# koadman/mauveAligner

Hardware: AMD Instinct MI355X
Metric: aligned Mbp/s (seed+extend+DP) (higher is better)
Workload: dtype u32; 1 GPU; C3: 5 x 5000000 bp synthetic genomes, ~3% divergence, ~50 inversions, seed weight 15, recursive anchoring + gapped DP on; genomes_per_gpu=5, genome_length=5000000, seed_weight=15, parallelism=independent genome sets per GPU (no data-path collective), extend_lcbs=1, max_extension_iters=4

## Files before the change

mauvealigner_amd/csrc/assemble_dev.hip:

```cpp
#include "common.hpp"
#include "dev_scan.hpp"
#include <cstring>
#include <cstdlib>
#include <algorithm>

namespace {
using namespace devscan;

__device__ __forceinline__ int64_t as_gap_len(const int32_t *__restrict__ alen, const int32_t *__restrict__ ast, int N, uint32_t k, int g)
{
    const int64_t sa = ast[(size_t)k * N + g], sb = ast[(size_t)(k + 1) * N + g];
    int64_t lo, hi;
    if (sa > 0) { lo = sa + alen[k]; hi = sb - 1; }
    else { lo = -sb + alen[k + 1]; hi = -sa - 1; }
    const int64_t ln = hi - lo + 1;
    return ln < 0 ? 0 : ln;
}

struct AsWidth {
    const int32_t *alen, *ast, *gapcode; const int64_t *dcol_off; int N;
    __device__ int64_t value(uint32_t a) const
    {
        int64_t w = alen[a];
        const int32_t code = gapcode[a];
        if (code >= 0) w += dcol_off[code + 1] - dcol_off[code];
        else if (code == -2) for (int g = 0; g < N; g++) w += as_gap_len(alen, ast, N, a, g);
        return w;
    }
};

__global__ void __launch_bounds__(256) as_lcb(const int32_t *__restrict__ alcb, const int32_t *__restrict__ gapcode, const int64_t *__restrict__ dscore,
                                              const int64_t *__restrict__ col0, uint32_t na, uint32_t *__restrict__ first_a, uint32_t *__restrict__ last_a,
                                              int64_t *__restrict__ lcb_col, unsigned long long *__restrict__ lcb_score)
{
    const uint32_t a = blockIdx.x * 256u + threadIdx.x;
    const bool in = a < na;
    const int32_t l = in ? alcb[a] : 0;
    const int32_t code = in ? gapcode[a] : -1;
    wave_keyed_add(lcb_score, code >= 0, (uint32_t)l, code >= 0 ? (unsigned long long)dscore[code] : 0ull);
    if (!in) return;
    if (a == 0 || alcb[a - 1] != l) { first_a[l] = a; lcb_col[l] = col0[a]; }
    if (a + 1 == na || alcb[a + 1] != l) last_a[l] = a;
}

__global__ void __launch_bounds__(256) as_extents(const int32_t *__restrict__ alen, const int32_t *__restrict__ ast, int N, uint32_t nl,
                                                  const uint32_t *__restrict__ first_a, const uint32_t *__restrict__ last_a,
                                                  int64_t *__restrict__ left, int64_t *__restrict__ right,
                                                  const unsigned long long *__restrict__ lw, int64_t *__restrict__ lw_row,
                                                  const int64_t *__restrict__ total_cols, int64_t *__restrict__ total_row)
{
    const uint32_t t = blockIdx.x * 256u + threadIdx.x;
    if (t >= nl * (uint32_t)N) return;
    const uint32_t l = t / (uint32_t)N; const int g = (int)(t % (uint32_t)N);
    if (g == 0) lw_row[l] = lw ? (int64_t)lw[l] : 0;
    if (t == 0) *total_row = *total_cols;
    const uint32_t a0 = first_a[l], a1 = last_a[l];
    const int64_t s0 = ast[(size_t)a0 * N + g], s1 = ast[(size_t)a1 * N + g];
    int64_t le, re;
    if (s0 > 0) { le = s0; re = s1 + alen[a1] - 1; }
    else { le = -s1; re = -s0 + alen[a0] - 1; }
    left[t] = s0 < 0 ? -le : le; right[t] = s0 < 0 ? -re : re;
}

__global__ void __launch_bounds__(256) as_fill(const int32_t *__restrict__ alen, const int32_t *__restrict__ ast, const int32_t *__restrict__ gapcode,
                                               const int64_t *__restrict__ dcol_off, const uint32_t *__restrict__ dcols,
                                               const int64_t *__restrict__ col0, uint32_t na, int N, uint32_t full, uint32_t *__restrict__ out)
{
    const int lane = threadIdx.x & 63;
    const uint32_t wave = (blockIdx.x * 256u + threadIdx.x) >> 6, nw = (gridDim.x * 256u) >> 6;
    for (uint32_t a = wave; a < na; a += nw) {
        uint32_t *o = out + col0[a];
        const int32_t ln = alen[a];
        for (int32_t c = lane; c < ln; c += 64) o[c] = full;
        o += ln;
        const int32_t code = gapcode[a];
        if (code >= 0) {
            const int64_t s0 = dcol_off[code], n = dcol_off[code + 1] - s0;
            for (int64_t c = lane; c < n; c += 64) o[c] = dcols[s0 + c];
        } else if (code == -2) {
            for (int g = 0; g < N; g++) {
                const int64_t n = as_gap_len(alen, ast, N, a, g);
                for (int64_t c = lane; c < n; c += 64) o[c] = 1u << g;
                o += n;
            }
        }
    }
}

struct Island { int64_t col, len; uint32_t bit, pad; };
__global__ void __launch_bounds__(256) as_islands(const Island *__restrict__ isl, uint32_t n, uint32_t *__restrict__ out)
{
    for (uint32_t k = blockIdx.x; k < n; k += gridDim.x) {
        const Island is = isl[k];
        uint32_t *o = out + is.col;
        for (int64_t c = threadIdx.x; c < is.len; c += 256) o[c] = is.bit;
    }
}

struct SpGenomes { uint64_t word_off[MAUVE_MAX_SEQ]; int32_t s[4][4]; };
template <int MODE>
__global__ void __launch_bounds__(256) sp_score_matches(const uint64_t *__restrict__ packed, SpGenomes G, int n, const int64_t *__restrict__ rec,
                                                        uint32_t nm, int64_t *__restrict__ out, SpMult M)
{
    const int lane = threadIdx.x & 63;
    const uint32_t wave = (blockIdx.x * 256u + threadIdx.x) >> 6, nw = (gridDim.x * 256u) >> 6;
    for (uint32_t i = wave; i < nm; i += nw) {
        const int64_t *r = rec + (size_t)i * (1 + n);
        const int64_t len = r[0];
        int64_t acc = 0;
        for (int64_t c = lane; c < len; c += 64) {
            uint32_t have = 0, bases = 0;
            uint64_t mlo = 0, mhi = 0;
            for (int g = 0; g < n; g++) {
                const int64_t st = r[1 + g];
                if (!st) continue;
                const int64_t p = st > 0 ? st - 1 + c : -st - 1 + (len - 1 - c);
                uint32_t b = (uint32_t)(packed[G.word_off[g] + (uint64_t)(p >> 5)] >> (2 * (p & 31))) & 3u;
                if (st < 0) b = 3u - b;
                have |= 1u << g; bases |= b << (2 * g);
                if (MODE) { const uint64_t mv = M.p[M.off[g] + (uint64_t)p]; if (g < 8) mlo |= mv << (8 * g); else mhi |= mv << (8 * (g - 8)); }
            }
            for (int x = 0; x < n; x++) {
                if (!(have >> x & 1)) continue;
                const uint32_t bx = (bases >> (2 * x)) & 3u;
                const uint32_t mx = MODE ? (uint32_t)((x < 8 ? mlo >> (8 * x) : mhi >> (8 * (x - 8))) & 255u) : 0u;
                for (int y = x + 1; y < n; y++)
                    if (have >> y & 1) {
                        const uint32_t my = MODE ? (uint32_t)((y < 8 ? mlo >> (8 * y) : mhi >> (8 * (y - 8))) & 255u) : 0u;
                        acc += sp_pair<MODE>(G.s[bx][(bases >> (2 * y)) & 3u], mx, my);
                    }
            }
        }
        for (int o = 32; o > 0; o >>= 1) acc += __shfl_xor(acc, o);
        if (lane == 0) out[i] = acc;
    }
}

__global__ void __launch_bounds__(256) as_widen_anchors(const int32_t *__restrict__ alen, const int32_t *__restrict__ ast, const int32_t *__restrict__ alcb, uint32_t na, int N,
                                                        int64_t *__restrict__ olen, int64_t *__restrict__ ost, int64_t *__restrict__ olcb)
{
    const uint32_t i = blockIdx.x * 256u + threadIdx.x;
    if (i < na) { olen[i] = alen[i]; olcb[i] = alcb[i]; }
    if (i < na * (uint32_t)N) ost[i] = ast[i];
}

}

int64_t sp_default_min_weight(int w, int n, const mauve_scoring *sc)
{
    int32_t d = sc->matrix[0][0];
    for (int a = 1; a < 4; a++) d = std::min(d, sc->matrix[a][a]);
    return (int64_t)3 * w * ((int64_t)n * (n - 1) / 2) * d;
}

int match_sp_scores(mauve_ctx *c, const MatchVec &m, const int *gmap, const mauve_scoring *sc, std::vector<int64_t> &out)
{
    const int n = m.N; const size_t nm = m.size();
    out.assign(nm, 0);
    if (nm == 0) return MAUVE_OK;
    if (n > 16) { c->err = "sum-of-pairs LCB scoring: at most 16 genomes"; return MAUVE_ERR_LIMIT; }
    for (size_t i = 0; i < nm; i++)
        for (int g = 0; g < n; g++) {
            const int64_t st = m.st(i)[g], L = c->lens[(size_t)(gmap ? gmap[g] : g)];
            if (st && m.len(i) > 0 && std::llabs(st) + m.len(i) - 1 > L) { c->err = "sp scores: match outside its genome"; return MAUVE_ERR_ARG; }
        }
    SpGenomes G; memset(&G, 0, sizeof G);
    for (int g = 0; g < n; g++) G.word_off[g] = c->word_off[(size_t)(gmap ? gmap[g] : g)];
    memcpy(G.s, sc->matrix, sizeof G.s);
    const size_t rb = nm * (1 + (size_t)n) * 8;
    HIPCHK(c, c->as_work.ensure(rb + nm * 8 + 64));
    HIPCHK(c, c->pin_asm.ensure(rb + nm * 8 + 64));
    int64_t *d_rec = c->as_work.as<int64_t>(), *d_out = d_rec + nm * (1 + (size_t)n);
    memcpy(c->pin_asm.p, m.d.data(), rb);
    HIPCHK(c, hipMemcpyAsync(d_rec, c->pin_asm.p, rb, hipMemcpyHostToDevice, c->stream));
    const uint32_t blocks = (uint32_t)std::min<size_t>((nm + 3) / 4, 256 * 8);
    SpMult M; memset(&M, 0, sizeof M);
    if (c->rp_now != MAUVE_REPEAT_PENALTY_OFF) {
        if (c->rp_gen != c->genome_gen) { c->err = "sp scores: repeat multiplicities missing"; return MAUVE_ERR_STATE; }
        M.p = c->rp_mult.as<uint8_t>();
        for (int g = 0; g < n; g++) M.off[g] = c->rp_off[(size_t)(gmap ? gmap[g] : g)];
    }
    if (c->rp_now == MAUVE_REPEAT_PENALTY_NEGATIVE)
        hipLaunchKernelGGL(sp_score_matches<MAUVE_REPEAT_PENALTY_NEGATIVE>, dim3(blocks), dim3(256), 0, c->stream, c->genomes.as<uint64_t>(), G, n, d_rec, (uint32_t)nm, d_out, M);
    else if (c->rp_now == MAUVE_REPEAT_PENALTY_ZERO)
        hipLaunchKernelGGL(sp_score_matches<MAUVE_REPEAT_PENALTY_ZERO>, dim3(blocks), dim3(256), 0, c->stream, c->genomes.as<uint64_t>(), G, n, d_rec, (uint32_t)nm, d_out, M);
    else
        hipLaunchKernelGGL(sp_score_matches<MAUVE_REPEAT_PENALTY_OFF>, dim3(blocks), dim3(256), 0, c->stream, c->genomes.as<uint64_t>(), G, n, d_rec, (uint32_t)nm, d_out, M);
    HIPCHK(c, hipGetLastError());
    int64_t *h_out = reinterpret_cast<int64_t *>(c->pin_asm.as<char>() + rb);
    HIPCHK(c, hipMemcpyAsync(h_out, d_out, nm * 8, hipMemcpyDeviceToHost, c->stream));
    HIPCHK(c, hipStreamSynchronize(c->stream));
    memcpy(out.data(), h_out, nm * 8);
    return MAUVE_OK;
}

int assemble_device(mauve_ctx *c, int64_t na64, int64_t cells, mauve_align_sizes *sizes, bool host_chains)
{
    static const bool trace = getenv("MAUVE_TRACE") != nullptr;
    AlignState &S = c->ast; AlignResult &R = c->res;
    const int N = S.N; const int64_t nl = S.nl; const uint32_t na = (uint32_t)na64;
    const mauve_ctx::DpFrontOut &fo = c->dpf_out;
    const double t0 = now_ms();
    c->stage.dp_ms = t0 - S.t_dp0;
    const uint32_t nb = (na + TILE - 1) / TILE, blocks = (na + 255) / 256;
    auto up8 = [](size_t x) { return (x + 7) & ~(size_t)7; };
    const size_t o_bsum = ((size_t)na + 1) * 8, o_first = o_bsum + ((size_t)nb + 8) * 8, o_last = up8(o_first + (size_t)nl * 4),
                 o_col = up8(o_last + (size_t)nl * 4), o_left = o_col + ((size_t)nl + 1) * 8, o_right = o_left + (size_t)nl * N * 8,
                 o_score = o_right + (size_t)nl * N * 8, o_lw = o_score + (size_t)nl * 8, o_tot = o_lw + (size_t)nl * 8, w_total = o_tot + 8;
    HIPCHK(c, c->as_work.ensure(w_total + 64));
    HIPCHK(c, c->res_cols.ensure(((size_t)S.sum + 64) * 4));
    char *wk = c->as_work.as<char>();
    int64_t *col0 = reinterpret_cast<int64_t *>(wk), *bsum = reinterpret_cast<int64_t *>(wk + o_bsum);
    uint32_t *first_a = reinterpret_cast<uint32_t *>(wk + o_first), *last_a = reinterpret_cast<uint32_t *>(wk + o_last);
    int64_t *lcb_col = reinterpret_cast<int64_t *>(wk + o_col), *left = reinterpret_cast<int64_t *>(wk + o_left),
            *right = reinterpret_cast<int64_t *>(wk + o_right);
    unsigned long long *score = reinterpret_cast<unsigned long long *>(wk + o_score);
    int64_t *lw_row = reinterpret_cast<int64_t *>(wk + o_lw), *tot_row = reinterpret_cast<int64_t *>(wk + o_tot);
    uint32_t *out = c->res_cols.as<uint32_t>();
    HIPCHK(c, hipMemsetAsync(score, 0, (size_t)nl * 8, c->stream));
    const AsWidth wf{fo.alen, fo.ast, fo.gapcode, fo.col_off, N};
    hipLaunchKernelGGL((vscan_partial<int64_t, AsWidth>), dim3(nb), dim3(256), 0, c->stream, wf, na, bsum);
    hipLaunchKernelGGL((vscan_write<int64_t, AsWidth>), dim3(nb), dim3(256), 0, c->stream, wf, na, bsum, col0, (int64_t *)nullptr);
    hipLaunchKernelGGL(as_lcb, dim3(blocks), dim3(256), 0, c->stream, fo.alcb, fo.gapcode, fo.score, col0, na, first_a, last_a, lcb_col, score);
    hipLaunchKernelGGL(as_extents, dim3(((uint32_t)nl * N + 255) / 256), dim3(256), 0, c->stream, fo.alen, fo.ast, N, (uint32_t)nl, first_a, last_a, left, right,
                       host_chains ? (const unsigned long long *)nullptr : c->ch_lw.as<unsigned long long>(), lw_row, col0 + na, tot_row);
    HIPCHK(c, hipGetLastError());
    const size_t rows_bytes = ((size_t)nl + 1) * 8 + 2 * (size_t)nl * N * 8 + 2 * (size_t)nl * 8 + 8;
    HIPCHK(c, c->pin_asm.ensure(64 + rows_bytes));
    int64_t *h_rows = c->pin_asm.as<int64_t>() + 8;
    HIPCHK(c, hipMemcpyAsync(h_rows, lcb_col, rows_bytes, hipMemcpyDeviceToHost, c->stream));
    {
        const uint32_t fb = (uint32_t)std::min<int64_t>(((int64_t)na + 3) / 4, 256 * 8);
        hipLaunchKernelGGL(as_fill, dim3(fb), dim3(256), 0, c->stream, fo.alen, fo.ast, fo.gapcode, fo.col_off, fo.cols, col0, na, N, S.full, out);
    }
    R.dev_nm = !host_chains && c->matches_pending ? (size_t)c->n_matches : 0;
    if (S.mums_kept >= 0) {
        std::swap(c->sorted_rec, c->sorted_rec_keep);
        R.dev_nm = (size_t)S.mums_kept; S.mums_kept = -1;
    }
    R.dev_alen = fo.alen; R.dev_ast = fo.ast; R.dev_alcb = fo.alcb;
    HIPCHK(c, hipGetLastError());
    if (c->pf.inflight) HIPCHK(c, hipStreamWaitEvent(c->stream, c->ev_io_done, 0));
    HIPCHK(c, hipStreamSynchronize(c->stream));
    c->pf.inflight = false;
    const double t1 = now_ms();
    const int64_t *h_col = h_rows, *h_left = h_col + nl + 1, *h_right = h_left + nl * N, *h_score = h_right + nl * N, *h_lw = h_score + nl;
    const int64_t lcb_cols = h_lw[nl];
    R.col_off.assign(h_col, h_col + nl);
    R.lcb_left.assign(h_left, h_left + nl * N); R.lcb_right.assign(h_right, h_right + nl * N);
    R.dp_score.assign(h_score, h_score + nl);
    if (!host_chains && !S.lw_from_host) R.lcb_weight.assign(h_lw, h_lw + nl);
    R.iv_left.assign((size_t)nl * N, 0); R.iv_right.assign((size_t)nl * N, 0); R.iv_reverse.assign((size_t)nl * N, 0);
    for (int64_t i = 0; i < nl * N; i++) {
        R.iv_left[(size_t)i] = std::llabs(R.lcb_left[(size_t)i]);
        R.iv_right[(size_t)i] = std::llabs(R.lcb_right[(size_t)i]);
        R.iv_reverse[(size_t)i] = R.lcb_left[(size_t)i] < 0;
    }
    int64_t ncols = lcb_cols, niv = nl;
    if (S.p.add_unaligned) {
        std::vector<Island> isl;
        for (int g = 0; g < N; g++) {
            std::vector<std::pair<int64_t, int64_t>> sp;
            for (int64_t l = 0; l < nl; l++) if (R.iv_left[(size_t)l * N + g]) sp.push_back({R.iv_left[(size_t)l * N + g], R.iv_right[(size_t)l * N + g]});
            std::sort(sp.begin(), sp.end());
            int64_t cur = 1;
            for (size_t i = 0; i <= sp.size(); i++) {
                const int64_t lo = cur, hi = i < sp.size() ? sp[i].first - 1 : c->lens[(size_t)g];
                if (hi >= lo) {
                    R.col_off.push_back(ncols);
                    Island is; is.col = ncols; is.len = hi - lo + 1; is.bit = 1u << g; is.pad = 0;
                    isl.push_back(is);
                    ncols += hi - lo + 1;
                    for (int h = 0; h < N; h++) { R.iv_left.push_back(h == g ? lo : 0); R.iv_right.push_back(h == g ? hi : 0); R.iv_reverse.push_back(0); }
                    R.dp_score.push_back(0);
                    niv++;
                }
                if (i < sp.size() && sp[i].second + 1 > cur) cur = sp[i].second + 1;
            }
        }
        if (ncols > S.sum) { c->err = "assemble_device: more columns than bases (internal error)"; return MAUVE_ERR_HIP; }
        if (!isl.empty()) {
            const size_t ib = isl.size() * sizeof(Island);
            HIPCHK(c, c->pin_asm.ensure(64 + rows_bytes + ib + 64));
            char *pi = c->pin_asm.as<char>() + 64 + rows_bytes;
            memcpy(pi, isl.data(), ib);
            HIPCHK(c, c->as_isl.ensure(ib + 64));
            HIPCHK(c, hipMemcpyAsync(c->as_isl.p, pi, ib, hipMemcpyHostToDevice, c->stream));
            hipLaunchKernelGGL(as_islands, dim3((uint32_t)std::min<size_t>(isl.size(), 1024)), dim3(256), 0, c->stream,
                               c->as_isl.as<Island>(), (uint32_t)isl.size(), out);
            HIPCHK(c, hipGetLastError());
            HIPCHK(c, hipStreamSynchronize(c->stream));
        }
    }
    R.col_off.push_back(ncols);
    R.n_cols = (size_t)ncols;
    if (host_chains && !S.anchor_table_done) {
        R.anchor_length.resize((size_t)na); R.anchor_start.resize((size_t)na * N); R.anchor_lcb.resize((size_t)na);
        size_t a = 0;
        for (int64_t l = 0; l < nl; l++) {
            const MatchVec &ch = S.chains[(size_t)l];
            for (size_t i = 0; i < ch.size(); i++, a++) {
                R.anchor_length[a] = ch.len(i); R.anchor_lcb[a] = l;
                std::copy(ch.st(i), ch.st(i) + N, &R.anchor_start[a * N]);
            }
        }
    }
    R.dev_pending = true; R.cols_pending = true; R.dev_na = host_chains ? 0 : na; R.cols_ext = nullptr;
    {
        mauve_ctx::TablePrefetch &P = c->pf;
        const bool dm = P.got_mums && !host_chains, da = P.got_anchors && !host_chains;
        R.del_mum_length = dm ? P.mum_length : nullptr; R.del_mum_start = dm ? P.mum_start : nullptr;
        R.del_alen = da ? P.anchor_length : nullptr; R.del_ast = da ? P.anchor_start : nullptr; R.del_alcb = da ? P.anchor_lcb : nullptr;
        P.got_mums = P.got_anchors = false;
    }
    R.cols_fill = 0; R.cols_dirty.clear();
    R.sz.n_mums = S.nm; R.sz.n_lcb = nl; R.sz.n_anchor = na; R.sz.n_iv = niv; R.sz.n_cols = ncols;
    R.sz.n_gap_dp = fo.n_dp; R.sz.n_dp_cells = cells;
    *sizes = R.sz;
    const double t2 = now_ms();
    if (trace) fprintf(stderr, "[trace] assemble (device): layout+fill %.3f ms, islands+tables %.3f\n", t1 - t0, t2 - t1);
    c->stage.assemble_ms = t2 - t0;
    c->stage.total_ms = t2 - S.t0;
    S.open = false;
    return MAUVE_OK;
}

int materialize_tables(mauve_ctx *c)
{
    AlignResult &R = c->res;
    R.del_mum_length = R.del_mum_start = R.del_alen = R.del_ast = R.del_alcb = nullptr;
    if (!R.dev_pending) return MAUVE_OK;
    HIPCHK(c, hipSetDevice(c->device));
    const int N = c->ast.N; const size_t na = R.dev_na;
    const size_t ab = (na * (2 + (size_t)N) * 4 + 63) & ~(size_t)63, mb = R.dev_nm * (1 + (size_t)N) * 8;
    HIPCHK(c, c->pin_tab.ensure(ab + mb + 64));
    char *pa = c->pin_tab.as<char>();
    if (ab) {
        HIPCHK(c, hipMemcpyAsync(pa, R.dev_alen, na * 4, hipMemcpyDeviceToHost, c->stream));
        HIPCHK(c, hipMemcpyAsync(pa + na * 4, R.dev_ast, na * N * 4, hipMemcpyDeviceToHost, c->stream));
        HIPCHK(c, hipMemcpyAsync(pa + na * 4 * (1 + (size_t)N), R.dev_alcb, na * 4, hipMemcpyDeviceToHost, c->stream));
    }
    if (mb) HIPCHK(c, hipMemcpyAsync(pa + ab, c->sorted_rec.p, mb, hipMemcpyDeviceToHost, c->stream));
    HIPCHK(c, hipStreamSynchronize(c->stream));
    if (mb) {
        const int64_t *hm = reinterpret_cast<const int64_t *>(pa + ab);
        R.mum_length.assign(hm, hm + R.dev_nm); R.mum_start.assign(hm + R.dev_nm, hm + R.dev_nm * (1 + (size_t)N));
        R.dev_nm = 0;
    }
    const int32_t *hl = reinterpret_cast<const int32_t *>(pa), *hs = hl + na, *hb = hs + na * N;
    if (na) {
        R.anchor_length.resize(na); R.anchor_start.resize(na * N); R.anchor_lcb.resize(na);
        for (size_t a = 0; a < na; a++) { R.anchor_length[a] = hl[a]; R.anchor_lcb[a] = hb[a]; }
        for (size_t i = 0; i < na * N; i++) R.anchor_start[i] = hs[i];
    }
    R.dev_pending = false;
    return MAUVE_OK;
}

bool fetch_tables_direct(mauve_ctx *c, int64_t *mum_length, int64_t *mum_start, int64_t *anchor_length, int64_t *anchor_start, int64_t *anchor_lcb, int *rc_out)
{
    AlignResult &R = c->res;
    *rc_out = MAUVE_OK;
    if (!R.dev_pending) return false;
    const int N = c->ast.N; const size_t na = R.dev_na, nm = R.dev_nm;
    if (nm && !(host_pointer_is_pinned(mum_length) && host_pointer_is_pinned(mum_start))) return false;
    if (na && !(host_pointer_is_pinned(anchor_length) && host_pointer_is_pinned(anchor_start) && host_pointer_is_pinned(anchor_lcb))) return false;
    auto chk = [&](hipError_t e) { if (e != hipSuccess && *rc_out == MAUVE_OK) { c->err = std::string("fetch: ") + hipGetErrorString(e); *rc_out = MAUVE_ERR_HIP; } };
    chk(hipSetDevice(c->device));
    if (na) {
        chk(c->as_wide.ensure(na * (2 + (size_t)N) * 8 + 64));
        if (*rc_out) return true;
        int64_t *wl = c->as_wide.as<int64_t>(), *ws = wl + na, *wb = ws + na * N;
        hipLaunchKernelGGL(as_widen_anchors, dim3((uint32_t)((na * N + 255) / 256)), dim3(256), 0, c->stream, R.dev_alen, R.dev_ast, R.dev_alcb, (uint32_t)na, N, wl, ws, wb);
        chk(hipGetLastError());
        chk(hipMemcpyAsync(anchor_length, wl, na * 8, hipMemcpyDeviceToHost, c->stream));
        chk(hipMemcpyAsync(anchor_start, ws, na * N * 8, hipMemcpyDeviceToHost, c->stream));
        chk(hipMemcpyAsync(anchor_lcb, wb, na * 8, hipMemcpyDeviceToHost, c->stream));
    }
    if (nm) {
        const int64_t *rec = c->sorted_rec.as<int64_t>();
        chk(hipMemcpyAsync(mum_length, rec, nm * 8, hipMemcpyDeviceToHost, c->stream));
        chk(hipMemcpyAsync(mum_start, rec + nm, nm * N * 8, hipMemcpyDeviceToHost, c->stream));
    }
    return true;
}

template <typename T>
__global__ void __launch_bounds__(256) as_narrow_cols(const uint32_t *__restrict__ in, size_t n, T *__restrict__ out)
{
    const size_t i0 = ((size_t)blockIdx.x * 256 + threadIdx.x) * 16;
    if (i0 + 16 <= n) {
        uint4 v[4];
#pragma unroll
        for (int q = 0; q < 4; q++) v[q] = reinterpret_cast<const uint4 *>(in + i0)[q];
        T o[16];
#pragma unroll
        for (int q = 0; q < 4; q++) { o[4 * q] = (T)v[q].x; o[4 * q + 1] = (T)v[q].y; o[4 * q + 2] = (T)v[q].z; o[4 * q + 3] = (T)v[q].w; }
        uint4 *dst = reinterpret_cast<uint4 *>(out + i0);
#pragma unroll
        for (int q = 0; q < (int)(sizeof(T) * 16 / 16); q++) dst[q] = reinterpret_cast<const uint4 *>(o)[q];
    } else
        for (size_t i = i0; i < n; i++) out[i] = (T)in[i];
}
__global__ void __launch_bounds__(256) as_narrow_i64(const int64_t *__restrict__ in, size_t n, int32_t *__restrict__ out)
{
    const size_t i = (size_t)blockIdx.x * 256 + threadIdx.x;
    if (i < n) out[i] = (int32_t)in[i];
}

bool fetch_compact_direct(mauve_ctx *c, int col_bytes, int32_t *mum_length, int32_t *mum_start, int32_t *anchor_length, int32_t *anchor_start, int32_t *anchor_lcb,
                          void *cols, bool *tables_done, bool *cols_done, int *rc_out)
{
    AlignResult &R = c->res;
    *rc_out = MAUVE_OK; *tables_done = false; *cols_done = false;
    auto chk = [&](hipError_t e) { if (e != hipSuccess && *rc_out == MAUVE_OK) { c->err = std::string("fetch_compact: ") + hipGetErrorString(e); *rc_out = MAUVE_ERR_HIP; } };
    const int N = c->ast.N; const size_t na = R.dev_na, nm = R.dev_nm;
    bool any = false;
    const bool have_m = R.del_mum_length && R.del_mum_length == mum_length && R.del_mum_start == mum_start;
    const bool have_a = R.del_alen && R.del_alen == anchor_length && R.del_ast == anchor_start && R.del_alcb == anchor_lcb;
    R.del_mum_length = R.del_mum_start = R.del_alen = R.del_ast = R.del_alcb = nullptr;
    if (R.dev_pending && mum_length && mum_start && anchor_length && anchor_start && anchor_lcb &&
        (!nm || have_m || (host_pointer_is_pinned(mum_length) && host_pointer_is_pinned(mum_start))) &&
        (!na || have_a || (host_pointer_is_pinned(anchor_length) && host_pointer_is_pinned(anchor_start) && host_pointer_is_pinned(anchor_lcb)))) {
        chk(hipSetDevice(c->device));
        if (na && !have_a) {
            chk(hipMemcpyAsync(anchor_length, R.dev_alen, na * 4, hipMemcpyDeviceToHost, c->stream));
            chk(hipMemcpyAsync(anchor_start, R.dev_ast, na * N * 4, hipMemcpyDeviceToHost, c->stream));
            chk(hipMemcpyAsync(anchor_lcb, R.dev_alcb, na * 4, hipMemcpyDeviceToHost, c->stream));
        }
        if (nm && !have_m) {
            const size_t n = nm * (1 + (size_t)N);
            chk(c->as_wide.ensure(n * 4 + 64));
            if (*rc_out) return true;
            hipLaunchKernelGGL(as_narrow_i64, dim3((uint32_t)((n + 255) / 256)), dim3(256), 0, c->stream, c->sorted_rec.as<int64_t>(), n, c->as_wide.as<int32_t>());
            chk(hipGetLastError());
            chk(hipMemcpyAsync(mum_length, c->as_wide.as<int32_t>(), nm * 4, hipMemcpyDeviceToHost, c->stream));
            chk(hipMemcpyAsync(mum_start, c->as_wide.as<int32_t>() + nm, nm * N * 4, hipMemcpyDeviceToHost, c->stream));
        }
        *tables_done = true; any = true;
    }
    if (cols && R.n_cols && R.cols_pending && host_pointer_is_pinned(cols)) {
        chk(hipSetDevice(c->device));
        const size_t n = R.n_cols;
        if (col_bytes == 4) chk(hipMemcpyAsync(cols, c->res_cols.p, n * 4, hipMemcpyDeviceToHost, c->stream));
        else {
            chk(c->res_narrow.ensure(n * (size_t)col_bytes + 64));
            if (*rc_out) return true;
            const uint32_t blocks = (uint32_t)((n + 4095) / 4096);
            if (col_bytes == 1) hipLaunchKernelGGL(as_narrow_cols<uint8_t>, dim3(blocks), dim3(256), 0, c->stream, c->res_cols.as<uint32_t>(), n, c->res_narrow.as<uint8_t>());
            else hipLaunchKernelGGL(as_narrow_cols<uint16_t>, dim3(blocks), dim3(256), 0, c->stream, c->res_cols.as<uint32_t>(), n, c->res_narrow.as<uint16_t>());
            chk(hipGetLastError());
            chk(hipMemcpyAsync(cols, c->res_narrow.p, n * (size_t)col_bytes, hipMemcpyDeviceToHost, c->stream));
        }
        *cols_done = true; any = true;
    }
    if (any) chk(hipStreamSynchronize(c->stream));
    return any;
}

int prefetch_tables_enqueue(mauve_ctx *c, int N, int64_t na, const int32_t *alen, const int32_t *ast, const int32_t *alcb)
{
    mauve_ctx::TablePrefetch &P = c->pf;
    P.got_mums = P.got_anchors = false;
    if (!P.live) return MAUVE_OK;
    P.live = false;
    const size_t nm = c->matches_pending && c->dev_rec_n == c->n_matches ? (size_t)c->n_matches : 0;
    const bool mums = nm && P.mum_length && P.mum_start && (int64_t)nm <= P.mum_cap;
    const bool anch = na > 0 && P.anchor_length && P.anchor_start && P.anchor_lcb && na <= P.anchor_cap;
    if (!mums && !anch) return MAUVE_OK;
    const size_t n = nm * (1 + (size_t)N);
    if (mums) {
        HIPCHK(c, c->pf_mums.ensure(n * 4 + 64));
    }
    HIPCHK(c, hipStreamWaitEvent(c->stream_io, c->ev_io_fork, 0));
// ... 52 lines not shown
```

mauvealigner_amd/csrc/common.hpp:

```cpp
#pragma once
#include <hip/hip_runtime.h>
#include <cstdint>
#include <cstdio>
#include <string>
#include <vector>
#include <functional>
#include "workers.hpp"
#include "host_chain.hpp"
#include <chrono>
#include <algorithm>
#include <cstring>

#include "../../include/mauve_hip.h"

#define HIPCHK(ctx, call)                                                                         \
    do {                                                                                          \
        hipError_t e__ = (call);                                                                  \
        if (e__ != hipSuccess) {                                                                  \
            (ctx)->err = std::string(#call) + ": " + hipGetErrorString(e__) + " (" __FILE__ ":" + \
                         std::to_string(__LINE__) + ")";                                          \
            return MAUVE_ERR_HIP;                                                                 \
        }                                                                                         \
    } while (0)

// ... 89 lines not shown
    int64_t *n_matches = nullptr;
};

struct AlignResult {
    mauve_align_sizes sz{};
    std::vector<int64_t> mum_length, mum_start;
    std::vector<int64_t> lcb_left, lcb_right, lcb_weight;
    std::vector<int64_t> anchor_length, anchor_start, anchor_lcb;
    std::vector<int64_t> iv_left, iv_right;
    std::vector<int8_t> iv_reverse;
    std::vector<int64_t> col_off;
    std::vector<uint32_t> cols;
    size_t n_cols = 0;
    uint32_t cols_fill = 0;
    std::vector<std::pair<size_t, size_t>> cols_dirty;
    std::vector<int64_t> dp_score;
    bool stale = false;
    bool genomes_replaced = false;
    bool dev_pending = false;
    bool cols_pending = false;
    size_t dev_na = 0, dev_nm = 0;
    const int32_t *dev_alen = nullptr, *dev_ast = nullptr, *dev_alcb = nullptr;
    const uint32_t *cols_ext = nullptr;
    const int32_t *del_mum_length = nullptr, *del_mum_start = nullptr, *del_alen = nullptr, *del_ast = nullptr, *del_alcb = nullptr;
    const uint32_t *cols_data() const { return cols_ext ? cols_ext : cols.data(); }
};

struct AlignState {
    typedef ::GapRef GapRef;
    struct Item { int64_t lcb; uint32_t idx; int64_t col0; int64_t gap; };
    bool open = false;
    bool anchor_table_done = false;
    bool dev_tail = false;
    const int32_t *dv_len = nullptr, *dv_st = nullptr, *dv_lcb = nullptr;
    bool lw_from_host = false;
    int64_t mums_kept = -1;
    mauve_params p{};
    int N = 0; uint32_t full = 0;
    int64_t sum = 0, nm = 0, nl = 0, n_dp = 0, code_total = 0, n_anchor = 0, anchor_cols = 0;
    double t0 = 0, t_dp0 = 0;
    std::vector<MatchVec> chains;
    std::vector<GapRef> gaps;
    std::vector<DpSeqDesc> desc;
    std::vector<int64_t> dcol_off, dscore;
    MatchVec m;
    std::vector<int64_t> match_lcb;
    std::vector<int64_t> match_weight;
    std::vector<Item> items;
    void count_anchors() { for (const MatchVec &ch : chains) { n_anchor += (int64_t)ch.size(); for (size_t i = 0; i < ch.size(); i++) anchor_cols += ch.len(i); } }
    void reset()
    {
        open = false; anchor_table_done = false; dev_tail = false; dv_len = dv_st = dv_lcb = nullptr; lw_from_host = false; mums_kept = -1; p = mauve_params(); N = 0; full = 0;
        sum = nm = nl = n_dp = code_total = n_anchor = anchor_cols = 0; t0 = t_dp0 = 0;
        gaps.clear(); desc.clear(); dcol_off.clear(); dscore.clear();
        match_lcb.clear(); match_weight.clear(); items.clear();
    }
};

struct CoordDev;
struct mauve_ctx {
    int device = 0;
    hipStream_t stream = nullptr;
    hipStream_t stream2 = nullptr;
    hipEvent_t ev_fork = nullptr, ev_join = nullptr;
    hipStream_t stream_io = nullptr;
    hipEvent_t ev_io_fork = nullptr, ev_io_done = nullptr;
    struct TablePrefetch {
        int32_t *mum_length = nullptr, *mum_start = nullptr, *anchor_length = nullptr, *anchor_start = nullptr, *anchor_lcb = nullptr;
        int64_t mum_cap = 0, anchor_cap = 0;
        bool armed = false;
        bool live = false;
        bool inflight = false;
        bool got_mums = false, got_anchors = false;
    } pf;
    DevBuf pf_mums;
    std::string err;
    char devname[256] = {0};
    int cus = 256;

    int nseq = 0;
    std::vector<int64_t> lens;
    std::vector<uint64_t> word_off;
    std::vector<const uint64_t *> host_packed;
    PinnedBuf pin_genomes;
    PinnedBuf pin_tail;
    bool host_copy_valid = false;
    size_t total_words = 0;
    DevBuf genomes;
    DevBuf base_invalid, contig_mask, node_cmask;
    bool has_invalid = false, has_contigs = false;
    std::vector<uint64_t> h_invalid, h_contig, base_mask_off;

    DevBuf keysA, keysB, valsA, valsB, hist, totals, posmask, hit_mask, hit_pos, hit_seg, cand, mlen, mstart, counters;
    DevBuf sorted_rec;
    DevBuf canon_k1, canon_k2, canon_v1, canon_v2;
    DevBuf join_bound;
    DevBuf join_ovf;
    DevBuf ch_len, ch_st, ch_crop, ch_ent, ch_ord, ch_rank, ch_node, ch_graph, ch_cnt;
    DevBuf gap_work;
    DevBuf ch_big;
    DevBuf ch_anch, ch_lw;
    DevBuf ch_anch2, ext_work, sorted_rec_keep;
    PinnedBuf pin_ext;
    DevBuf ch_mw;
    DevBuf as_wide;
    DevBuf res_narrow;
    DevBuf hom_cols;
    DevBuf as_work, as_isl, res_cols;
    PinnedBuf pin_tab;
    PinnedBuf pin_asm, pin_cols;
    PinnedBuf pin_chain;
    PinnedBuf pin_mask;
    struct BackboneResult {
        int N = 0; bool valid = false;
        std::vector<int64_t> seg_iv, seg_col, seg_len, seg_left, seg_right, islands;
        std::vector<uint32_t> seg_mask;
    } bb;
    PinnedBuf pin_bb;
    DevBuf bb_cols, bb_work, bb_query;
    size_t bb_rec_cap = 0;
    struct CoordIndex { bool valid = false; int N = 0; int64_t n_iv = 0, n_cols = 0; uint64_t genome_gen = 0; struct ::CoordDev *dev = nullptr; } co;
    DevBuf co_index, co_q;
    PinnedBuf pin_stage;
    CoordIndex co_truth;
    DevBuf co_truth_index, sc_out;
    struct ExtractSel {
        bool valid = false; uint64_t genome_gen = 0;
        int64_t n_sel = 0, n_range = 0;
        int n_keep = 0; int32_t keep[MAUVE_MAX_SEQ] = {0};
    } ex;
    DevBuf ex_work, ex_bits, ex_sel, ex_mat;
    DevBuf ps_work, ps_out;
    struct Excursions { bool valid = false; uint64_t genome_gen = 0; int64_t n_stream = 0, n_exc = 0; } exc;
    DevBuf exc_work, exc_tmp, exc_meta, exc_rec;
    DevBuf run_sum;
    DevBuf rec_vinv, rec_vcm;
    DevBuf rec_genomes, rec_seg;
    DevBuf placed_mask;
    std::vector<int64_t> match_len, match_start;
    int64_t n_matches = 0;
    int64_t dev_rec_n = -1;

    DevBuf dp_desc, dp_list, dp_codes, dp_off, dp_prof_cnt, dp_prof_mask, dp_prof2_cnt, dp_prof2_mask, dp_tb, dp_meta, dp_score,
        dp_cols, dp_rows, dp_sp, dp_pick, dp_wflags;

    bool pair_sums_only = false;
    std::vector<int64_t> pair_sums;
    int64_t bp_min_len = -1;
    std::vector<int64_t> pair_bp;
    DevBuf bp_work;
    std::vector<uint8_t> rec_flags;
    bool lazy_matches_ok = false, matches_pending = false;
    int match_nseq = 0;
    struct DpFrontOut { const int32_t *alen, *ast, *alcb, *gapcode; const int64_t *col_off, *score; const uint32_t *cols; int64_t n_dp, n_cols; } dpf_out{};
    std::vector<DpSeqDesc> prog_desc;
    const int64_t *dp_last_col_off = nullptr; int64_t dp_last_n = 0;
    int64_t dp_band_from = INT64_MAX;
    DevBuf dpf_anch, dpf_work, dpf_tot;

    bool prof = false;
    hipEvent_t ev0 = nullptr, ev1 = nullptr;
    double k_ms[MAUVE_K_COUNT] = {0};
    int64_t k_launch[MAUVE_K_COUNT] = {0};
    int64_t k_units[MAUVE_K_COUNT] = {0};

    PinnedBuf pin_anch;
    PinnedBuf pin_dcols;
    PinnedBuf pin_meta;
    PinnedBuf pin_dp_in;
    PinnedBuf pin_seed;
    struct DpHost {
        std::vector<int64_t> tb_off, rows_off, est, need, nmax, lst, lst2, seq_off, tb_list;
        std::vector<uint8_t> is_big, cls;
    } dph;
    struct SeedHost {
        std::vector<int32_t> hl, hs;
        std::vector<uint32_t> order, tmp;
        std::vector<uint64_t> k1;
    } sdh;

    std::function<void()> shadow;

    SpinPool *pool = nullptr;

    int shard_rank = 0, shard_world = 1; mauve_allgather_fn shard_fn = nullptr; void *shard_user = nullptr;
    bool shard_on = false;
    void *shard_comm = nullptr;
    DevBuf shard_dev;
    PinnedBuf shard_pin;
    mauve_shard_stats shard_stat = {0, 0, 0, 0.0};

    int repeat_mode = MAUVE_REPEAT_PENALTY_OFF, rp_now = MAUVE_REPEAT_PENALTY_OFF;
    uint64_t genome_gen = 0;
    uint64_t rp_gen = 0, rp_pat = 0;
    DevBuf rp_wcnt, rp_mult;
    std::vector<uint64_t> rp_off;

    AlignResult res;
    AlignState ast;
    mauve_stage_times stage{};
};

struct SpMult { const uint8_t *p; uint64_t off[MAUVE_MAX_SEQ]; };
template <int MODE>
__device__ __forceinline__ int64_t sp_pair(int32_t s, uint32_t mx, uint32_t my)
{
    if (MODE == MAUVE_REPEAT_PENALTY_OFF || s <= 0) return s;
    const int64_t r = (int64_t)(mx > my ? mx : my);
    return MODE == MAUVE_REPEAT_PENALTY_NEGATIVE ? (int64_t)s * (2 - r) / r : (int64_t)s / r;
}

struct RepeatScope {
    mauve_ctx *c;
    explicit RepeatScope(mauve_ctx *ctx) : c(ctx) { c->rp_now = MAUVE_REPEAT_PENALTY_OFF; }
    ~RepeatScope() { c->rp_now = MAUVE_REPEAT_PENALTY_OFF; }
};

struct KernelTimer {
    mauve_ctx *c; int id; int64_t units;
    KernelTimer(mauve_ctx *ctx, int kid, int64_t u) : c(ctx), id(kid), units(u)
    {
        if (c->prof) (void)hipEventRecord(c->ev0, c->stream);
    }
    ~KernelTimer()
    {
        if (!c->prof) return;
        (void)hipEventRecord(c->ev1, c->stream);
        (void)hipEventSynchronize(c->ev1);
        float ms = 0.f;
        (void)hipEventElapsedTime(&ms, c->ev0, c->ev1);
        c->k_ms[id] += ms; c->k_launch[id] += 1; c->k_units[id] += units;
    }
};

static inline double now_ms()
{
    using namespace std::chrono;
    return duration<double, std::milli>(steady_clock::now().time_since_epoch()).count();
}

int rec_gap_flags_device(mauve_ctx *c, const int32_t *alen, const int32_t *ast, const int32_t *alcb, int64_t na, int N, int64_t min_gap, uint8_t *d_flag);
int shard_allgather(mauve_ctx *c, const void *send, size_t bytes, std::vector<std::pair<const char *, size_t>> &parts);
void shard_lpt(const std::vector<int64_t> &cost, int world, std::vector<int> &owner);
bool make_seed_shape(uint64_t pattern, SeedShape *out);
GenomeSet main_genome_set(mauve_ctx *ctx);
bool seedpass_wide(int64_t total_windows);
int refuse_scoring(mauve_ctx *c, const mauve_scoring *sc, const char *what);
int refuse_scoring_batch(mauve_ctx *c, const mauve_scoring *sc, int nseq, int64_t n_iv, const int64_t *seq_off, const char *what);
int refuse_scoring_params(mauve_ctx *c, const mauve_params *p, const char *what);
int refuse_past_2g(mauve_ctx *c, const char *what);
int seedpass_run(mauve_ctx *ctx, const GenomeSet &gs, uint64_t pattern, int mode, uint64_t mask, int extend,
                 const uint32_t *seg_dev, uint32_t nseg, int64_t *n_matches);
int seedpass_enumerate(mauve_ctx *ctx, const GenomeSet &gs, int seq, uint64_t pattern, EnumRequest &q);
int seedpass_from_hits(mauve_ctx *ctx, const GenomeSet &gs, uint64_t pattern, const HostHits &hits, int extend, int64_t *n_matches);
int seedpass_sorted_list(mauve_ctx *ctx, const GenomeSet &gs, int seq, uint64_t pattern, std::vector<uint64_t> *keys,
                         std::vector<uint32_t> *vals, int *weight);

int sort_pairs_u32(mauve_ctx *ctx, uint32_t n, int key_bits, uint32_t **keys_io, uint32_t **vals_io, uint32_t *keys_alt, uint32_t *vals_alt,
                   int timer_id);
int sort_pairs_u32_batch(mauve_ctx *ctx, uint32_t S, uint32_t n, size_t seg_stride, int key_bits, uint32_t **keys_io, uint32_t **vals_io,
                         uint32_t *keys_alt, uint32_t *vals_alt, int timer_id);
int sort_pairs_u64(mauve_ctx *ctx, uint32_t n, int key_bits, uint64_t **keys_io, uint32_t **vals_io, uint64_t *keys_alt, uint32_t *vals_alt,
                   int timer_id);
int seed_finish(mauve_ctx *ctx, const GenomeSet &gs, const SeedRequest &rq, uint32_t ncand, bool on_host, double &trace_t0);
bool seed_trace_on();
uint32_t canon_device_min();
inline void seed_trace(mauve_ctx *ctx, const char *label, double &t0)
{
    if (!seed_trace_on()) return;
    (void)hipStreamSynchronize(ctx->stream);
    const double t = now_ms();
    fprintf(stderr, "[trace] %-22s +%.3f ms\n", label, t - t0);
    t0 = t;
}
inline int seed_counters(mauve_ctx *ctx, size_t bytes, const uint32_t **words)
{
    HIPCHK(ctx, ctx->pin_seed.ensure(64));
    HIPCHK(ctx, hipMemcpyAsync(ctx->pin_seed.p, ctx->counters.p, bytes, hipMemcpyDeviceToHost, ctx->stream));
    HIPCHK(ctx, hipStreamSynchronize(ctx->stream));
    *words = ctx->pin_seed.as<uint32_t>();
    return MAUVE_OK;
}
int chain_device(mauve_ctx *c, int N, int64_t min_weight, bool collinear, MatchVec &m, std::vector<int64_t> &match_lcb, int64_t &n_lcb, const mauve_scoring *sp_scoring = nullptr);
struct ChainGraphHost { uint32_t na, K; int64_t *weight; uint32_t *orient; int32_t *prev, *next; int32_t *final_stage; int32_t *final_dev; };
int chain_device_graph(mauve_ctx *c, int N, int64_t maxlen, const uint32_t *seg0, uint32_t nseg, ChainGraphHost *G, bool graph_to_host = true, const mauve_scoring *sp_scoring = nullptr);
int chain_device_gaps_compact(mauve_ctx *c, int N, int64_t maxlen, const uint32_t *seg0_dev, uint32_t nseg, const int32_t **hl_out, const int32_t **hs_out,
                              const uint32_t **hgap_out, uint32_t *ns_out);
int chain_device_core(mauve_ctx *c, int N, int64_t min_weight, bool collinear, int64_t &n_lcb, const mauve_scoring *sp_scoring = nullptr);
int chain_device_gaps(mauve_ctx *c, int N, int64_t maxlen, const uint32_t *seg0_dev, uint32_t nseg, const int32_t **hl_out, const int32_t **hs_out,
                      std::vector<uint8_t> &survive);
int chain_device_copy_back(mauve_ctx *c, int N, MatchVec &m, std::vector<int64_t> &match_lcb);
int chain_order_device(mauve_ctx *c, int N, int64_t nl, int64_t min_gap, int64_t *na_out, int64_t *n_rec_out);
int extend_lcbs_device(mauve_ctx *c, const mauve_params *p, int w, int64_t lcbw, int N, const int32_t **alen_io, const int32_t **ast_io,
                       const int32_t **alcb_io, int64_t *na_io, int64_t *nl_io, int64_t *n_rec_io, std::vector<int64_t> &lcb_weight);

struct ChainOrders { std::vector<std::vector<uint32_t>> ord; bool sparse = false; };
void host_eliminate_overlaps(MatchVec &m, ChainOrders *orders = nullptr, bool compact = true);
int seed_family_matches(mauve_ctx *c, const GenomeSet &gs, int w, int mode, uint64_t mask, MatchVec &out);
void host_merge_matches(MatchVec &kept, const MatchVec &add);
void host_left_orders(const MatchVec &m, ChainOrders &orders);
void host_lcb_chain(const MatchVec &m, int64_t min_weight, bool collinear, std::vector<int64_t> &match_lcb, int64_t &n_lcb,
                    const ChainOrders *orders = nullptr, const int64_t *match_weight = nullptr);
int match_sp_scores(mauve_ctx *c, const MatchVec &m, const int *gmap, const mauve_scoring *sc, std::vector<int64_t> &out);
int repeat_multiplicity(mauve_ctx *c, uint64_t pattern);
int repeat_begin(mauve_ctx *c, const mauve_params *p, int w, uint64_t pat);
int64_t sp_default_min_weight(int w, int n, const mauve_scoring *sc);
int resolve_seed(mauve_ctx *c, const mauve_params *p, int64_t avg_len, const char *who, int *w, uint64_t *pat);
void seed_matches_to_vec(const mauve_ctx *c, int n, int64_t nm, MatchVec &m);
int host_chain_lcbs(mauve_ctx *c, const mauve_params *p, MatchVec &m, const int *gmap, int64_t lcbw, int64_t minw_sp, std::vector<int64_t> &match_lcb,
                    int64_t &nl, std::vector<int64_t> *match_weight, bool compact, double *t_elim = nullptr);
void result_reset(AlignResult &R);
void restore_cols(AlignResult &R, uint32_t full, SpinPool *pool = nullptr);

void lcb_greedy(int N, int32_t K, int64_t *weight, const uint32_t *orient_bits, int32_t *prevv, int32_t *nextv, int64_t min_weight,
                bool collinear, std::vector<int64_t> &final_id, int64_t &n_lcb);

int dp_batch_run_desc(mauve_ctx *ctx, int nseq, int64_t n_iv, const DpSeqDesc *desc, const mauve_scoring *sc,
                      uint32_t *cols, int64_t *col_off, int64_t *score, int64_t *cells, bool may_shard = false, int64_t *sp = nullptr);
bool dp_desc_rotations_on_device(int64_t n_total);
int dp_batch_run_desc_rot(mauve_ctx *ctx, int nseq, int64_t n_orig, const DpSeqDesc *desc, const int32_t *cbase, int64_t n_total, const mauve_scoring *sc,
                          int64_t *col_off, int64_t *score, int64_t *cells, int64_t *sp);
inline int64_t dp_len_limit(const mauve_params *p) { return p->max_banded_len > p->max_gapped_len ? p->max_banded_len : p->max_gapped_len; }
inline int64_t dp_band_from_of(const mauve_params *p) { return p->max_banded_len > p->max_gapped_len ? p->max_gapped_len : INT64_MAX; }
int dp_run_from_anchors(mauve_ctx *ctx, int N, int64_t na, const int32_t *h_len, const int32_t *h_st, const int32_t *h_lcb, int gapped,
                        int64_t max_gapped_len, const mauve_scoring *scoring, int32_t *gapcode, int64_t *n_dp_out, int64_t *code_total_out,
                        PinnedBuf *dcols, std::vector<int64_t> &dcol_off, std::vector<int64_t> &dscore, int64_t *cells, int stay = 0);
int assemble_device(mauve_ctx *c, int64_t na, int64_t cells, mauve_align_sizes *sizes, bool host_chains = false);
int check_columns(mauve_ctx *c, const char *who, int N, int64_t n_iv, const int64_t *left, const int64_t *right, const int64_t *col_off, const uint32_t *d_cols);
void coord_index_release(mauve_ctx *c);
int coord_index_arrays(mauve_ctx *c, const char *who, mauve_ctx::CoordIndex &X, DevBuf &index, int nseq, int64_t n_iv, const int64_t *left, const int64_t *right,
                       const int8_t *reverse, const int64_t *col_off, const uint32_t *cols);
int materialize_result(mauve_ctx *c);
int materialize_tables(mauve_ctx *c);
int fetch_columns(mauve_ctx *c, uint32_t *dst);
bool fetch_compact_direct(mauve_ctx *c, int col_bytes, int32_t *mum_length, int32_t *mum_start, int32_t *anchor_length, int32_t *anchor_start, int32_t *anchor_lcb,
                          void *cols, bool *tables_done, bool *cols_done, int *rc_out);
int prefetch_tables_enqueue(mauve_ctx *c, int N, int64_t na, const int32_t *alen, const int32_t *ast, const int32_t *alcb);
bool fetch_tables_direct(mauve_ctx *c, int64_t *mum_length, int64_t *mum_start, int64_t *anchor_length, int64_t *anchor_start, int64_t *anchor_lcb, int *rc_out);
bool host_pointer_is_pinned(const void *p);
inline int copy_to_caller(mauve_ctx *c, PinnedBuf &pin, void *dst, const void *src, size_t bytes)
{
    if (!bytes) return MAUVE_OK;
    if (host_pointer_is_pinned(dst)) { HIPCHK(c, hipMemcpyAsync(dst, src, bytes, hipMemcpyDeviceToHost, c->stream)); return MAUVE_OK; }
    const size_t piece = (size_t)64 << 20;
    HIPCHK(c, pin.ensure(std::min(bytes, piece)));
    for (size_t o = 0; o < bytes; o += piece) {
        const size_t n = std::min(piece, bytes - o);
        HIPCHK(c, hipMemcpyAsync(pin.p, static_cast<const char *>(src) + o, n, hipMemcpyDeviceToHost, c->stream));
        HIPCHK(c, hipStreamSynchronize(c->stream));
        memcpy(static_cast<char *>(dst) + o, pin.p, n);
    }
    return MAUVE_OK;
}
int host_genomes(mauve_ctx *c);
int seed_matches_to_host(mauve_ctx *ctx);
int dp_fetch_picked(mauve_ctx *ctx, int64_t n_pick, const int64_t *pick, const int64_t *col_off, uint32_t *out, int64_t *out_off);
int dp_batch_run(mauve_ctx *ctx, int nseq, int64_t n_iv, const uint8_t *codes, const int64_t *seq_off,
                 const mauve_scoring *sc, uint32_t *cols, int64_t *col_off, int64_t *score, int64_t *cells);
```

mauvealigner_amd/csrc/dev_scan.hpp:

```cpp
#pragma once
#include <hip/hip_runtime.h>
#include <cstdint>

namespace devscan {

constexpr int TILE = 1024;

__device__ __forceinline__ uint32_t bscan_add(uint32_t v, uint32_t *total, uint32_t *lds )
{
    const int lane = threadIdx.x & 63, wave = threadIdx.x >> 6;
    uint32_t inc = v;
#pragma unroll
    for (int o = 1; o < 64; o <<= 1) { const uint32_t t = __shfl_up(inc, o); if (lane >= o) inc += t; }
    __syncthreads();
    if (lane == 63) lds[wave] = inc;
    __syncthreads();
    uint32_t wbase = 0, tot = 0;
#pragma unroll
    for (int w = 0; w < 4; w++) { const uint32_t c = lds[w]; if (w < wave) wbase += c; tot += c; }
    *total = tot;
    return wbase + inc - v;
}
__device__ __forceinline__ uint32_t bscan_max(uint32_t v, uint32_t *total, uint32_t *lds )
{
    const int lane = threadIdx.x & 63, wave = threadIdx.x >> 6;
    uint32_t inc = v;
#pragma unroll
    for (int o = 1; o < 64; o <<= 1) { const uint32_t t = __shfl_up(inc, o); if (lane >= o) inc = max(inc, t); }
    __syncthreads();
    if (lane == 63) lds[wave] = inc;
    __syncthreads();
    uint32_t wbase = 0, tot = 0;
#pragma unroll
    for (int w = 0; w < 4; w++) { const uint32_t c = lds[w]; if (w < wave) wbase = max(wbase, c); tot = max(tot, c); }
    *total = tot;
    const uint32_t up = __shfl_up(inc, 1);
    return max(wbase, lane ? up : 0u);
}
__device__ __forceinline__ void tiles_before_add(const uint32_t *__restrict__ v, uint32_t b, uint32_t nb, uint32_t *before, uint32_t *all, uint32_t *lds)
{
    uint32_t sb = 0, sa = 0;
    for (uint32_t t = threadIdx.x; t < nb; t += 256) { const uint32_t x = v[t]; sa += x; if (t < b) sb += x; }
    uint32_t tb, ta;
    (void)bscan_add(sb, &tb, lds); (void)bscan_add(sa, &ta, lds);
    *before = tb; *all = ta;
}

__device__ __forceinline__ void wave_keyed_add(unsigned long long *arr, bool active, uint32_t l, unsigned long long v)
{
    const uint64_t act = __ballot(active);
    if (!act) return;
    const int first = __ffsll((unsigned long long)act) - 1;
    const uint32_t l0 = (uint32_t)__shfl((int)l, first);
    if (__ballot(active && l == l0) == act) {
        unsigned long long s = active ? v : 0ull;
#pragma unroll
        for (int o = 32; o > 0; o >>= 1) s += __shfl_xor(s, o);
        if ((int)(threadIdx.x & 63) == first) atomicAdd(&arr[l0], s);
    } else if (active) atomicAdd(&arr[l], v);
}

template <class F>
__global__ void __launch_bounds__(256) cmp_count(F f, uint32_t *__restrict__ bcnt)
{
    __shared__ uint32_t lds[4];
    const int y = blockIdx.y;
    const uint32_t dom = f.domain(y), r0 = blockIdx.x * (uint32_t)TILE + threadIdx.x * 4u;
    uint32_t c = 0;
#pragma unroll
    for (int i = 0; i < 4; i++) if (r0 + i < dom) c += f.flag(r0 + i, y) ? 1u : 0u;
    uint32_t tc;
    (void)bscan_add(c, &tc, lds);
    if (threadIdx.x == 0) bcnt[(size_t)y * gridDim.x + blockIdx.x] = tc;
}
template <class F>
__global__ void __launch_bounds__(256) cmp_write(F f, const uint32_t *__restrict__ bcnt)
{
    __shared__ uint32_t lds[4];
    const int y = blockIdx.y;
    const uint32_t dom = f.domain(y), r0 = blockIdx.x * (uint32_t)TILE + threadIdx.x * 4u;
    uint32_t before, all;
    tiles_before_add(bcnt + (size_t)y * gridDim.x, blockIdx.x, gridDim.x, &before, &all, lds);
    bool fl[4]; uint32_t c = 0;
#pragma unroll
    for (int i = 0; i < 4; i++) { fl[i] = r0 + i < dom && f.flag(r0 + i, y); c += fl[i] ? 1u : 0u; }
    uint32_t dummy;
    uint32_t o = before + bscan_add(c, &dummy, lds);
#pragma unroll
    for (int i = 0; i < 4; i++) {
        if (r0 + i >= dom) break;
        f.each(r0 + i, o, fl[i], y);
        if (fl[i]) { f.emit(r0 + i, o, y); o++; }
    }
    if (blockIdx.x == 0 && threadIdx.x == 0) f.total(all, y);
}


template <class T, class In>
__global__ void __launch_bounds__(256) vscan_partial(In in, uint32_t n, T *__restrict__ bsum)
{
    __shared__ T red[4];
    const uint32_t r0 = blockIdx.x * (uint32_t)TILE + threadIdx.x * 4u;
    T s = 0;
#pragma unroll
    for (int i = 0; i < 4; i++) if (r0 + i < n) s += in.value(r0 + i);
#pragma unroll
    for (int o = 32; o > 0; o >>= 1) s += __shfl_down(s, o);
    if ((threadIdx.x & 63) == 0) red[threadIdx.x >> 6] = s;
    __syncthreads();
    if (threadIdx.x == 0) bsum[blockIdx.x] = red[0] + red[1] + red[2] + red[3];
}
template <class T, class In>
__global__ void __launch_bounds__(256) vscan_write(In in, uint32_t n, const T *__restrict__ bsum, T *__restrict__ out, T *__restrict__ total)
{
    __shared__ T red[4];
    __shared__ T s_before, s_all;
    const int lane = threadIdx.x & 63, wave = threadIdx.x >> 6;
    T sb = 0, sa = 0;
    for (uint32_t t = threadIdx.x; t < gridDim.x; t += 256) { const T x = bsum[t]; sa += x; if (t < blockIdx.x) sb += x; }
#pragma unroll
    for (int o = 32; o > 0; o >>= 1) { sb += __shfl_down(sb, o); sa += __shfl_down(sa, o); }
    if (lane == 0) red[wave] = sb;
    __syncthreads();
    if (threadIdx.x == 0) s_before = red[0] + red[1] + red[2] + red[3];
    __syncthreads();
    if (lane == 0) red[wave] = sa;
    __syncthreads();
    if (threadIdx.x == 0) s_all = red[0] + red[1] + red[2] + red[3];
    __syncthreads();
    const uint32_t r0 = blockIdx.x * (uint32_t)TILE + threadIdx.x * 4u;
    T v[4], s = 0;
#pragma unroll
    for (int i = 0; i < 4; i++) { v[i] = r0 + i < n ? in.value(r0 + i) : (T)0; s += v[i]; }
    T inc = s;
#pragma unroll
    for (int o = 1; o < 64; o <<= 1) { const T t = __shfl_up(inc, o); if (lane >= o) inc += t; }
    __syncthreads();
    if (lane == 63) red[wave] = inc;
    __syncthreads();
    T run = s_before + inc - s;
    for (int w = 0; w < wave; w++) run += red[w];
#pragma unroll
    for (int i = 0; i < 4; i++) { if (r0 + i < n) out[r0 + i] = run; run += v[i]; }
    if (blockIdx.x == 0 && threadIdx.x == 0) { if (total) *total = s_all; out[n] = s_all; }
}

}
```

mauvealigner_amd/csrc/dp_batch.hip:

```cpp
#include "common.hpp"
#include "dev_scan.hpp"
#include <algorithm>
#include <functional>
#include <cstring>
#include <cstdlib>

#define DP_NEG_INF (-(1 << 29))

struct DpMeta {
    int32_t m;
    int32_t krows;
    int32_t cur;
    int32_t pad;
    int64_t score;
    int64_t cells;
};

struct DpScoring { int32_t go, ge; int32_t s[4][4]; };

__device__ __forceinline__ void dp_row_coef(uint32_t cn, const DpScoring &sc, int32_t &s0, int32_t &s1, int32_t &s2, int32_t &s3, int32_t &gxo, int32_t &gxe)
{
    const int32_t c0 = cn & 255, c1 = (cn >> 8) & 255, c2 = (cn >> 16) & 255, c3 = cn >> 24;
    const int32_t rr = c0 + c1 + c2 + c3;
    s0 = c0 * sc.s[0][0] + c1 * sc.s[1][0] + c2 * sc.s[2][0] + c3 * sc.s[3][0];
// ... 1437 lines not shown
        }
        for (int o = 32; o; o >>= 1) total += __shfl_xor(total, o);
        if (lane == 0) out[iv] = (unsigned long long)total;
    }
}

struct DpGenomeWords { uint64_t word_off[MAUVE_MAX_SEQ]; };

__global__ void __launch_bounds__(256) dp_gather_codes(const uint64_t *__restrict__ packed, DpGenomeWords gw,
                                                       const DpSeqDesc *__restrict__ desc, const int64_t *__restrict__ seq_off,
                                                       int64_t ndesc, uint8_t *__restrict__ codes)
{
    const int lane = threadIdx.x & 63, sub = lane >> 4, sl = lane & 15;
    const int64_t wave_global = ((int64_t)blockIdx.x * blockDim.x + threadIdx.x) >> 6;
    const int64_t nwaves = ((int64_t)gridDim.x * blockDim.x) >> 6;
    for (int64_t d0 = wave_global * 4; d0 < ndesc; d0 += nwaves * 4) {
        const int64_t d = d0 + sub;
        if (d >= ndesc) continue;
        const DpSeqDesc ds = desc[d];
        const uint64_t *G = packed + gw.word_off[ds.genome];
        uint8_t *out = codes + seq_off[d];
        for (int64_t i = sl; i < ds.len; i += 16) {
            const int64_t p = ds.rev ? ds.lo0 + ds.len - 1 - i : ds.lo0 + i;
            const uint32_t b = (uint32_t)(G[p >> 5] >> (2 * (p & 31))) & 3u;
            out[i] = (uint8_t)(ds.rev ? 3u - b : b);
        }
    }
}

struct DpSizing {
    int64_t need = 0, est = 0;
    __host__ __device__ DpSizing(int64_t band_from, bool no_mw_, bool no_groups_, int class_mode, int64_t longest)
        : banded(longest > band_from), no_mw(no_mw_), no_groups(no_groups_), mode(class_mode) {}
    __host__ __device__ void add(int64_t n)
    {
        if (n == 0) return;
        if (first) { first = false; mmax = mmin = n; return; }
        const int64_t tbo = dp_tb_need(mmin, mmax, n, banded);
        const int64_t tbn = banded ? tbo : max2(tbo, max2(dp2_tb_need(mmax, n), dp3_tb_need(mmax, n)));
        rneed = max2(rneed, dp3_rows_need(mmax, n));
        need = max2(need, tbn);
        nmax = max2(nmax, n);
        const int64_t e_m = min2(mmax, mmin + mmin / 8 + 2);
        if (max2(e_m, n) > DP3_BAND && !no_mw) wide = true;
        est += dp3_scan_steps(e_m, n);
        crows = max2(crows, mode == 0 ? e_m : min2(mmax, mode == 1 ? mmax : mmin / 2 + 1));
        mmax += n; mmin = max2(mmin, n);
    }
    __host__ __device__ int64_t rows() const { return max2(6 * (nmax + 1), rneed); }
    __host__ __device__ uint8_t cand() const { return banded && nmax ? 2 : (wide ? 1 : 0); }
    __host__ __device__ uint8_t cls() const
    {
        if (no_groups || banded) return 1;
        if (crows <= 4 * DP2_R && nmax + 4 <= DP2_T) return 4;
        if (crows <= 8 * DP2_R && nmax + 8 <= DP2_T) return 3;
        if (crows <= 16 * DP2_R && nmax + 16 <= DP2_T) return 2;
        return 1;
    }
    __host__ __device__ static uint32_t sizekey(int64_t need) { int c = 0; for (int64_t f = need; f > 1; f >>= 1) c++; return (uint32_t)(63 - c); }
    __host__ __device__ uint32_t sizekey() const { return sizekey(need); }
private:
    __host__ __device__ static int64_t max2(int64_t a, int64_t b) { return a > b ? a : b; }
    __host__ __device__ static int64_t min2(int64_t a, int64_t b) { return a < b ? a : b; }
    bool banded, no_mw, no_groups, wide = false, first = true; int mode;
    int64_t mmin = 0, mmax = 0, nmax = 0, rneed = 0, crows = 0;
};

static int dp_class_mode()
{
    static const int m = []() { const char *e = getenv("MAUVE_DP_CLASS"); return !e ? 0 : (!strcmp(e, "bound") ? 1 : (!strcmp(e, "wild") ? 2 : 0)); }();
    return m;
}
static int64_t dp_wide_min() { static const int64_t f = getenv("MAUVE_DP_WIDE_MIN") ? atoll(getenv("MAUVE_DP_WIDE_MIN")) : 1024; return f; }
static int64_t dp_big_max() { static const int64_t m = getenv("MAUVE_DP_BIG_MAX") ? atoll(getenv("MAUVE_DP_BIG_MAX")) : 256; return m; }
static bool dp_wide_on() { static const bool o = getenv("MAUVE_DP_NO_WIDE") == nullptr; return o; }

static int dp_launch_steps(mauve_ctx *ctx, int nseq, int64_t a, int64_t b, int64_t n_big, int64_t big_len, const DpClasses &full, const int64_t *d_seq_off,
                           const int64_t *d_tb_off, const int64_t *d_rows_off, const DpScoring &sc, int64_t tb_base, int64_t band_from)
{
    auto clip = [&](int64_t first, int64_t n, int64_t &f2, int64_t &n2) { f2 = std::max(first, a); n2 = std::max<int64_t>(0, std::min(first + n, b) - f2); };
    int64_t bf, bn;
    clip(0, n_big, bf, bn);
    DpClasses cl; memset(&cl, 0, sizeof cl);
    clip(full.first_med, full.n_med, cl.first_med, cl.n_med);
    clip(full.first_c, full.n_c, cl.first_c, cl.n_c);
    clip(full.first_s32, full.n_s32, cl.first_s32, cl.n_s32);
    clip(full.first_s16, full.n_s16, cl.first_s16, cl.n_s16);
    static const bool no_scan = getenv("MAUVE_DP_NOSCAN") != nullptr;
    cl.scan = no_scan ? 0 : 1;
    const int64_t wpb = DP2_WAVES, cap = 256 * 16;
    cl.blocks_med = (uint32_t)std::min<int64_t>((cl.n_med + wpb - 1) / wpb, cap);
    cl.blocks_c = (uint32_t)std::min<int64_t>((cl.n_c + 4 * wpb - 1) / (4 * wpb), cap);
    cl.blocks_s32 = (uint32_t)std::min<int64_t>((cl.n_s32 + 8 * wpb - 1) / (8 * wpb), cap);
    const uint32_t blocks = cl.blocks_med + cl.blocks_c + cl.blocks_s32 + (uint32_t)std::min<int64_t>((cl.n_s16 + 16 * wpb - 1) / (16 * wpb), cap);
    uint8_t *tb = ctx->dp_tb.as<uint8_t>() - tb_base;
    KernelTimer t(ctx, MAUVE_K_DP, b - a);
#define DP_STEP_ARGS ctx->dp_codes.as<uint8_t>(), d_seq_off, ctx->dp_meta.as<DpMeta>(), ctx->dp_prof_cnt.as<uint32_t>(), ctx->dp_prof_mask.as<uint32_t>(), \
                     ctx->dp_prof2_cnt.as<uint32_t>(), ctx->dp_prof2_mask.as<uint32_t>(), tb, d_tb_off, ctx->dp_rows.as<int32_t>(), d_rows_off, \
                     ctx->dp_score.as<uint8_t>(), sc
    hipStream_t small_stream = bn ? ctx->stream2 : ctx->stream;
    if (bn) {
        HIPCHK(ctx, hipEventRecord(ctx->ev_fork, ctx->stream));
        HIPCHK(ctx, hipStreamWaitEvent(ctx->stream2, ctx->ev_fork, 0));
        const bool wide = dp_wide_on();
        static const int64_t cl_max = getenv("MAUVE_DP_CLUSTER") ? atoll(getenv("MAUVE_DP_CLUSTER")) : 32;
        const int64_t n_cl = wide ? std::min<int64_t>(bn, cl_max) : 0;
        unsigned long long *flags = nullptr;
        if (n_cl) {
            HIPCHK(ctx, ctx->dp_wflags.ensure((size_t)n_cl * DPW_FLAGS * 8));
            HIPCHK(ctx, hipMemsetAsync(ctx->dp_wflags.p, 0, (size_t)n_cl * DPW_FLAGS * 8, ctx->stream));
            flags = ctx->dp_wflags.as<unsigned long long>();
        }
#define DPW_LAUNCH(first, count, K) hipLaunchKernelGGL((dp_step_wide<4, 8>), dim3((uint32_t)((count) * (K))), dim3(64 * 8), 0, ctx->stream, nseq, \
                               ctx->dp_list.as<int64_t>() + bf + (first), DP_STEP_ARGS, band_from, (int)(K), flags)
        if (wide) { if (n_cl) DPW_LAUNCH(0, n_cl, DPW_KMAX); if (bn > n_cl) DPW_LAUNCH(n_cl, bn - n_cl, 1); }
#undef DPW_LAUNCH
        if (!wide || band_from != INT64_MAX || !dp3_admissible(std::max<int64_t>(big_len, 1), nseq, sc.ge, sc.go))
            hipLaunchKernelGGL(dp_step_big, dim3((uint32_t)bn), dim3(64 * DP_MW_WAVES), 0, ctx->stream, nseq, ctx->dp_list.as<int64_t>() + bf, DP_STEP_ARGS,
                               band_from, wide ? 1 : 0);
    }
    if (blocks) hipLaunchKernelGGL(dp_step2, dim3(blocks), dim3(64 * DP2_WAVES), 0, small_stream, nseq, ctx->dp_list.as<int64_t>(), cl, DP_STEP_ARGS);
#undef DP_STEP_ARGS
    if (bn) { HIPCHK(ctx, hipEventRecord(ctx->ev_join, ctx->stream2)); HIPCHK(ctx, hipStreamWaitEvent(ctx->stream, ctx->ev_join, 0)); }
    return MAUVE_OK;
}

static int64_t dp_tb_budget()
{
    static const int64_t b = getenv("MAUVE_DP_TB_BUDGET") ? atoll(getenv("MAUVE_DP_TB_BUDGET")) : (8LL << 30);
    return std::max<int64_t>(b, 1 << 16);
}
static int dp_launch_rounds(mauve_ctx *ctx, int nseq, int64_t n_iv, int64_t n_big, int64_t big_len, const DpClasses &cl, const int64_t *d_seq_off,
                            const int64_t *d_tb_off, const int64_t *d_rows_off, const DpScoring &sc, const int64_t *tb_list, int *rounds_out,
                            int64_t band_from)
{
    const int64_t budget = dp_tb_budget();
    int rounds = 0;
    for (int64_t a = 0; a < n_iv;) {
        int64_t b = a + 1;
        if (tb_list) {
            if (tb_list[a + 1] - tb_list[a] > budget) { ctx->err = "dp: one interval needs more traceback than MAUVE_DP_TB_BUDGET allows"; return MAUVE_ERR_LIMIT; }
            while (b < n_iv && tb_list[b + 1] - tb_list[a] <= budget) b++;
        } else b = n_iv;
        int rc = dp_launch_steps(ctx, nseq, a, b, n_big, big_len, cl, d_seq_off, d_tb_off, d_rows_off, sc, tb_list ? tb_list[a] : 0, band_from);
        if (rc) return rc;
        rounds++;
        a = b;
    }
    if (rounds_out) *rounds_out = rounds;
    return MAUVE_OK;
}

static const char *const DP_ERR_CLUSTER = "dp: a cluster of workgroups could not make progress on an interval (wide sweep)";
static DpScoring dp_scoring_of(const mauve_scoring *scoring)
{
    DpScoring sc; sc.go = scoring->gap_open; sc.ge = scoring->gap_extend; memcpy(sc.s, scoring->matrix, sizeof sc.s);
    return sc;
}
static int dp_ensure_batch(mauve_ctx *ctx, int64_t total, int64_t tbt, int64_t rwt)
{
    HIPCHK(ctx, ctx->dp_codes.ensure((size_t)total + 16));
    HIPCHK(ctx, ctx->dp_prof_cnt.ensure((size_t)(total + 1) * 4));
    HIPCHK(ctx, ctx->dp_prof_mask.ensure((size_t)(total + 1) * 4));
    HIPCHK(ctx, ctx->dp_prof2_cnt.ensure((size_t)(total + 1) * 4));
    HIPCHK(ctx, ctx->dp_prof2_mask.ensure((size_t)(total + 1) * 4));
    HIPCHK(ctx, ctx->dp_tb.ensure((size_t)std::min<int64_t>(tbt, dp_tb_budget()) + 64));
    HIPCHK(ctx, ctx->dp_rows.ensure((size_t)(rwt + 1) * 4));
    HIPCHK(ctx, ctx->dp_score.ensure((size_t)total + 16));
    HIPCHK(ctx, ctx->dp_cols.ensure((size_t)(total + 1) * 4));
    return MAUVE_OK;
}
static void dp_launch_gather_codes(mauve_ctx *ctx, const int64_t *d_seq_off, int64_t nd)
{
    DpGenomeWords gw; memset(&gw, 0, sizeof gw);
    for (int g = 0; g < ctx->nseq; g++) gw.word_off[g] = ctx->word_off[g];
    const uint32_t gb = (uint32_t)std::min<int64_t>((nd + 15) / 16, 256 * 8);
    hipLaunchKernelGGL(dp_gather_codes, dim3(gb), dim3(256), 0, ctx->stream, ctx->genomes.as<uint64_t>(), gw, ctx->dp_desc.as<DpSeqDesc>(), d_seq_off, nd,
                       ctx->dp_codes.as<uint8_t>());
}

static int dp_core(mauve_ctx *ctx, int nseq, int64_t n_iv, const uint8_t *codes, const DpSeqDesc *desc,
                   const int64_t *seq_off, const mauve_scoring *scoring, uint32_t *cols, int64_t *col_off,
                   int64_t *score, int64_t *cells, int64_t *sp = nullptr)
{
    if (cells) *cells = 0;
    col_off[0] = 0;
    if (n_iv == 0) return MAUVE_OK;
    static const bool trace = getenv("MAUVE_TRACE") != nullptr;
    const double td0 = now_ms();
    const int64_t total = seq_off[n_iv * nseq];
    mauve_ctx::DpHost &H = ctx->dph;
    std::vector<int64_t> &tb_off = H.tb_off, &rows_off = H.rows_off, &est = H.est;
    std::vector<uint8_t> &is_big = H.is_big;
    tb_off.resize((size_t)n_iv + 1); rows_off.resize((size_t)n_iv + 1);
    is_big.assign((size_t)n_iv, 0); est.assign((size_t)n_iv, 0);
    int64_t est_total = 0;
    const int64_t band_from = ctx->dp_band_from;
    static const bool no_mw = getenv("MAUVE_DP_ONE_WAVE") != nullptr;
    static const bool no_groups = getenv("MAUVE_DP_NO_GROUPS") != nullptr;
    std::vector<uint8_t> &cls = H.cls; cls.assign((size_t)n_iv, 1);
    int64_t tbt = 0, rwt = 0;
    std::vector<int64_t> &need_v = H.need, &nmax_v = H.nmax;
    need_v.resize((size_t)n_iv); nmax_v.resize((size_t)n_iv);
    ctx->pool->parallel_for(n_iv, 2048, [&](int64_t b, int64_t e) {
        for (int64_t iv = b; iv < e; iv++) {
            int64_t longest = 0;
            for (int g = 0; g < nseq; g++) longest = std::max(longest, seq_off[iv * nseq + g + 1] - seq_off[iv * nseq + g]);
            DpSizing z(band_from, no_mw, no_groups, dp_class_mode(), longest);
            for (int g = 0; g < nseq; g++) z.add(seq_off[iv * nseq + g + 1] - seq_off[iv * nseq + g]);
            need_v[(size_t)iv] = z.need; nmax_v[(size_t)iv] = z.rows(); est[(size_t)iv] = z.est; is_big[(size_t)iv] = z.cand(); cls[(size_t)iv] = z.cls();
        }
    });
    for (int64_t iv = 0; iv < n_iv; iv++) {
        tb_off[iv] = tbt; rows_off[iv] = rwt;
        tbt += need_v[(size_t)iv]; rwt += nmax_v[(size_t)iv];
        est_total += est[(size_t)iv];
    }
    tb_off[n_iv] = tbt; rows_off[n_iv] = rwt;

    const DpScoring sc = dp_scoring_of(scoring);
    std::vector<int64_t> &lst = H.lst; lst.resize((size_t)n_iv);
    {
        int64_t cnt[66] = {0};
        auto cls = [&](int64_t iv) { return DpSizing::sizekey(need_v[(size_t)iv]); };
        for (int64_t iv = 0; iv < n_iv; iv++) cnt[cls(iv) + 1]++;
        for (int c = 0; c < 65; c++) cnt[c + 1] += cnt[c];
        for (int64_t iv = 0; iv < n_iv; iv++) lst[(size_t)cnt[cls(iv)]++] = iv;
    }
    int64_t n_big = 0;
    {
        for (int64_t k = 0; k < n_iv; k++) {
            uint8_t &b = is_big[(size_t)lst[(size_t)k]];
            if (b == 1 && (n_big >= dp_big_max() || est[(size_t)lst[(size_t)k]] < dp_wide_min())) b = 0;
            n_big += b != 0;
        }
    }
    DpClasses cl; memset(&cl, 0, sizeof cl);
    {
        std::vector<int64_t> &tmp = H.lst2; tmp.resize((size_t)n_iv);
        int64_t cnt4[5] = {0, 0, 0, 0, 0};
        auto klass = [&](int64_t iv) { return is_big[(size_t)iv] ? 0 : (int)cls[(size_t)iv]; };
        for (int64_t k = 0; k < n_iv; k++) cnt4[klass(lst[(size_t)k])]++;
        int64_t pos[5] = {0, cnt4[0], cnt4[0] + cnt4[1], cnt4[0] + cnt4[1] + cnt4[2], cnt4[0] + cnt4[1] + cnt4[2] + cnt4[3]};
        cl.first_med = pos[1]; cl.n_med = cnt4[1]; cl.first_c = pos[2]; cl.n_c = cnt4[2]; cl.first_s32 = pos[3]; cl.n_s32 = cnt4[3]; cl.first_s16 = pos[4]; cl.n_s16 = cnt4[4];
        for (int64_t k = 0; k < n_iv; k++) { const int64_t iv = lst[(size_t)k]; tmp[(size_t)pos[klass(iv)]++] = iv; }
        lst.swap(tmp);
    }
    int64_t big_len = 0;
    for (int64_t k = 0; k < n_big; k++) { const int64_t iv = lst[(size_t)k]; big_len = std::max(big_len, seq_off[(iv + 1) * nseq] - seq_off[iv * nseq]); }
    std::vector<int64_t> &tb_list = H.tb_list; tb_list.resize((size_t)n_iv + 1);
    tbt = 0;
    for (int64_t k = 0; k < n_iv; k++) { const int64_t iv = lst[(size_t)k]; tb_off[iv] = tbt; tb_list[(size_t)k] = tbt; tbt += need_v[(size_t)iv]; }
    tb_list[(size_t)n_iv] = tbt; tb_off[n_iv] = tbt;
    const bool one_round = tbt <= dp_tb_budget();

    { int rce = dp_ensure_batch(ctx, total, tbt, rwt); if (rce) return rce; }
    HIPCHK(ctx, ctx->dp_off.ensure((size_t)(n_iv * nseq + 1 + 3 * (n_iv + 1)) * sizeof(int64_t)));
    HIPCHK(ctx, ctx->dp_meta.ensure((size_t)n_iv * sizeof(DpMeta)));
    int64_t *d_seq_off = ctx->dp_off.as<int64_t>();
    int64_t *d_tb_off = d_seq_off + (n_iv * nseq + 1);
    int64_t *d_rows_off = d_tb_off + (n_iv + 1);
    int64_t *d_col_off = d_rows_off + (n_iv + 1);
    const size_t n_so = (size_t)(n_iv * nseq + 1), n_o = (size_t)n_iv + 1;
    const size_t desc_bytes = desc ? (size_t)n_iv * nseq * sizeof(DpSeqDesc) : 0;
    HIPCHK(ctx, ctx->pin_dp_in.ensure((n_so + 3 * n_o) * 8 + desc_bytes + 64));
    int64_t *pin_off = ctx->pin_dp_in.as<int64_t>();
    memcpy(pin_off, seq_off, n_so * 8);
    memcpy(pin_off + n_so, tb_off.data(), n_o * 8);
    memcpy(pin_off + n_so + n_o, rows_off.data(), n_o * 8);
    HIPCHK(ctx, hipMemcpyAsync(d_seq_off, pin_off, (n_so + 2 * n_o) * 8, hipMemcpyHostToDevice, ctx->stream));
    if (desc) {
        const int64_t nd = n_iv * nseq;
        HIPCHK(ctx, ctx->dp_desc.ensure((size_t)nd * sizeof(DpSeqDesc)));
        char *pin_desc = reinterpret_cast<char *>(pin_off + n_so + 3 * n_o);
        memcpy(pin_desc, desc, desc_bytes);
        HIPCHK(ctx, hipMemcpyAsync(ctx->dp_desc.p, pin_desc, desc_bytes, hipMemcpyHostToDevice, ctx->stream));
        dp_launch_gather_codes(ctx, d_seq_off, nd);
    } else if (total) {
        HIPCHK(ctx, hipMemcpyAsync(ctx->dp_codes.p, codes, (size_t)total, hipMemcpyHostToDevice, ctx->stream));
    }
    const double td1 = now_ms();
    HIPCHK(ctx, ctx->dp_list.ensure((size_t)n_iv * 8));
    int64_t *pin_list = pin_off + n_so + 2 * n_o;
    memcpy(pin_list, lst.data(), (size_t)n_iv * 8);
    HIPCHK(ctx, hipMemcpyAsync(ctx->dp_list.p, pin_list, (size_t)n_iv * 8, hipMemcpyHostToDevice, ctx->stream));
    int rounds = 1;
    { int rcl = dp_launch_rounds(ctx, nseq, n_iv, n_big, big_len, cl, d_seq_off, d_tb_off, d_rows_off, sc, one_round ? nullptr : tb_list.data(), &rounds, band_from); if (rcl) return rcl; }
    HIPCHK(ctx, hipGetLastError());
    if (ctx->shadow) { std::function<void()> f; f.swap(ctx->shadow); f(); }
    HIPCHK(ctx, ctx->pin_meta.ensure((size_t)n_iv * sizeof(DpMeta)));
    DpMeta *hm = ctx->pin_meta.as<DpMeta>();
    const double td2 = now_ms();
    HIPCHK(ctx, hipMemcpyAsync(hm, ctx->dp_meta.p, (size_t)n_iv * sizeof(DpMeta), hipMemcpyDeviceToHost, ctx->stream));
    HIPCHK(ctx, hipStreamSynchronize(ctx->stream));
    const double td3 = now_ms();
    int64_t tc = 0, ncell = 0;
    for (int64_t iv = 0; iv < n_iv; iv++) {
        if (hm[iv].pad) { ctx->err = DP_ERR_CLUSTER; return MAUVE_ERR_HIP; }
        col_off[iv] = tc; tc += hm[iv].m; ncell += hm[iv].cells;
        if (score) score[iv] = hm[iv].score;
    }
    col_off[n_iv] = tc;
    if (cells) *cells = ncell;
    ctx->dp_last_col_off = d_col_off; ctx->dp_last_n = n_iv;
    if (tc) {
        HIPCHK(ctx, hipMemcpyAsync(d_col_off, col_off, (size_t)(n_iv + 1) * 8, hipMemcpyHostToDevice, ctx->stream));
        const uint32_t gblocks = (uint32_t)std::min<int64_t>((n_iv + 3) / 4, 256 * 8);
        hipLaunchKernelGGL(dp_gather, dim3(gblocks), dim3(256), 0, ctx->stream, nseq, n_iv, d_seq_off, ctx->dp_meta.as<DpMeta>(),
                           ctx->dp_prof_mask.as<uint32_t>(), ctx->dp_prof2_mask.as<uint32_t>(), d_col_off,
                           ctx->dp_cols.as<uint32_t>());
        HIPCHK(ctx, hipGetLastError());
        if (sp && nseq >= 2) {
            HIPCHK(ctx, ctx->dp_sp.ensure((size_t)n_iv * 8 + 64));
            HIPCHK(ctx, hipMemsetAsync(ctx->dp_sp.p, 0, (size_t)n_iv * 8, ctx->stream));
            hipLaunchKernelGGL(dp_sp_scores, dim3((uint32_t)std::min<int64_t>((n_iv + 3) / 4, 256 * 16)), dim3(256), 0, ctx->stream, nseq, n_iv, ctx->dp_codes.as<uint8_t>(), d_seq_off,
                               ctx->dp_cols.as<uint32_t>(), d_col_off, sc, ctx->dp_sp.as<unsigned long long>());
            HIPCHK(ctx, hipGetLastError());
            HIPCHK(ctx, hipMemcpyAsync(ctx->pin_meta.p, ctx->dp_sp.p, (size_t)n_iv * 8, hipMemcpyDeviceToHost, ctx->stream));
        }
        if (cols) HIPCHK(ctx, hipMemcpyAsync(cols, ctx->dp_cols.p, (size_t)tc * 4, hipMemcpyDeviceToHost, ctx->stream));
        HIPCHK(ctx, hipStreamSynchronize(ctx->stream));
        if (sp && nseq >= 2) memcpy(sp, ctx->pin_meta.p, (size_t)n_iv * 8);
    }
    if (sp && (!tc || nseq < 2)) for (int64_t iv = 0; iv < n_iv; iv++) sp[iv] = 0;
    if (trace) {
        std::vector<int64_t> e2(est); std::sort(e2.begin(), e2.end(), std::greater<int64_t>());
        fprintf(stderr, "[trace] dp_core: %d round(s); %lld intervals: %lld workgroup, %lld one-wave, %lld two/wave, %lld four/wave; single-wave steps: total %lld (balanced %lld), top", rounds, (long long)n_iv,
                (long long)n_big, (long long)cl.n_med, (long long)cl.n_s32, (long long)cl.n_s16, (long long)est_total, (long long)(est_total / 3072));
        for (size_t i = 0; i < e2.size() && i < 8; i++) fprintf(stderr, " %lld", (long long)e2[i]);
        fprintf(stderr, "\n");
    }
    if (trace) fprintf(stderr, "[trace] dp_core: sizing+H2D %.3f ms, order+launch %.3f, kernel+meta D2H %.3f, gather+cols D2H %.3f\n",
                       td1 - td0, td2 - td1, td3 - td2, now_ms() - td3);
    return MAUVE_OK;
}


namespace {
using namespace devscan;

struct DpFrontTotals {
    int64_t codes, tb, rows, est, n_dp, first_med, first_s32, first_s16, cols, cells, first_c, err;
    unsigned long long big_len;
};

__device__ __forceinline__ void dpf_gap(const int32_t *__restrict__ alen, const int32_t *__restrict__ ast, int N, uint32_t k, int g,
                                        int64_t &lo, int64_t &ln, bool &rev)
{
    const int64_t sa = ast[(size_t)k * N + g], sb = ast[(size_t)(k + 1) * N + g];
    int64_t hi;
    if (sa > 0) { lo = sa + alen[k]; hi = sb - 1; rev = false; }
    else { lo = -sb + alen[k + 1]; hi = -sa - 1; rev = true; }
    ln = hi - lo + 1; if (ln < 0) ln = 0;
}

__global__ void __launch_bounds__(256) dpf_gap_flags(const int32_t *__restrict__ alen, const int32_t *__restrict__ ast,
                                                     const int32_t *__restrict__ alcb, uint32_t na, int N, int gapped, int64_t max_gapped,
                                                     int32_t *__restrict__ gapcode, uint32_t *__restrict__ totals_words)
{
    const uint32_t k = blockIdx.x * 256u + threadIdx.x;
    if (k < 64) totals_words[k] = 0;
    if (k >= na) return;
    int32_t code = -1;
    if (k + 1 < na && alcb[k] == alcb[k + 1]) {
        int64_t tot = 0, mx = 0; int nonempty = 0;
        for (int g = 0; g < N; g++) {
            int64_t lo, ln; bool rv;
            dpf_gap(alen, ast, N, k, g, lo, ln, rv);
            tot += ln; mx = max(mx, ln); nonempty += ln > 0;
        }
        if (tot > 0) code = (gapped && nonempty >= 2 && mx <= max_gapped) ? 0 : -2;
    }
    gapcode[k] = code;
}
struct DpSlots {
    int32_t *gapcode; uint32_t na; uint32_t *anchor_of; DpFrontTotals *tot;
    __device__ uint32_t domain(int) const { return na; }
    __device__ bool flag(uint32_t k, int) const { return gapcode[k] == 0; }
    __device__ void each(uint32_t, uint32_t, bool, int) const {}
    __device__ void emit(uint32_t k, uint32_t o, int) const { gapcode[k] = (int32_t)o; anchor_of[o] = k; }
    __device__ void total(uint32_t n, int) const { tot->n_dp = n; }
};

struct DpSizingOut {
    int64_t *need, *rowsn, *est; uint8_t *cand, *cls; uint32_t *sizekey, *slotval;
    __device__ void put(uint32_t s, const DpSizing &z) const
    {
        need[s] = z.need; rowsn[s] = z.rows(); est[s] = z.est; cand[s] = z.cand(); cls[s] = z.cls();
        sizekey[s] = z.sizekey(); slotval[s] = s;
    }
};
__global__ void __launch_bounds__(256) dpf_desc(const int32_t *__restrict__ alen, const int32_t *__restrict__ ast, int N,
                                                const uint32_t *__restrict__ anchor_of, const DpFrontTotals *__restrict__ tot,
                                                DpSeqDesc *__restrict__ desc, DpSizingOut out, int no_mw, int no_groups, int64_t band_from, int class_mode)
{
    const uint32_t s = blockIdx.x * 256u + threadIdx.x;
    if (s >= (uint32_t)tot->n_dp) return;
    const uint32_t k = anchor_of[s];
    int64_t longest = 0;
    for (int g = 0; g < N; g++) {
        int64_t lo, n; bool rv;
        dpf_gap(alen, ast, N, k, g, lo, n, rv);
        longest = max(longest, n);
    }
    DpSizing z(band_from, no_mw, no_groups, class_mode, longest);
    for (int g = 0; g < N; g++) {
        int64_t lo, n; bool rv;
        dpf_gap(alen, ast, N, k, g, lo, n, rv);
        DpSeqDesc d; d.genome = g; d.rev = rv; d.lo0 = lo - 1; d.len = n;
        desc[(size_t)s * N + g] = d;
        z.add(n);
    }
    out.put(s, z);
}
__global__ void __launch_bounds__(256) dpf_size_desc(const DpSeqDesc *__restrict__ desc, int N, uint32_t n, DpFrontTotals *__restrict__ tot,
                                                     DpSizingOut out, int no_mw, int no_groups, int64_t band_from, int class_mode)
{
    const uint32_t s = blockIdx.x * 256u + threadIdx.x;
    if (s == 0) tot->n_dp = n;
    if (s >= n) return;
    int64_t longest = 0;
    for (int g = 0; g < N; g++) longest = max(longest, desc[(size_t)s * N + g].len);
    DpSizing z(band_from, no_mw, no_groups, class_mode, longest);
    for (int g = 0; g < N; g++) z.add(desc[(size_t)s * N + g].len);
    out.put(s, z);
}
struct DescLen { const DpSeqDesc *d; __device__ int64_t value(uint32_t i) const { return d[i].len; } };
struct ArrVal { const int64_t *a; __device__ int64_t value(uint32_t i) const { return a[i]; } };
struct ListVal { const int64_t *a; const uint32_t *order; __device__ int64_t value(uint32_t j) const { return a[order[j]]; } };
__global__ void __launch_bounds__(256) dpf_tb_scatter(const int64_t *__restrict__ tb_list, const uint32_t *__restrict__ order, uint32_t n, int64_t *__restrict__ tb_off)
{
    const uint32_t j = blockIdx.x * 256u + threadIdx.x;
    if (j < n) tb_off[order[j]] = tb_list[j];
}

struct DpBigPick {
    const uint32_t *order; const uint8_t *cand, *cls; const int64_t *est; const DpFrontTotals *tot; uint32_t *key2; int64_t wide_min; uint32_t maxn;
    __device__ uint32_t domain(int) const { return (uint32_t)tot->n_dp; }
    __device__ bool flag(uint32_t j, int) const { const uint32_t s = order[j]; return cand[s] == 1 && est[s] >= wide_min; }
    __device__ void each(uint32_t j, uint32_t before, bool fl, int) const { key2[j] = ((fl && before < maxn) || cand[order[j]] == 2) ? 0u : (uint32_t)cls[order[j]]; }
    __device__ void emit(uint32_t, uint32_t, int) const {}
    __device__ void total(uint32_t, int) const {}
};
__global__ void __launch_bounds__(256) dpf_list(const uint32_t *__restrict__ key2, const uint32_t *__restrict__ order, DpFrontTotals *__restrict__ tot,
                                                int64_t *__restrict__ list, const int64_t *__restrict__ seq_off, int N)
{
    const uint32_t n = (uint32_t)tot->n_dp, j = blockIdx.x * 256u + threadIdx.x;
    if (j < n) {
        const uint32_t s = order[j];
        list[j] = s;
        if (key2[j] == 0) atomicMax(&tot->big_len, (unsigned long long)(seq_off[((size_t)s + 1) * N] - seq_off[(size_t)s * N]));
    }
    if (j < 4) {
        uint32_t lo = 0, hi = n;
        while (lo < hi) { const uint32_t mid = (lo + hi) / 2; if (key2[mid] >= j + 1) hi = mid; else lo = mid + 1; }
        if (j == 0) tot->first_med = lo; else if (j == 1) tot->first_c = lo; else if (j == 2) tot->first_s32 = lo; else tot->first_s16 = lo;
    }
}
struct MetaCols { const DpMeta *m; __device__ int64_t value(uint32_t i) const { return m[i].m; } };
struct MetaCells { const DpMeta *m; __device__ int64_t value(uint32_t i) const { return m[i].cells; } };
__global__ void __launch_bounds__(256) dpf_scores(const DpMeta *__restrict__ meta, uint32_t n, int64_t *__restrict__ score, DpFrontTotals *__restrict__ tot)
{
    const uint32_t i = blockIdx.x * 256u + threadIdx.x;
    if (i < n) { score[i] = meta[i].score; if (meta[i].pad) tot->err = 1; }
}

}

struct DpFrontWork {
    DpSeqDesc *desc; DpFrontTotals *tot;
    int64_t *need, *rowsn, *est; uint8_t *cand, *cls;
    uint32_t *k1, *v1, *k2, *v2, *k3, *bcnt; int64_t *bsum, *bsum2;
    int64_t *d_seq_off, *d_tb_off, *d_rows_off, *d_col_off;
    DpSizingOut sizing() const { return DpSizingOut{need, rowsn, est, cand, cls, k1, v1}; }
};
static int dpf_work_area(mauve_ctx *ctx, uint32_t na, int N, DpFrontWork &W)
{
    const uint32_t nb = (na + TILE - 1) / TILE;
    auto up8 = [](size_t x) { return (x + 7) & ~(size_t)7; };
    const size_t o_cand = (size_t)na * 24, o_k = up8(o_cand + 2 * (size_t)na), o_bcnt = o_k + (size_t)na * 20, o_bsum = up8(o_bcnt + (size_t)nb * 4),
                 o_bsum2 = o_bsum + ((size_t)nb * N + 8) * 8, w_total = o_bsum2 + ((size_t)nb + 8) * 8;
    HIPCHK(ctx, ctx->dp_desc.ensure((size_t)na * N * sizeof(DpSeqDesc)));
    HIPCHK(ctx, ctx->dpf_work.ensure(w_total));
    HIPCHK(ctx, ctx->dp_off.ensure(((size_t)na * N + 1 + 3 * ((size_t)na + 1)) * sizeof(int64_t)));
    HIPCHK(ctx, ctx->dp_list.ensure((size_t)na * 8));
    HIPCHK(ctx, ctx->dp_meta.ensure((size_t)na * sizeof(DpMeta)));
    HIPCHK(ctx, ctx->dpf_tot.ensure(256));
    char *wk = ctx->dpf_work.as<char>();
    W.desc = ctx->dp_desc.as<DpSeqDesc>(); W.tot = ctx->dpf_tot.as<DpFrontTotals>();
    W.need = reinterpret_cast<int64_t *>(wk); W.rowsn = W.need + na; W.est = W.rowsn + na;
    W.cand = reinterpret_cast<uint8_t *>(wk + o_cand); W.cls = W.cand + na;
    W.k1 = reinterpret_cast<uint32_t *>(wk + o_k); W.v1 = W.k1 + na; W.k2 = W.v1 + na; W.v2 = W.k2 + na; W.k3 = W.v2 + na;
    W.bcnt = reinterpret_cast<uint32_t *>(wk + o_bcnt);
    W.bsum = reinterpret_cast<int64_t *>(wk + o_bsum); W.bsum2 = reinterpret_cast<int64_t *>(wk + o_bsum2);
    W.d_seq_off = ctx->dp_off.as<int64_t>();
    W.d_tb_off = W.d_seq_off + ((size_t)na * N + 1); W.d_rows_off = W.d_tb_off + (na + 1); W.d_col_off = W.d_rows_off + (na + 1);
    return MAUVE_OK;
}

struct DpFrontRun { int64_t n_big; DpClasses cl; int rounds; double t_sized; };
static int dpf_run(mauve_ctx *ctx, const DpFrontWork &W, int N, uint32_t n_dp, const DpScoring &sc, DpFrontTotals *ht, DpFrontRun &R)
{
    const uint32_t nbd = (n_dp + TILE - 1) / TILE, nbs = (n_dp * (uint32_t)N + TILE - 1) / TILE, blk_d = (n_dp + 255) / 256;
    DpFrontTotals *tot = W.tot;
    hipLaunchKernelGGL((vscan_partial<int64_t, DescLen>), dim3(nbs), dim3(256), 0, ctx->stream, DescLen{W.desc}, n_dp * (uint32_t)N, W.bsum);
    hipLaunchKernelGGL((vscan_write<int64_t, DescLen>), dim3(nbs), dim3(256), 0, ctx->stream, DescLen{W.desc}, n_dp * (uint32_t)N, W.bsum, W.d_seq_off, &tot->codes);
    hipLaunchKernelGGL((vscan_partial<int64_t, ArrVal>), dim3(nbd), dim3(256), 0, ctx->stream, ArrVal{W.rowsn}, n_dp, W.bsum);
    hipLaunchKernelGGL((vscan_write<int64_t, ArrVal>), dim3(nbd), dim3(256), 0, ctx->stream, ArrVal{W.rowsn}, n_dp, W.bsum, W.d_rows_off, &tot->rows);
    hipLaunchKernelGGL((vscan_partial<int64_t, ArrVal>), dim3(nbd), dim3(256), 0, ctx->stream, ArrVal{W.est}, n_dp, W.bsum2);
    hipLaunchKernelGGL((vscan_write<int64_t, ArrVal>), dim3(nbd), dim3(256), 0, ctx->stream, ArrVal{W.est}, n_dp, W.bsum2, W.d_col_off , &tot->est);
    uint32_t *ok = W.k1, *ov = W.v1;
    int rc = sort_pairs_u32(ctx, n_dp, 6, &ok, &ov, W.k2, W.v2, MAUVE_K_MISC);
    if (rc) return rc;
    uint32_t *fk = ok == W.k1 ? W.k2 : W.k1, *fv = ov == W.v1 ? W.v2 : W.v1;
    const DpBigPick bp{ov, W.cand, W.cls, W.est, tot, fk, dp_wide_min(), (uint32_t)dp_big_max()};
    hipLaunchKernelGGL((cmp_count<DpBigPick>), dim3(nbd), dim3(256), 0, ctx->stream, bp, W.bcnt);
    hipLaunchKernelGGL((cmp_write<DpBigPick>), dim3(nbd), dim3(256), 0, ctx->stream, bp, W.bcnt);
    uint32_t *ck = fk, *cv = ov;
    rc = sort_pairs_u32(ctx, n_dp, 3, &ck, &cv, W.k3, fv, MAUVE_K_MISC);
    if (rc) return rc;
    hipLaunchKernelGGL(dpf_list, dim3(blk_d), dim3(256), 0, ctx->stream, ck, cv, tot, ctx->dp_list.as<int64_t>(), W.d_seq_off, N);
    int64_t *tb_list_dev = W.d_col_off;
    hipLaunchKernelGGL((vscan_partial<int64_t, ListVal>), dim3(nbd), dim3(256), 0, ctx->stream, ListVal{W.need, cv}, n_dp, W.bsum2);
    hipLaunchKernelGGL((vscan_write<int64_t, ListVal>), dim3(nbd), dim3(256), 0, ctx->stream, ListVal{W.need, cv}, n_dp, W.bsum2, tb_list_dev, &tot->tb);
    hipLaunchKernelGGL(dpf_tb_scatter, dim3(blk_d), dim3(256), 0, ctx->stream, tb_list_dev, cv, n_dp, W.d_tb_off);
    HIPCHK(ctx, hipGetLastError());
    HIPCHK(ctx, hipMemcpyAsync(ht, tot, sizeof(DpFrontTotals), hipMemcpyDeviceToHost, ctx->stream));
    HIPCHK(ctx, hipStreamSynchronize(ctx->stream));
    const int64_t total = ht->codes, tbt = ht->tb, rwt = ht->rows;
    DpClasses &cl = R.cl; memset(&cl, 0, sizeof cl);
    R.n_big = ht->first_med;
    cl.first_med = ht->first_med; cl.n_med = ht->first_c - ht->first_med;
    cl.first_c = ht->first_c; cl.n_c = ht->first_s32 - ht->first_c;
    cl.first_s32 = ht->first_s32; cl.n_s32 = ht->first_s16 - ht->first_s32;
    cl.first_s16 = ht->first_s16; cl.n_s16 = (int64_t)n_dp - ht->first_s16;
    R.t_sized = now_ms();
    rc = dp_ensure_batch(ctx, total, tbt, rwt);
    if (rc) return rc;
    std::vector<int64_t> &tb_list = ctx->dph.tb_list; tb_list.clear();
    if (tbt > dp_tb_budget()) {
        tb_list.resize((size_t)n_dp + 1);
        HIPCHK(ctx, hipMemcpy(tb_list.data(), tb_list_dev, ((size_t)n_dp + 1) * 8, hipMemcpyDeviceToHost));
    }
    dp_launch_gather_codes(ctx, W.d_seq_off, (int64_t)n_dp * N);
    R.rounds = 1;
    rc = dp_launch_rounds(ctx, N, n_dp, R.n_big, (int64_t)ht->big_len, cl, W.d_seq_off, W.d_tb_off, W.d_rows_off, sc, tb_list.empty() ? nullptr : tb_list.data(), &R.rounds, ctx->dp_band_from);
    if (rc) return rc;
    const DpMeta *meta = ctx->dp_meta.as<DpMeta>();
    hipLaunchKernelGGL((vscan_partial<int64_t, MetaCols>), dim3(nbd), dim3(256), 0, ctx->stream, MetaCols{meta}, n_dp, W.bsum);
    hipLaunchKernelGGL((vscan_write<int64_t, MetaCols>), dim3(nbd), dim3(256), 0, ctx->stream, MetaCols{meta}, n_dp, W.bsum, W.d_col_off, &tot->cols);
    hipLaunchKernelGGL((vscan_partial<int64_t, MetaCells>), dim3(nbd), dim3(256), 0, ctx->stream, MetaCells{meta}, n_dp, W.bsum2);
    hipLaunchKernelGGL((vscan_write<int64_t, MetaCells>), dim3(nbd), dim3(256), 0, ctx->stream, MetaCells{meta}, n_dp, W.bsum2, W.rowsn , &tot->cells);
    hipLaunchKernelGGL(dpf_scores, dim3(blk_d), dim3(256), 0, ctx->stream, meta, n_dp, W.need, tot);
    const uint32_t gblocks = (uint32_t)std::min<int64_t>(((int64_t)n_dp + 3) / 4, 256 * 8);
    hipLaunchKernelGGL(dp_gather, dim3(gblocks), dim3(256), 0, ctx->stream, N, (int64_t)n_dp, W.d_seq_off, meta, ctx->dp_prof_mask.as<uint32_t>(),
                       ctx->dp_prof2_mask.as<uint32_t>(), W.d_col_off, ctx->dp_cols.as<uint32_t>());
    HIPCHK(ctx, hipGetLastError());
    return MAUVE_OK;
}

int dp_run_from_anchors(mauve_ctx *ctx, int N, int64_t na64, const int32_t *h_len, const int32_t *h_st, const int32_t *h_lcb, int gapped,
                        int64_t max_gapped_len, const mauve_scoring *scoring, int32_t *gapcode, int64_t *n_dp_out, int64_t *code_total_out,
                        PinnedBuf *dcols, std::vector<int64_t> &dcol_off, std::vector<int64_t> &dscore, int64_t *cells, int stay)
{
    const bool stay_on_device = stay != 0, anchors_in_place = stay == 1;
    static const bool trace = getenv("MAUVE_TRACE") != nullptr;
    static const bool no_mw = getenv("MAUVE_DP_ONE_WAVE") != nullptr, no_groups = getenv("MAUVE_DP_NO_GROUPS") != nullptr;
    const double t0 = now_ms();
    *n_dp_out = 0; *code_total_out = 0; if (cells) *cells = 0;
    dcol_off.assign(1, 0); dscore.clear();
    if (na64 < 2) { if (stay_on_device) { ctx->err = "dp: device tail needs two anchors"; return MAUVE_ERR_STATE; } for (int64_t k = 0; k < na64; k++) gapcode[k] = -1; return MAUVE_OK; }
    if (na64 >= (1LL << 31)) { ctx->err = "dp: too many anchors"; return MAUVE_ERR_LIMIT; }
    const uint32_t na = (uint32_t)na64, nb = (na + TILE - 1) / TILE, blocks = (na + 255) / 256;
    const size_t w_anch = (size_t)na * (2 + (size_t)N) * 4;
    HIPCHK(ctx, ctx->dpf_anch.ensure(w_anch + (size_t)na * 4 * 2 + 64));
    DpFrontWork W;
    int rc = dpf_work_area(ctx, na, N, W);
    if (rc) return rc;
    DpFrontTotals *tot = W.tot;
    int32_t *alen = ctx->dpf_anch.as<int32_t>(), *ast = alen + na, *alcb = ast + (size_t)na * N, *d_gapcode = alcb + na;
    uint32_t *anchor_of = reinterpret_cast<uint32_t *>(d_gapcode + na);
    if (anchors_in_place) {
        alen = const_cast<int32_t *>(h_len); ast = const_cast<int32_t *>(h_st); alcb = const_cast<int32_t *>(h_lcb);
    } else {
        HIPCHK(ctx, hipMemcpyAsync(alen, h_len, (size_t)na * 4, hipMemcpyHostToDevice, ctx->stream));
        HIPCHK(ctx, hipMemcpyAsync(ast, h_st, (size_t)na * N * 4, hipMemcpyHostToDevice, ctx->stream));
        HIPCHK(ctx, hipMemcpyAsync(alcb, h_lcb, (size_t)na * 4, hipMemcpyHostToDevice, ctx->stream));
    }
    hipLaunchKernelGGL(dpf_gap_flags, dim3(blocks), dim3(256), 0, ctx->stream, alen, ast, alcb, na, N, gapped, max_gapped_len, d_gapcode, reinterpret_cast<uint32_t *>(tot));
    const DpSlots sl{d_gapcode, na, anchor_of, tot};
    hipLaunchKernelGGL((cmp_count<DpSlots>), dim3(nb), dim3(256), 0, ctx->stream, sl, W.bcnt);
    hipLaunchKernelGGL((cmp_write<DpSlots>), dim3(nb), dim3(256), 0, ctx->stream, sl, W.bcnt);
    hipLaunchKernelGGL(dpf_desc, dim3(blocks), dim3(256), 0, ctx->stream, alen, ast, N, anchor_of, tot, W.desc, W.sizing(),
                       (int)no_mw, (int)no_groups, ctx->dp_band_from, dp_class_mode());
    HIPCHK(ctx, hipGetLastError());
    HIPCHK(ctx, ctx->pin_dp_in.ensure(256 + (size_t)na * 4));
    DpFrontTotals *ht = ctx->pin_dp_in.as<DpFrontTotals>();
    int32_t *h_gapcode = reinterpret_cast<int32_t *>(ctx->pin_dp_in.as<char>() + 256);
    HIPCHK(ctx, hipMemcpyAsync(ht, tot, sizeof(DpFrontTotals), hipMemcpyDeviceToHost, ctx->stream));
    if (!stay_on_device) HIPCHK(ctx, hipMemcpyAsync(h_gapcode, d_gapcode, (size_t)na * 4, hipMemcpyDeviceToHost, ctx->stream));
    HIPCHK(ctx, hipStreamSynchronize(ctx->stream));
    const uint32_t n_dp = (uint32_t)ht->n_dp;
    if (!stay_on_device) memcpy(gapcode, h_gapcode, (size_t)na * 4);
    *n_dp_out = n_dp;
    int64_t *d_col_off = W.d_col_off, *d_score = W.need;
    mauve_ctx::DpFrontOut &fo = ctx->dpf_out;
    fo.alen = alen; fo.ast = ast; fo.alcb = alcb; fo.gapcode = d_gapcode; fo.col_off = d_col_off; fo.score = d_score; fo.cols = nullptr; fo.n_dp = n_dp; fo.n_cols = 0;
    const double t1 = now_ms();
    if (n_dp == 0) return MAUVE_OK;
    DpFrontRun R;
    rc = dpf_run(ctx, W, N, n_dp, dp_scoring_of(scoring), ht, R);
    if (rc) return rc;
    *code_total_out = ht->codes;
    const double t2 = R.t_sized;
    if (ctx->shadow) { std::function<void()> f; f.swap(ctx->shadow); f(); }
    if (stay_on_device) {
        HIPCHK(ctx, hipMemcpyAsync(ht, tot, sizeof(DpFrontTotals), hipMemcpyDeviceToHost, ctx->stream));
        HIPCHK(ctx, hipStreamSynchronize(ctx->stream));
        if (ht->err) { ctx->err = DP_ERR_CLUSTER; return MAUVE_ERR_HIP; }
        if (cells) *cells = ht->cells;
        fo.cols = ctx->dp_cols.as<uint32_t>(); fo.n_cols = ht->cols;
        if (trace) fprintf(stderr, "[trace] dp (device front, results stay): %u intervals (%lld workgroup, %lld one-wave, %lld two/wave, %lld four/wave), %d round(s); gaps+slots %.3f ms, sizing+order %.3f, kernels+offsets %.3f\n",
                           n_dp, (long long)R.n_big, (long long)R.cl.n_med, (long long)R.cl.n_s32, (long long)R.cl.n_s16, R.rounds, t1 - t0, t2 - t1, now_ms() - t2);
        return MAUVE_OK;
    }
    dcol_off.resize((size_t)n_dp + 1); dscore.resize((size_t)n_dp);
    HIPCHK(ctx, ctx->pin_meta.ensure(((size_t)n_dp * 2 + 2) * 8));
    int64_t *p_off = ctx->pin_meta.as<int64_t>(), *p_score = p_off + n_dp + 1;
    HIPCHK(ctx, hipMemcpyAsync(ht, tot, sizeof(DpFrontTotals), hipMemcpyDeviceToHost, ctx->stream));
    HIPCHK(ctx, hipMemcpyAsync(p_off, d_col_off, ((size_t)n_dp + 1) * 8, hipMemcpyDeviceToHost, ctx->stream));
    HIPCHK(ctx, hipMemcpyAsync(p_score, d_score, (size_t)n_dp * 8, hipMemcpyDeviceToHost, ctx->stream));
    HIPCHK(ctx, hipStreamSynchronize(ctx->stream));
    const double t3 = now_ms();
    if (ht->err) { ctx->err = DP_ERR_CLUSTER; return MAUVE_ERR_HIP; }
    const int64_t tc = ht->cols;
    if (cells) *cells = ht->cells;
    memcpy(dcol_off.data(), p_off, ((size_t)n_dp + 1) * 8);
    memcpy(dscore.data(), p_score, (size_t)n_dp * 8);
    HIPCHK(ctx, dcols->ensure(((size_t)tc + 1) * 4));
    if (tc) {
        HIPCHK(ctx, hipMemcpyAsync(dcols->p, ctx->dp_cols.p, (size_t)tc * 4, hipMemcpyDeviceToHost, ctx->stream));
        HIPCHK(ctx, hipStreamSynchronize(ctx->stream));
    }
    if (trace) fprintf(stderr, "[trace] dp (device front): %u intervals (%lld workgroup, %lld one-wave, %lld two/wave, %lld four/wave), %d round(s); gaps+slots %.3f ms, sizing+order %.3f, kernels+offsets %.3f, columns %.3f\n",
                       n_dp, (long long)R.n_big, (long long)R.cl.n_med, (long long)R.cl.n_s32, (long long)R.cl.n_s16, R.rounds, t1 - t0, t2 - t1, t3 - t2, now_ms() - t3);
    return MAUVE_OK;
}

__global__ void __launch_bounds__(256) dpf_rotate_desc(DpSeqDesc *__restrict__ desc, int N, uint32_t n_orig, const int32_t *__restrict__ cbase)
{
    const uint32_t iv = blockIdx.x * 256u + threadIdx.x;
    if (iv >= n_orig) return;
    const int32_t c0 = cbase[iv], cnt = cbase[iv + 1] - c0;
    if (cnt <= 0) return;
    const DpSeqDesc *di = desc + (size_t)iv * N;
    int k = 0;
    for (int j = 0; j < N; j++) k += di[j].len != 0;
    DpSeqDesc none = di[0]; none.rev = 0; none.lo0 = 0; none.len = 0;
    for (int r = 1; r <= cnt; r++) {
        DpSeqDesc *o = desc + ((size_t)n_orig + (size_t)c0 + (size_t)(r - 1)) * N;
        int t = 0, filled = 0;
        for (int j = 0; j < N; j++) {
            if (!di[j].len) continue;
            const int slot = ((t - r) % k + k) % k;
            o[slot] = di[j]; t++; filled++;
        }
        for (int j = filled; j < N; j++) o[j] = none;
    }
}

int dp_run_from_desc(mauve_ctx *ctx, int N, int64_t n_iv, const DpSeqDesc *h_desc, const mauve_scoring *scoring, uint32_t *cols, int64_t *col_off, int64_t *score,
                     int64_t *cells, int64_t *sp, int64_t n_orig = -1, const int32_t *cbase = nullptr)
{
    static const bool trace = getenv("MAUVE_TRACE") != nullptr;
    static const bool no_mw = getenv("MAUVE_DP_ONE_WAVE") != nullptr, no_groups = getenv("MAUVE_DP_NO_GROUPS") != nullptr;
    const double t0 = now_ms();
    if (cells) *cells = 0;
    col_off[0] = 0;
    if (n_iv == 0) return MAUVE_OK;
    if (n_iv >= (1LL << 31) / std::max(N, 1)) { ctx->err = "dp: too many intervals"; return MAUVE_ERR_LIMIT; }
    const uint32_t n_dp = (uint32_t)n_iv;
    DpFrontWork W;
    int rc = dpf_work_area(ctx, n_dp, N, W);
    if (rc) return rc;
    DpSeqDesc *desc = W.desc;
    DpFrontTotals *tot = W.tot;
    const bool rot = cbase != nullptr && n_orig >= 0 && n_orig < n_iv;
    const size_t rows_up = rot ? (size_t)n_orig : (size_t)n_dp;
    const size_t desc_bytes = rows_up * N * sizeof(DpSeqDesc), cb_bytes = rot ? ((size_t)n_orig + 1) * 4 : 0;
    HIPCHK(ctx, ctx->pin_dp_in.ensure(256 + desc_bytes + cb_bytes + 64));
    DpFrontTotals *ht = ctx->pin_dp_in.as<DpFrontTotals>();
    memcpy(ctx->pin_dp_in.as<char>() + 256, h_desc, desc_bytes);
    HIPCHK(ctx, hipMemcpyAsync(desc, ctx->pin_dp_in.as<char>() + 256, desc_bytes, hipMemcpyHostToDevice, ctx->stream));
    if (rot) {
        if ((int64_t)cbase[n_orig] != n_iv - n_orig) { ctx->err = "dp: the rotation table does not match the batch"; return MAUVE_ERR_ARG; }
        char *pcb = ctx->pin_dp_in.as<char>() + 256 + ((desc_bytes + 7) & ~(size_t)7);
        memcpy(pcb, cbase, cb_bytes);
        int32_t *d_cb = reinterpret_cast<int32_t *>(W.k1);
        HIPCHK(ctx, hipMemcpyAsync(d_cb, pcb, cb_bytes, hipMemcpyHostToDevice, ctx->stream));
        hipLaunchKernelGGL(dpf_rotate_desc, dim3((uint32_t)((n_orig + 255) / 256)), dim3(256), 0, ctx->stream, desc, N, (uint32_t)n_orig, d_cb);
    }
    HIPCHK(ctx, hipMemsetAsync(tot, 0, 256, ctx->stream));
    hipLaunchKernelGGL(dpf_size_desc, dim3((n_dp + 255) / 256), dim3(256), 0, ctx->stream, desc, N, n_dp, tot, W.sizing(), (int)no_mw, (int)no_groups,
                       ctx->dp_band_from, dp_class_mode());
    const DpScoring sc = dp_scoring_of(scoring);
    DpFrontRun R;
    rc = dpf_run(ctx, W, N, n_dp, sc, ht, R);
    if (rc) return rc;
    int64_t *d_col_off = W.d_col_off, *d_score = W.need;
    HIPCHK(ctx, ctx->pin_meta.ensure(((size_t)n_dp * 3 + 2) * 8));
    int64_t *p_off = ctx->pin_meta.as<int64_t>(), *p_score = p_off + n_dp + 1, *p_sp = p_score + n_dp;
    if (sp && N >= 2) {
        HIPCHK(ctx, ctx->dp_sp.ensure((size_t)n_dp * 8 + 64));
        hipLaunchKernelGGL(dp_sp_scores, dim3((uint32_t)std::min<int64_t>(((int64_t)n_dp + 3) / 4, 256 * 16)), dim3(256), 0, ctx->stream, N, (int64_t)n_dp, ctx->dp_codes.as<uint8_t>(), W.d_seq_off,
                           ctx->dp_cols.as<uint32_t>(), d_col_off, sc, ctx->dp_sp.as<unsigned long long>());
        HIPCHK(ctx, hipGetLastError());
        HIPCHK(ctx, hipMemcpyAsync(p_sp, ctx->dp_sp.p, (size_t)n_dp * 8, hipMemcpyDeviceToHost, ctx->stream));
    }
    HIPCHK(ctx, hipMemcpyAsync(ht, tot, sizeof(DpFrontTotals), hipMemcpyDeviceToHost, ctx->stream));
    HIPCHK(ctx, hipMemcpyAsync(p_off, d_col_off, ((size_t)n_dp + 1) * 8, hipMemcpyDeviceToHost, ctx->stream));
    HIPCHK(ctx, hipMemcpyAsync(p_score, d_score, (size_t)n_dp * 8, hipMemcpyDeviceToHost, ctx->stream));
    HIPCHK(ctx, hipStreamSynchronize(ctx->stream));
    if (ht->err) { ctx->err = DP_ERR_CLUSTER; return MAUVE_ERR_HIP; }
    const int64_t tc = ht->cols;
    if (cells) *cells = ht->cells;
    memcpy(col_off, p_off, ((size_t)n_dp + 1) * 8);
    if (score) memcpy(score, p_score, (size_t)n_dp * 8);
    if (sp) { if (N >= 2) memcpy(sp, p_sp, (size_t)n_dp * 8); else memset(sp, 0, (size_t)n_dp * 8); }
    ctx->dp_last_col_off = d_col_off; ctx->dp_last_n = n_dp;
    if (cols && tc) {
        if (host_pointer_is_pinned(cols)) HIPCHK(ctx, hipMemcpyAsync(cols, ctx->dp_cols.p, (size_t)tc * 4, hipMemcpyDeviceToHost, ctx->stream));
        else HIPCHK(ctx, hipMemcpy(cols, ctx->dp_cols.p, (size_t)tc * 4, hipMemcpyDeviceToHost));
        HIPCHK(ctx, hipStreamSynchronize(ctx->stream));
    }
    if (trace) fprintf(stderr, "[trace] dp (descriptor batch, device front): %u intervals (%lld workgroup, %lld one-wave, %lld two/wave, %lld four/wave), %d round(s); upload+sizing+order %.3f ms, kernels+results %.3f\n",
                       n_dp, (long long)R.n_big, (long long)R.cl.n_med, (long long)R.cl.n_s32, (long long)R.cl.n_s16, R.rounds, R.t_sized - t0, now_ms() - R.t_sized);
    return MAUVE_OK;
}

__global__ void __launch_bounds__(256) dp_pick_cols(const uint32_t *__restrict__ cols, const int64_t *__restrict__ col_off, const int64_t *__restrict__ pick,
                                                    const int64_t *__restrict__ out_off, int64_t n_pick, uint32_t *__restrict__ out)
{
    const int lane = threadIdx.x & 63;
    const int64_t wave = ((int64_t)blockIdx.x * 256 + threadIdx.x) >> 6, nw = ((int64_t)gridDim.x * 256) >> 6;
    for (int64_t q = wave; q < n_pick; q += nw) {
        const int64_t iv = pick[q], a = col_off[iv], n = col_off[iv + 1] - a, o = out_off[q];
        for (int64_t c = lane; c < n; c += 64) out[o + c] = cols[a + c];
    }
}

int dp_fetch_picked(mauve_ctx *ctx, int64_t n_pick, const int64_t *pick, const int64_t *col_off, uint32_t *out, int64_t *out_off)
{
    out_off[0] = 0;
    for (int64_t q = 0; q < n_pick; q++) {
        if (pick[q] < 0 || pick[q] >= ctx->dp_last_n) { ctx->err = "dp_fetch_picked: interval outside the last batch"; return MAUVE_ERR_ARG; }
        out_off[q + 1] = out_off[q] + (col_off[pick[q] + 1] - col_off[pick[q]]);
    }
    const int64_t total = out_off[n_pick];
    if (!total) return MAUVE_OK;
    HIPCHK(ctx, ctx->dp_pick.ensure((size_t)(2 * n_pick + 1) * 8 + (size_t)total * 4 + 64));
    HIPCHK(ctx, ctx->pin_dp_in.ensure((size_t)(2 * n_pick + 1) * 8));
    int64_t *hp = ctx->pin_dp_in.as<int64_t>();
    memcpy(hp, pick, (size_t)n_pick * 8); memcpy(hp + n_pick, out_off, (size_t)(n_pick + 1) * 8);
    int64_t *d_pick = ctx->dp_pick.as<int64_t>(), *d_off = d_pick + n_pick;
    uint32_t *d_out = reinterpret_cast<uint32_t *>(d_off + n_pick + 1);
    HIPCHK(ctx, hipMemcpyAsync(d_pick, hp, (size_t)(2 * n_pick + 1) * 8, hipMemcpyHostToDevice, ctx->stream));
    hipLaunchKernelGGL(dp_pick_cols, dim3((uint32_t)std::min<int64_t>((n_pick + 3) / 4, 256 * 8)), dim3(256), 0, ctx->stream, ctx->dp_cols.as<uint32_t>(), ctx->dp_last_col_off, d_pick,
                       d_off, n_pick, d_out);
    HIPCHK(ctx, hipGetLastError());
    HIPCHK(ctx, hipMemcpyAsync(out, d_out, (size_t)total * 4, hipMemcpyDeviceToHost, ctx->stream));
    HIPCHK(ctx, hipStreamSynchronize(ctx->stream));
    return MAUVE_OK;
}

int dp_batch_run(mauve_ctx *ctx, int nseq, int64_t n_iv, const uint8_t *codes, const int64_t *seq_off,
                 const mauve_scoring *scoring, uint32_t *cols, int64_t *col_off, int64_t *score, int64_t *cells)
{
    return dp_core(ctx, nseq, n_iv, codes, nullptr, seq_off, scoring, cols, col_off, score, cells);
}

static bool dp_desc_host() { static const bool h = getenv("MAUVE_DP_DESC_HOST") != nullptr; return h; }
static int64_t dp_desc_min() { static const int64_t m = getenv("MAUVE_DP_DESC_MIN") ? atoll(getenv("MAUVE_DP_DESC_MIN")) : 2048; return m; }
bool dp_desc_rotations_on_device(int64_t n_total) { return !dp_desc_host() && n_total >= dp_desc_min(); }
int dp_batch_run_desc_rot(mauve_ctx *ctx, int nseq, int64_t n_orig, const DpSeqDesc *desc, const int32_t *cbase, int64_t n_total, const mauve_scoring *scoring,
                          int64_t *col_off, int64_t *score, int64_t *cells, int64_t *sp)
{
    if (!dp_desc_rotations_on_device(n_total)) { ctx->err = "dp: rotations on the device need the device front"; return MAUVE_ERR_STATE; }
    return dp_run_from_desc(ctx, nseq, n_total, desc, scoring, nullptr, col_off, score, cells, sp, n_orig, cbase);
}
int dp_batch_run_desc(mauve_ctx *ctx, int nseq, int64_t n_iv, const DpSeqDesc *desc, const mauve_scoring *scoring,
                      uint32_t *cols, int64_t *col_off, int64_t *score, int64_t *cells, bool may_shard, int64_t *sp)
{
    std::vector<int64_t> &seq_off = ctx->dph.seq_off;
    if (may_shard && ctx->shard_on && n_iv >= 2 * ctx->shard_world) {
        std::vector<int64_t> cost((size_t)n_iv);
        for (int64_t k = 0; k < n_iv; k++) {
            int64_t m = 0, cl = 0;
            for (int g = 0; g < nseq; g++) { const int64_t n = desc[k * nseq + g].len; if (!n) continue; if (!m) { m = n; continue; } cl += m * n; m += n; }
            cost[(size_t)k] = cl;
        }
        std::vector<int> owner; shard_lpt(cost, ctx->shard_world, owner);
        std::vector<int64_t> mine;
        for (int64_t k = 0; k < n_iv; k++) if (owner[(size_t)k] == ctx->shard_rank) mine.push_back(k);
        const int64_t nmine = (int64_t)mine.size();
        std::vector<DpSeqDesc> sub((size_t)nmine * nseq);
        int64_t cap = 0;
        for (int64_t q = 0; q < nmine; q++)
            for (int g = 0; g < nseq; g++) { sub[(size_t)(q * nseq + g)] = desc[mine[(size_t)q] * nseq + g]; cap += desc[mine[(size_t)q] * nseq + g].len; }
        std::vector<uint32_t> mcols((size_t)cap + 1); std::vector<int64_t> moff((size_t)nmine + 1, 0), mscore((size_t)nmine + 1, 0), msp((size_t)nmine + 1, 0);
        int64_t mcells = 0;
        seq_off.resize((size_t)(nmine * nseq + 1));
        { int64_t t = 0; for (int64_t i = 0; i < nmine * nseq; i++) { seq_off[(size_t)i] = t; t += sub[(size_t)i].len; } seq_off[(size_t)(nmine * nseq)] = t; }
        const int rc_local = dp_core(ctx, nseq, nmine, nullptr, sub.data(), seq_off.data(), scoring, mcols.data(), moff.data(), mscore.data(), &mcells, sp ? msp.data() : nullptr);
        const int64_t ncol = rc_local ? 0 : moff[(size_t)nmine];
        std::vector<char> msg(rc_local ? 16 : (size_t)(2 + 3 * nmine) * 8 + (size_t)ncol * 4);
        int64_t *h = reinterpret_cast<int64_t *>(msg.data());
        if (rc_local) { h[0] = -1; h[1] = rc_local; }
        else {
            h[0] = nmine; h[1] = mcells;
            for (int64_t q = 0; q < nmine; q++) { h[2 + q] = moff[(size_t)q + 1] - moff[(size_t)q]; h[2 + nmine + q] = mscore[(size_t)q]; h[2 + 2 * nmine + q] = msp[(size_t)q]; }
            if (ncol) memcpy(msg.data() + (size_t)(2 + 3 * nmine) * 8, mcols.data(), (size_t)ncol * 4);
        }
        std::vector<std::pair<const char *, size_t>> parts;
        const std::string err_local = ctx->err;
        int rc = shard_allgather(ctx, msg.data(), msg.size(), parts);
        if (rc) return rc;
        if (rc_local) { ctx->err = err_local; return rc_local; }
        for (int r = 0; r < ctx->shard_world; r++)
            if (parts[(size_t)r].second >= 16 && reinterpret_cast<const int64_t *>(parts[(size_t)r].first)[0] == -1) {
                ctx->err = "dp shard: rank " + std::to_string(r) + " failed (status " + std::to_string(reinterpret_cast<const int64_t *>(parts[(size_t)r].first)[1]) + ")";
                return MAUVE_ERR_STATE;
            }
        std::vector<int64_t> len_of((size_t)n_iv, 0);
        std::vector<std::vector<int64_t>> ids((size_t)ctx->shard_world);
        for (int64_t k = 0; k < n_iv; k++) ids[(size_t)owner[(size_t)k]].push_back(k);
        int64_t total_cells = 0;
        for (int r = 0; r < ctx->shard_world; r++) {
            const int64_t *hr = reinterpret_cast<const int64_t *>(parts[(size_t)r].first);
            if (parts[(size_t)r].second < 16 || hr[0] != (int64_t)ids[(size_t)r].size()) { ctx->err = "dp shard: ranks disagree about the interval table"; return MAUVE_ERR_STATE; }
            total_cells += hr[1];
            {
                const size_t nr = ids[(size_t)r].size();
                if (parts[(size_t)r].second < (2 + 3 * nr) * 8) { ctx->err = "dp shard: a rank's part is shorter than its header"; return MAUVE_ERR_STATE; }
                int64_t sum = 0; bool neg = false;
                for (size_t q = 0; q < nr; q++) { neg |= hr[2 + q] < 0; sum += hr[2 + q]; }
                if (neg || parts[(size_t)r].second != (2 + 3 * nr) * 8 + (size_t)sum * 4) { ctx->err = "dp shard: a rank's part does not hold the columns it announces"; return MAUVE_ERR_STATE; }
            }
            for (size_t q = 0; q < ids[(size_t)r].size(); q++) { len_of[(size_t)ids[(size_t)r][q]] = hr[2 + q]; if (score) score[ids[(size_t)r][q]] = hr[2 + ids[(size_t)r].size() + q]; if (sp) sp[ids[(size_t)r][q]] = hr[2 + 2 * ids[(size_t)r].size() + q]; }
        }
        col_off[0] = 0;
        for (int64_t k = 0; k < n_iv; k++) col_off[k + 1] = col_off[k] + len_of[(size_t)k];
        for (int r = 0; r < ctx->shard_world; r++) {
            const int64_t nr = (int64_t)ids[(size_t)r].size();
            const uint32_t *cr = reinterpret_cast<const uint32_t *>(parts[(size_t)r].first + (size_t)(2 + 3 * nr) * 8);
            for (int64_t q = 0; q < nr; q++) {
                const int64_t k = ids[(size_t)r][(size_t)q];
                memcpy(cols + col_off[k], cr, (size_t)len_of[(size_t)k] * 4);
                cr += len_of[(size_t)k];
            }
        }
// ... 37 lines not shown
```

mauvealigner_amd/csrc/pipeline.cpp:

```cpp
#include "common.hpp"
#include <algorithm>
#include <cstdlib>
#include <cstring>

namespace {

inline uint8_t base_at(const uint64_t *w, int64_t i) { return (uint8_t)((w[(size_t)(i >> 5)] >> (2 * (i & 31))) & 3); }

}

int recursive_anchoring(mauve_ctx *c, const mauve_params *p, int w0, std::vector<MatchVec> &chains, int N, const int *gmap);

static int extend_lcbs(mauve_ctx *c, const mauve_params *p, int w, int64_t lcbw, MatchVec &m, std::vector<int64_t> &match_lcb,
                       int64_t &nl)
{
    const int N = m.N;
    const uint32_t full = full_mask(N);
    int w_e = w;
    MatchVec base(N); ChainOrders base_ord; bool have_base = false;
    for (int iter = 0; iter < p->max_extension_iters; iter++) {
        w_e -= 2;
        if (w_e < 5) break;
        const uint64_t pe = mauve_get_seed(w_e, 0);
        if (!pe) break;
// ... 482 lines not shown
    const double ta2 = now_ms();
    if (!S.anchor_table_done) fill_anchor_table(c);
    {
        uint32_t *out = R.cols.data();
        R.cols_dirty.assign((size_t)S.n_anchor, std::pair<size_t, size_t>(0, 0));
        c->pool->parallel_for(S.n_anchor, 1024, [&](int64_t ab, int64_t ae) {
            for (int64_t a = ab; a < ae; a++) {
                const Item &it = items[(size_t)a];
                const MatchVec &ch = chains[(size_t)it.lcb];
                const int64_t alen = ch.len(it.idx);
                uint32_t *o = out + it.col0 + alen;
                if (it.gap >= 0) {
                    const GapRef &gr = S.gaps[(size_t)it.gap];
                    const size_t glen = (size_t)(gr.dp ? dcol_off[(size_t)gr.dp_slot + 1] - dcol_off[(size_t)gr.dp_slot] : gr.tot);
                    R.cols_dirty[(size_t)a] = {(size_t)(o - out), glen};
                    if (gr.dp) std::copy(dcols + dcol_off[(size_t)gr.dp_slot], dcols + dcol_off[(size_t)gr.dp_slot + 1], o);
                    else for (int g = 0; g < N; g++) {
                        int64_t lo, ln;
                        gap_of(ch.rec(it.idx), ch.rec(it.idx + 1), g, lo, ln);
                        std::fill(o, o + ln, 1u << g); o += ln;
                    }
                }
            }
        });
    }
    const double ta3 = now_ms();
    size_t ncols = (size_t)col;
    int64_t niv = nl;
    R.iv_left.assign((size_t)nl * N, 0); R.iv_right.assign((size_t)nl * N, 0); R.iv_reverse.assign((size_t)nl * N, 0);
    for (int64_t i = 0; i < nl * N; i++) {
        R.iv_left[(size_t)i] = std::llabs(R.lcb_left[(size_t)i]);
        R.iv_right[(size_t)i] = std::llabs(R.lcb_right[(size_t)i]);
        R.iv_reverse[(size_t)i] = R.lcb_left[(size_t)i] < 0;
    }
    if (p->add_unaligned) {
        for (int g = 0; g < N; g++) {
            std::vector<std::pair<int64_t, int64_t>> sp;
            for (int64_t l = 0; l < nl; l++) if (R.iv_left[(size_t)l * N + g]) sp.push_back({R.iv_left[(size_t)l * N + g], R.iv_right[(size_t)l * N + g]});
            std::sort(sp.begin(), sp.end());
            int64_t cur = 1;
            for (size_t i = 0; i <= sp.size(); i++) {
                int64_t lo = cur, hi = i < sp.size() ? sp[i].first - 1 : c->lens[g];
                if (hi >= lo) {
                    R.col_off.push_back((int64_t)ncols);
                    std::fill(R.cols.begin() + ncols, R.cols.begin() + ncols + (size_t)(hi - lo + 1), 1u << g);
                    R.cols_dirty.push_back({ncols, (size_t)(hi - lo + 1)});
                    ncols += (size_t)(hi - lo + 1);
                    for (int h = 0; h < N; h++) { R.iv_left.push_back(h == g ? lo : 0); R.iv_right.push_back(h == g ? hi : 0); R.iv_reverse.push_back(0); }
                    R.dp_score.push_back(0);
                    niv++;
                }
                if (i < sp.size() && sp[i].second + 1 > cur) cur = sp[i].second + 1;
            }
        }
    }
    R.col_off.push_back((int64_t)ncols);
    R.n_cols = ncols;
    R.sz.n_mums = S.nm; R.sz.n_lcb = nl; R.sz.n_anchor = S.n_anchor; R.sz.n_iv = niv; R.sz.n_cols = (int64_t)ncols;
    R.sz.n_gap_dp = n_dp; R.sz.n_dp_cells = cells;
    *sizes = R.sz;
    const double t5 = now_ms();
    if (g_trace_pipeline) fprintf(stderr, "[trace] assemble: layout %.3f ms, restore %.3f, anchors+gaps %.3f, unaligned+sizes %.3f\n", ta1 - t4, ta2 - ta1, ta3 - ta2, t5 - ta3);
    c->stage.assemble_ms = t5 - t4;
    c->stage.total_ms = t5 - S.t0;
    S.open = false;
    return MAUVE_OK;
}

static int align_begin_lcbs(mauve_ctx *c, const mauve_params *p, std::vector<MatchVec> &lcbs)
{
    const int N = c->nseq;
    AlignState &S = c->ast;
    S.reset();
    c->rec_flags.clear();
    S.p = *p; S.N = N; S.t0 = now_ms();
    AlignResult &R = c->res;
    result_reset(R);
    memset(&c->stage, 0, sizeof c->stage);
    c->shadow = nullptr;
    int64_t sum = 0; for (int g = 0; g < N; g++) sum += c->lens[g];
    S.sum = sum;
    int w;
    (void)resolve_seed(c, p, sum / N, "align_lcbs", &w, nullptr);
    S.full = full_mask(N);
    S.nm = 0; S.nl = (int64_t)lcbs.size();
    S.chains.swap(lcbs);
    R.lcb_weight.assign((size_t)S.nl, 0);
    for (int64_t l = 0; l < S.nl; l++) for (size_t i = 0; i < S.chains[(size_t)l].size(); i++) R.lcb_weight[(size_t)l] += S.chains[(size_t)l].len(i) * N;
    const double t2 = now_ms();
    if (p->recursive) { const int rc = recursive_anchoring(c, p, w, S.chains, N, nullptr); if (rc) return rc; }
    c->stage.recurse_ms = now_ms() - t2;
    S.count_anchors();
    S.t_dp0 = now_ms();
    S.open = true;
    return MAUVE_OK;
}

static int align_dp_finish(mauve_ctx *c, mauve_align_sizes *sizes, bool shadow)
{
    AlignState &S = c->ast;
    HIPCHK(c, c->pin_dcols.ensure(((size_t)S.code_total + 1) * sizeof(uint32_t)));
    uint32_t *dcols = c->pin_dcols.as<uint32_t>();
    S.dcol_off.assign((size_t)S.n_dp + 1, 0); S.dscore.assign((size_t)S.n_dp + 1, 0);
    int64_t cells = 0;
    if (shadow && S.n_dp) c->shadow = [c]() { fill_anchor_table(c); };
    const int rc = align_dp(c, nullptr, S.n_dp, dcols, S.dcol_off.data(), S.dscore.data(), &cells);
    c->shadow = nullptr;
    if (rc) return rc;
    return align_finish(c, dcols, S.dcol_off.data(), S.dscore.data(), cells, sizes);
}

static int kept_mums_to_host(mauve_ctx *c)
{
    AlignState &S = c->ast; AlignResult &R = c->res;
    if (S.mums_kept < 0) return MAUVE_OK;
    std::swap(c->sorted_rec, c->sorted_rec_keep);
    const size_t n = (size_t)S.mums_kept, N = (size_t)S.N;
    S.mums_kept = -1;
    HIPCHK(c, c->pin_tab.ensure(n * (1 + N) * 8 + 64));
    if (n) HIPCHK(c, hipMemcpy(c->pin_tab.p, c->sorted_rec.p, n * (1 + N) * 8, hipMemcpyDeviceToHost));
    const int64_t *hm = c->pin_tab.as<int64_t>();
    R.mum_length.assign(hm, hm + n); R.mum_start.assign(hm + n, hm + n * (1 + N));
    return MAUVE_OK;
}

static int align_tail_host_chains(mauve_ctx *c, mauve_align_sizes *sizes)
{
    AlignState &S = c->ast;
    static const bool no_shadow = getenv("MAUVE_NO_SHADOW") != nullptr;
    int64_t cells = 0;
    int rc;
    const int N = S.N; const int64_t na = S.n_anchor;
    HIPCHK(c, c->pin_anch.ensure((size_t)na * (3 + (size_t)N) * 4 + 64));
    int32_t *h_len = c->pin_anch.as<int32_t>(), *h_st = h_len + na, *h_lcb = h_st + (size_t)na * N, *gapcode = h_lcb + na;
    {
        size_t a = 0;
        for (int64_t l = 0; l < S.nl; l++) {
            const MatchVec &ch = S.chains[(size_t)l];
            for (size_t i = 0; i < ch.size(); i++, a++) {
                const int64_t *r = ch.rec(i);
                h_len[a] = (int32_t)r[0]; h_lcb[a] = (int32_t)l;
                for (int g = 0; g < N; g++) h_st[a * N + g] = (int32_t)r[1 + g];
            }
        }
    }
    if (!no_shadow && na) c->shadow = [c]() { fill_anchor_table(c); };
    c->dp_band_from = dp_band_from_of(&S.p);
    static const bool host_tail = getenv("MAUVE_HOST_TAIL") != nullptr;
    if (!host_tail && na >= 2) {
        rc = dp_run_from_anchors(c, N, na, h_len, h_st, h_lcb, S.p.gapped, dp_len_limit(&S.p), &S.p.scoring, nullptr, &S.n_dp, &S.code_total,
                                 nullptr, S.dcol_off, S.dscore, &cells, 2);
        if (c->shadow) { std::function<void()> f; f.swap(c->shadow); f(); }
        if (rc) return rc;
        return assemble_device(c, na, cells, sizes, true);
    }
    { const int rck = kept_mums_to_host(c); if (rck) return rck; }
    rc = dp_run_from_anchors(c, N, na, h_len, h_st, h_lcb, S.p.gapped, dp_len_limit(&S.p), &S.p.scoring, gapcode, &S.n_dp, &S.code_total,
                             &c->pin_dcols, S.dcol_off, S.dscore, &cells);
    c->shadow = nullptr;
    if (rc) return rc;
    {
        size_t a = 0;
        for (int64_t l = 0; l < S.nl; l++) {
            const MatchVec &ch = S.chains[(size_t)l];
            for (size_t i = 0; i < ch.size(); i++, a++) {
                const int32_t code = gapcode[a];
                if (code == -1) continue;
                GapRef gr{l, (int64_t)i, code >= 0, code >= 0 ? code : -1, 0};
                if (!gr.dp)
                    for (int g = 0; g < N; g++) { int64_t lo, ln; gap_of(ch.rec(i), ch.rec(i + 1), g, lo, ln); gr.tot += ln; }
                S.gaps.push_back(gr);
            }
        }
    }
    S.dscore.push_back(0);
    return align_finish(c, c->pin_dcols.as<uint32_t>(), S.dcol_off.data(), S.dscore.data(), cells, sizes);
}

extern "C" {

int mauve_align_prefetch(mauve_ctx *c, int32_t *mum_length, int32_t *mum_start, int64_t mum_cap, int32_t *anchor_length, int32_t *anchor_start,
                         int32_t *anchor_lcb, int64_t anchor_cap)
{
    if (!c) return MAUVE_ERR_ARG;
    mauve_ctx::TablePrefetch &P = c->pf;
    if (mum_cap > 0 && anchor_cap > 0 && P.mum_length && P.anchor_length && mum_length == P.mum_length && mum_start == P.mum_start && mum_cap == P.mum_cap &&
        anchor_length == P.anchor_length && anchor_start == P.anchor_start && anchor_lcb == P.anchor_lcb && anchor_cap == P.anchor_cap) { P.armed = true; return MAUVE_OK; }
    HIPCHK(c, hipSetDevice(c->device));
    const bool m = mum_cap > 0 && host_pointer_is_pinned(mum_length) && host_pointer_is_pinned(mum_start);
    const bool a = anchor_cap > 0 && host_pointer_is_pinned(anchor_length) && host_pointer_is_pinned(anchor_start) && host_pointer_is_pinned(anchor_lcb);
    P.mum_length = m ? mum_length : nullptr; P.mum_start = m ? mum_start : nullptr; P.mum_cap = m ? mum_cap : 0;
    P.anchor_length = a ? anchor_length : nullptr; P.anchor_start = a ? anchor_start : nullptr; P.anchor_lcb = a ? anchor_lcb : nullptr; P.anchor_cap = a ? anchor_cap : 0;
    P.armed = m || a;
    return MAUVE_OK;
}

static int align_whole(mauve_ctx *c, const mauve_params *p, mauve_align_sizes *sizes);

int mauve_align(mauve_ctx *c, const mauve_params *p, mauve_align_sizes *sizes)
{
    if (!c || !p || !sizes) return MAUVE_ERR_ARG;
    mauve_ctx::TablePrefetch &P = c->pf;
    P.live = P.armed; P.armed = false;
    const int rc = align_whole(c, p, sizes);
    P.live = false;
    if (P.inflight) {
        (void)hipStreamSynchronize(c->stream_io);
        P.inflight = false; P.got_mums = P.got_anchors = false;
    }
    return rc;
}

static int align_whole(mauve_ctx *c, const mauve_params *p, mauve_align_sizes *sizes)
{
    { const int rg = refuse_past_2g(c, "align"); if (rg) return rg; }
    { const int rs = refuse_scoring_params(c, p, "align"); if (rs) return rs; }
    if (c->nseq < 2) { c->err = "align: at least two genomes required"; return MAUVE_ERR_STATE; }
    HIPCHK(c, hipSetDevice(c->device));
    static const bool host_front = getenv("MAUVE_HOST_DP_FRONT") != nullptr;
    static const bool no_shadow = getenv("MAUVE_NO_SHADOW") != nullptr;
    int rc = align_begin(c, p, !host_front, nullptr, !host_front);
    if (rc) return rc;
    AlignState &S = c->ast;
    int64_t cells = 0;
    if (S.dev_tail) {
        const int32_t *d_len = S.dv_len, *d_st = S.dv_st, *d_lcb = S.dv_lcb;
        c->dp_band_from = dp_band_from_of(&S.p);
        int rc_pf = MAUVE_OK;
        if (c->pf.live) { const int N = S.N; const int64_t na = S.n_anchor; c->shadow = [=, &rc_pf]() { rc_pf = prefetch_tables_enqueue(c, N, na, d_len, d_st, d_lcb); }; }
        rc = dp_run_from_anchors(c, S.N, S.n_anchor, d_len, d_st, d_lcb, S.p.gapped, dp_len_limit(&S.p), &S.p.scoring, nullptr, &S.n_dp, &S.code_total,
                                 nullptr, S.dcol_off, S.dscore, &cells, 1);
        if (c->shadow) { std::function<void()> f; f.swap(c->shadow); if (!rc) f(); }
        if (rc || rc_pf) return rc ? rc : rc_pf;
        return assemble_device(c, S.n_anchor, cells, sizes);
    }
    if (host_front) return align_dp_finish(c, sizes, !no_shadow);
    return align_tail_host_chains(c, sizes);
}

int mauve_align_lcbs(mauve_ctx *c, const mauve_params *p, int64_t n, const int64_t *length, const int64_t *start, const int64_t *lcb, mauve_align_sizes *sizes)
{
    if (!c || !p || !sizes) return MAUVE_ERR_ARG;
    { const int rg = refuse_past_2g(c, "align_lcbs"); if (rg) return rg; }
    { const int rs = refuse_scoring_params(c, p, "align_lcbs"); if (rs) return rs; }
    if (c->nseq < 2) { c->err = "align_lcbs: at least two genomes required"; return MAUVE_ERR_STATE; }
    if (n < 0 || (n && (!length || !start || !lcb))) { c->err = "align_lcbs: bad anchor list"; return MAUVE_ERR_ARG; }
    HIPCHK(c, hipSetDevice(c->device));
    { int rcm = materialize_tables(c); if (rcm) return rcm; }
    const int N = c->nseq;
    int64_t nl = 0;
    for (int64_t i = 0; i < n; i++) {
        if (lcb[i] < 0 || lcb[i] >= n) { c->err = "align_lcbs: LCB ids must be 0 .. n_lcb-1"; return MAUVE_ERR_ARG; }
        nl = std::max(nl, lcb[i] + 1);
        if (length[i] <= 0) { c->err = "align_lcbs: anchor of length <= 0"; return MAUVE_ERR_ARG; }
        for (int g = 0; g < N; g++) {
            const int64_t s = start[i * N + g];
            if (!s) { c->err = "align_lcbs: anchors have a component in every genome"; return MAUVE_ERR_ARG; }
            if (std::llabs(s) + length[i] - 1 > c->lens[(size_t)g]) { c->err = "align_lcbs: anchor outside its genome"; return MAUVE_ERR_ARG; }
        }
        if (start[i * N] < 0) { c->err = "align_lcbs: anchors are forward in genome 0 (Match::Invert them first)"; return MAUVE_ERR_ARG; }
    }
    std::vector<MatchVec> chains((size_t)nl, MatchVec(N));
    for (int64_t i = 0; i < n; i++) chains[(size_t)lcb[i]].push(length[i], start + i * N);
    for (int64_t l = 0; l < nl; l++) {
        MatchVec &ch = chains[(size_t)l];
        if (ch.empty()) { c->err = "align_lcbs: an LCB id without anchors"; return MAUVE_ERR_ARG; }
        ch.sort_by_start0();
        for (size_t i = 0; i + 1 < ch.size(); i++)
            for (int g = 0; g < N; g++) {
                const int64_t a = ch.st(i)[g], b = ch.st(i + 1)[g];
                const bool ok = (a > 0) == (b > 0) && (a > 0 ? a + ch.len(i) <= b : -b + ch.len(i + 1) <= -a);
                if (!ok) { c->err = "align_lcbs: the anchors of an LCB must be collinear and free of overlaps"; return MAUVE_ERR_ARG; }
            }
    }
    int rc = align_begin_lcbs(c, p, chains);
    if (rc) return rc;
    return align_tail_host_chains(c, sizes);
}

static int given_matches(mauve_ctx *c, int64_t n, const int64_t *length, const int64_t *start, MatchVec &mv)
{
    if (n < 0 || (n && (!length || !start))) { c->err = "align_matches: bad match list"; return MAUVE_ERR_ARG; }
    mv.N = c->nseq; mv.resize((size_t)n);
    for (int64_t i = 0; i < n; i++) {
        if (length[i] <= 0) { c->err = "align_matches: match of length <= 0"; return MAUVE_ERR_ARG; }
        mv.len((size_t)i) = length[i];
        for (int g = 0; g < c->nseq; g++) {
            const int64_t s = start[i * c->nseq + g];
            if (s && std::llabs(s) + length[i] - 1 > c->lens[(size_t)g]) { c->err = "align_matches: match outside its genome"; return MAUVE_ERR_ARG; }
            mv.st((size_t)i)[g] = s;
        }
    }
    return MAUVE_OK;
}

int mauve_match_sp_scores(mauve_ctx *c, int64_t n, const int64_t *length, const int64_t *start, const mauve_scoring *sc, int64_t *scores)
{
    if (!c || !sc || n < 0 || (n && (!length || !start || !scores))) return MAUVE_ERR_ARG;
    { const int rg = refuse_past_2g(c, "match_sp_scores"); if (rg) return rg; }
    { const int rs = refuse_scoring(c, sc, "match_sp_scores"); if (rs) return rs; }
    if (c->nseq < 2) { c->err = "match_sp_scores: at least two genomes required"; return MAUVE_ERR_STATE; }
    HIPCHK(c, hipSetDevice(c->device));
    const int N = c->nseq;
    MatchVec m(N); m.resize((size_t)n);
    for (int64_t i = 0; i < n; i++) { m.len((size_t)i) = length[i]; std::copy(start + i * N, start + (i + 1) * N, m.st((size_t)i)); }
    std::vector<int64_t> out;
    int rc = match_sp_scores(c, m, nullptr, sc, out);
    if (rc) return rc;
    std::copy(out.begin(), out.end(), scores);
    return MAUVE_OK;
}

int mauve_match_sp_scores_repeat(mauve_ctx *c, uint64_t pattern, int mode, int64_t n, const int64_t *length, const int64_t *start,
                                 const mauve_scoring *sc, int64_t *scores)
{
    if (!c || !sc || n < 0 || (n && (!length || !start || !scores))) return MAUVE_ERR_ARG;
    { const int rg = refuse_past_2g(c, "match_sp_scores_repeat"); if (rg) return rg; }
    { const int rs = refuse_scoring(c, sc, "match_sp_scores_repeat"); if (rs) return rs; }
    if (mode != MAUVE_REPEAT_PENALTY_OFF && mode != MAUVE_REPEAT_PENALTY_NEGATIVE && mode != MAUVE_REPEAT_PENALTY_ZERO) { c->err = "match_sp_scores_repeat: unknown mode"; return MAUVE_ERR_ARG; }
    SeedShape sh;
    if (!make_seed_shape(pattern, &sh)) { c->err = "seed pattern must be palindromic, span <= 49, weight <= 31"; return MAUVE_ERR_ARG; }
    if (mode == MAUVE_REPEAT_PENALTY_OFF) return mauve_match_sp_scores(c, n, length, start, sc, scores);
    if (c->nseq < 2) { c->err = "match_sp_scores: at least two genomes required"; return MAUVE_ERR_STATE; }
    HIPCHK(c, hipSetDevice(c->device));
    { int rcm = materialize_tables(c); if (rcm) return rcm; }
    int rc = repeat_multiplicity(c, pattern);
    if (rc) return rc;
    RepeatScope rp_scope(c);
    c->rp_now = mode;
    return mauve_match_sp_scores(c, n, length, start, sc, scores);
}

int mauve_align_matches(mauve_ctx *c, const mauve_params *p, int64_t n, const int64_t *length, const int64_t *start, mauve_align_sizes *sizes)
{
    if (!c || !p || !sizes) return MAUVE_ERR_ARG;
    { const int rg = refuse_past_2g(c, "align_matches"); if (rg) return rg; }
    { const int rs = refuse_scoring_params(c, p, "align_matches"); if (rs) return rs; }
    if (c->nseq < 2) { c->err = "align: at least two genomes required"; return MAUVE_ERR_STATE; }
    HIPCHK(c, hipSetDevice(c->device));
    MatchVec mv;
    int rc = given_matches(c, n, length, start, mv);
    if (rc) return rc;
    rc = align_begin(c, p, false, &mv);
    if (rc) return rc;
    return align_dp_finish(c, sizes, false);
}

int mauve_align_begin_matches(mauve_ctx *c, const mauve_params *p, int64_t n, const int64_t *length, const int64_t *start, int64_t *n_dp,
                              int64_t *n_codes)
{
    if (!c || !p || !n_dp) return MAUVE_ERR_ARG;
    { const int rg = refuse_past_2g(c, "align_begin_matches"); if (rg) return rg; }
    { const int rs = refuse_scoring_params(c, p, "align_begin_matches"); if (rs) return rs; }
    if (c->nseq < 2) { c->err = "align: at least two genomes required"; return MAUVE_ERR_STATE; }
    HIPCHK(c, hipSetDevice(c->device));
    MatchVec mv;
    int rc = given_matches(c, n, length, start, mv);
    if (rc) return rc;
    rc = align_begin(c, p, false, &mv);
    if (rc) return rc;
    *n_dp = c->ast.n_dp;
    if (n_codes) *n_codes = c->ast.code_total;
    return MAUVE_OK;
}

int mauve_align_dp_anchors(mauve_ctx *c, int64_t *left, int64_t *right)
{
    if (!c || !c->ast.open) { if (c) c->err = "align_dp_anchors: no alignment in progress"; return c ? MAUVE_ERR_STATE : MAUVE_ERR_ARG; }
    const AlignState &S = c->ast;
    const int N = S.N;
    for (const GapRef &gr : S.gaps) {
        if (!gr.dp) continue;
        const MatchVec &ch = S.chains[(size_t)gr.lcb];
        if (left) std::copy(ch.rec((size_t)gr.idx), ch.rec((size_t)gr.idx) + 1 + N, left + gr.dp_slot * (1 + N));
        if (right) std::copy(ch.rec((size_t)gr.idx + 1), ch.rec((size_t)gr.idx + 1) + 1 + N, right + gr.dp_slot * (1 + N));
    }
    return MAUVE_OK;
}

int mauve_align_begin(mauve_ctx *c, const mauve_params *p, int64_t *n_dp, int64_t *n_codes)
{
    if (!c || !p || !n_dp) return MAUVE_ERR_ARG;
    { const int rg = refuse_past_2g(c, "align_begin"); if (rg) return rg; }
    { const int rs = refuse_scoring_params(c, p, "align_begin"); if (rs) return rs; }
    if (c->nseq < 2) { c->err = "align: at least two genomes required"; return MAUVE_ERR_STATE; }
    HIPCHK(c, hipSetDevice(c->device));
    int rc = align_begin(c, p);
// ... 152 lines not shown
```

Before: 10240 Mbp/s.

## Remove host syncs from DP front and build unaligned islands on device

Removes the host round-trip that read the DP interval count and gapcodes before launching DP rounds; the DP front now runs with a device-side count and defers error and cell-count checks to the final assembly sync. The unaligned-island table is built on device with a single-block bitonic sort and wave prefix sweep, and islands are filled by kernel instead of being computed on the host afterwards. Two scans are also merged into one multi-value scan, and a device wall-clock stamp is subtracted from the DP stage time. This trades host stalls for extra single-block kernels and a more complex error path.

Result: no change. 10270 Mbp/s (median of 2 runs) (+0.3%).

```diff
diff --git a/mauvealigner_amd/csrc/assemble_dev.hip b/mauvealigner_amd/csrc/assemble_dev.hip
--- a/mauvealigner_amd/csrc/assemble_dev.hip
+++ b/mauvealigner_amd/csrc/assemble_dev.hip
@@ -1,5 +1,6 @@
 #include "common.hpp"
 #include "dev_scan.hpp"
+#include "island_sweep.hpp"
 #include <cstring>
 #include <cstdlib>
 #include <algorithm>
@@ -18,7 +19,15 @@
 }
 
 struct AsWidth {
-    const int32_t *alen, *ast, *gapcode; const int64_t *dcol_off; int N;
+    const int32_t *alen, *ast, *gapcode; const int64_t *dcol_off; int N; const int64_t *err;
+    unsigned long long *lcb_score; uint32_t nl;
+    int64_t *stamp;
+    __device__ bool live() const { return *err == 0; }
+    __device__ void open(uint32_t t, uint32_t nt) const
+    {
+        for (uint32_t l = t; l < nl; l += nt) lcb_score[l] = 0;
+        if (t == 0) { stamp[0] = (int64_t)wall_clock64(); stamp[2] = 0; }
+    }
     __device__ int64_t value(uint32_t a) const
     {
         int64_t w = alen[a];
@@ -29,10 +38,21 @@
     }
 };
 
+__device__ __forceinline__ void as_stamp_end(int64_t *stamp)
+{
+    if (!stamp) return;
+    __syncthreads();
+    if (threadIdx.x == 0) {
+        __threadfence();
+        if (atomicAdd(reinterpret_cast<unsigned long long *>(stamp + 2), 1ull) + 1ull == (unsigned long long)gridDim.x) stamp[1] = (int64_t)wall_clock64();
+    }
+}
+
 __global__ void __launch_bounds__(256) as_lcb(const int32_t *__restrict__ alcb, const int32_t *__restrict__ gapcode, const int64_t *__restrict__ dscore,
                                               const int64_t *__restrict__ col0, uint32_t na, uint32_t *__restrict__ first_a, uint32_t *__restrict__ last_a,
-                                              int64_t *__restrict__ lcb_col, unsigned long long *__restrict__ lcb_score)
-{
+                                              int64_t *__restrict__ lcb_col, unsigned long long *__restrict__ lcb_score, const int64_t *__restrict__ err)
+{
+    if (*err) return;
     const uint32_t a = blockIdx.x * 256u + threadIdx.x;
     const bool in = a < na;
     const int32_t l = in ? alcb[a] : 0;
@@ -47,8 +67,9 @@
                                                   const uint32_t *__restrict__ first_a, const uint32_t *__restrict__ last_a,
                                                   int64_t *__restrict__ left, int64_t *__restrict__ right,
                                                   const unsigned long long *__restrict__ lw, int64_t *__restrict__ lw_row,
-                                                  const int64_t *__restrict__ total_cols, int64_t *__restrict__ total_row)
-{
+                                                  const int64_t *__restrict__ total_cols, int64_t *__restrict__ total_row, const int64_t *__restrict__ err)
+{
+    if (*err) return;
     const uint32_t t = blockIdx.x * 256u + threadIdx.x;
     if (t >= nl * (uint32_t)N) return;
     const uint32_t l = t / (uint32_t)N; const int g = (int)(t % (uint32_t)N);
@@ -64,8 +85,10 @@
 
 __global__ void __launch_bounds__(256) as_fill(const int32_t *__restrict__ alen, const int32_t *__restrict__ ast, const int32_t *__restrict__ gapcode,
                                                const int64_t *__restrict__ dcol_off, const uint32_t *__restrict__ dcols,
-                                               const int64_t *__restrict__ col0, uint32_t na, int N, uint32_t full, uint32_t *__restrict__ out)
-{
+                                               const int64_t *__restrict__ col0, uint32_t na, int N, uint32_t full, uint32_t *__restrict__ out,
+                                               const int64_t *__restrict__ err, int64_t *stamp)
+{
+    if (*err) return;
     const int lane = threadIdx.x & 63;
     const uint32_t wave = (blockIdx.x * 256u + threadIdx.x) >> 6, nw = (gridDim.x * 256u) >> 6;
     for (uint32_t a = wave; a < na; a += nw) {
@@ -85,15 +108,109 @@
             }
         }
     }
+    as_stamp_end(stamp);
 }
 
 struct Island { int64_t col, len; uint32_t bit, pad; };
-__global__ void __launch_bounds__(256) as_islands(const Island *__restrict__ isl, uint32_t n, uint32_t *__restrict__ out)
-{
+__global__ void __launch_bounds__(256) as_islands(const Island *__restrict__ isl, uint32_t n, const int64_t *__restrict__ n_dev, uint32_t *__restrict__ out,
+                                                  const int64_t *__restrict__ err, int64_t *stamp)
+{
+    if (*err) return;
+    if (n_dev) n = (uint32_t)*n_dev;
     for (uint32_t k = blockIdx.x; k < n; k += gridDim.x) {
         const Island is = isl[k];
         uint32_t *o = out + is.col;
         for (int64_t c = threadIdx.x; c < is.len; c += 256) o[c] = is.bit;
+    }
+    as_stamp_end(stamp);
+}
+
+constexpr int ISL_WAVES = 16;
+constexpr uint32_t ISL_LDS_EXTENTS = 4096;
+struct IslandLens { int64_t len[MAUVE_MAX_SEQ]; };
+
+__device__ __forceinline__ void isl_wave_sweep(const IslandExtent *ext, uint32_t n, int64_t glen, int64_t col0, uint32_t idx0, uint32_t bit,
+                                               Island *__restrict__ isl, bool write, int64_t *cols, uint32_t *cnt)
+{
+    const int lane = threadIdx.x & 63;
+    int64_t carry = 0, col = col0; uint32_t idx = idx0;
+    for (uint32_t c = 0; c <= n; c += 64) {
+        const uint32_t i = c + lane;
+        const bool active = i <= n;
+        int64_t m = active && i >= 1 ? ext[i - 1].right : 0;
+#pragma unroll
+        for (int o = 1; o < 64; o <<= 1) { const int64_t t = __shfl_up(m, o); if (lane >= o) m = max(m, t); }
+        m = max(m, carry);
+        int64_t lo = 0, len = 0;
+        if (active) len = island_gap(m, i < n ? ext[i].left : glen + 1, &lo);
+        if (len < 0) len = 0;
+        int64_t inc = len;
+#pragma unroll
+        for (int o = 1; o < 64; o <<= 1) { const int64_t t = __shfl_up(inc, o); if (lane >= o) inc += t; }
+        const uint64_t fl = __ballot(len > 0);
+        if (write && len > 0) {
+            Island is; is.col = col + inc - len; is.len = len; is.bit = bit; is.pad = 0;
+            isl[idx + (uint32_t)__popcll(fl & ((1ull << lane) - 1ull))] = is;
+        }
+        col += __shfl(inc, 63); idx += (uint32_t)__popcll(fl); carry = __shfl(m, 63);
+    }
+    *cols = col - col0; *cnt = idx - idx0;
+}
+
+__global__ void __launch_bounds__(64 * ISL_WAVES) as_island_table(const int64_t *__restrict__ left, const int64_t *__restrict__ right, uint32_t nl, int N, uint32_t P,
+                                                                  IslandLens G, const int64_t *__restrict__ lcb_cols, int64_t col_limit,
+                                                                  Island *__restrict__ isl, int64_t *__restrict__ isl_row, const int64_t *__restrict__ err)
+{
+    __shared__ IslandExtent ext[ISL_LDS_EXTENTS];
+    __shared__ int64_t g_cols[MAUVE_MAX_SEQ];
+    __shared__ uint32_t g_cnt[MAUVE_MAX_SEQ], g_n[MAUVE_MAX_SEQ];
+    if (*err) return;
+    const int lane = threadIdx.x & 63, wave = threadIdx.x >> 6, nw = blockDim.x >> 6;
+    for (int g = wave; g < N; g += nw) {
+        IslandExtent *e = ext + (size_t)g * P;
+        uint32_t n = 0;
+        for (uint32_t i0 = 0; i0 < P; i0 += 64) {
+            const uint32_t i = i0 + lane;
+            const int64_t l = i < nl ? left[(size_t)i * N + g] : 0;
+            if (i < P) {
+                IslandExtent x; x.left = INT64_MAX; x.right = INT64_MAX;
+                if (l != 0) { const int64_t r = right[(size_t)i * N + g]; x.left = l < 0 ? -l : l; x.right = r < 0 ? -r : r; }
+                e[i] = x;
+            }
+            n += (uint32_t)__popcll(__ballot(l != 0));
+        }
+        if (lane == 0) g_n[g] = n;
+    }
+    __syncthreads();
+    for (uint32_t k = 2; k <= P; k <<= 1)
+        for (uint32_t j = k >> 1; j > 0; j >>= 1) {
+            for (int g = wave; g < N; g += nw) {
+                IslandExtent *e = ext + (size_t)g * P;
+                for (uint32_t t = lane; t < P / 2; t += 64) {
+                    const uint32_t i = ((t & ~(j - 1)) << 1) | (t & (j - 1)), x = i | j;
+                    const bool up = (i & k) == 0;
+                    const IslandExtent a = e[i], b = e[x];
+                    if ((b < a) == up) { e[i] = b; e[x] = a; }
+                }
+            }
+            __syncthreads();
+        }
+    for (int g = wave; g < N; g += nw) {
+        int64_t cols; uint32_t cnt;
+        isl_wave_sweep(ext + (size_t)g * P, g_n[g], G.len[g], 0, 0, 1u << g, isl, false, &cols, &cnt);
+        if (lane == 0) { g_cols[g] = cols; g_cnt[g] = cnt; }
+    }
+    __syncthreads();
+    int64_t all = *lcb_cols; uint32_t n_all = 0;
+    for (int h = 0; h < N; h++) { all += g_cols[h]; n_all += g_cnt[h]; }
+    const bool fits = all <= col_limit;
+    if (threadIdx.x == 0) { isl_row[0] = fits ? (int64_t)n_all : 0; isl_row[1] = all; }
+    if (!fits) return;
+    for (int g = wave; g < N; g += nw) {
+        int64_t col0 = *lcb_cols; uint32_t idx0 = 0;
+        for (int h = 0; h < g; h++) { col0 += g_cols[h]; idx0 += g_cnt[h]; }
+        int64_t cols; uint32_t cnt;
+        isl_wave_sweep(ext + (size_t)g * P, g_n[g], G.len[g], col0, idx0, 1u << g, isl, true, &cols, &cnt);
     }
 }
 
@@ -194,19 +311,18 @@
     return MAUVE_OK;
 }
 
-int assemble_device(mauve_ctx *c, int64_t na64, int64_t cells, mauve_align_sizes *sizes, bool host_chains)
+int assemble_device(mauve_ctx *c, int64_t na64, mauve_align_sizes *sizes, bool host_chains)
 {
     static const bool trace = getenv("MAUVE_TRACE") != nullptr;
     AlignState &S = c->ast; AlignResult &R = c->res;
     const int N = S.N; const int64_t nl = S.nl; const uint32_t na = (uint32_t)na64;
     const mauve_ctx::DpFrontOut &fo = c->dpf_out;
     const double t0 = now_ms();
-    c->stage.dp_ms = t0 - S.t_dp0;
     const uint32_t nb = (na + TILE - 1) / TILE, blocks = (na + 255) / 256;
     auto up8 = [](size_t x) { return (x + 7) & ~(size_t)7; };
     const size_t o_bsum = ((size_t)na + 1) * 8, o_first = o_bsum + ((size_t)nb + 8) * 8, o_last = up8(o_first + (size_t)nl * 4),
                  o_col = up8(o_last + (size_t)nl * 4), o_left = o_col + ((size_t)nl + 1) * 8, o_right = o_left + (size_t)nl * N * 8,
-                 o_score = o_right + (size_t)nl * N * 8, o_lw = o_score + (size_t)nl * 8, o_tot = o_lw + (size_t)nl * 8, w_total = o_tot + 8;
+                 o_score = o_right + (size_t)nl * N * 8, o_lw = o_score + (size_t)nl * 8, o_tot = o_lw + (size_t)nl * 8, o_isl = o_tot + 8, o_stamp = o_isl + 16, w_total = o_stamp + 24;
     HIPCHK(c, c->as_work.ensure(w_total + 64));
     HIPCHK(c, c->res_cols.ensure(((size_t)S.sum + 64) * 4));
     char *wk = c->as_work.as<char>();
@@ -215,24 +331,40 @@
     int64_t *lcb_col = reinterpret_cast<int64_t *>(wk + o_col), *left = reinterpret_cast<int64_t *>(wk + o_left),
             *right = reinterpret_cast<int64_t *>(wk + o_right);
     unsigned long long *score = reinterpret_cast<unsigned long long *>(wk + o_score);
-    int64_t *lw_row = reinterpret_cast<int64_t *>(wk + o_lw), *tot_row = reinterpret_cast<int64_t *>(wk + o_tot);
+    int64_t *lw_row = reinterpret_cast<int64_t *>(wk + o_lw), *tot_row = reinterpret_cast<int64_t *>(wk + o_tot), *isl_row = reinterpret_cast<int64_t *>(wk + o_isl),
+            *stamp = reinterpret_cast<int64_t *>(wk + o_stamp);
     uint32_t *out = c->res_cols.as<uint32_t>();
-    HIPCHK(c, hipMemsetAsync(score, 0, (size_t)nl * 8, c->stream));
-    const AsWidth wf{fo.alen, fo.ast, fo.gapcode, fo.col_off, N};
+    static const bool isl_host = getenv("MAUVE_AS_ISL_HOST") != nullptr;
+    static const int64_t isl_max = []() { const char *e = getenv("MAUVE_AS_ISL_MAX"); return e ? (int64_t)atoll(e) : (int64_t)ISL_LDS_EXTENTS; }();
+    uint32_t isl_p = 1;
+    while ((int64_t)isl_p < nl) isl_p <<= 1;
+    const bool isl_dev = S.p.add_unaligned && !isl_host && nl >= 1 && nl <= isl_max && (size_t)isl_p * N <= ISL_LDS_EXTENTS;
+    if (isl_dev) HIPCHK(c, c->as_isl.ensure((size_t)N * ((size_t)nl + 1) * sizeof(Island) + 64));
+    const AsWidth wf{fo.alen, fo.ast, fo.gapcode, fo.col_off, N, fo.d_err, score, (uint32_t)nl, stamp};
     hipLaunchKernelGGL((vscan_partial<int64_t, AsWidth>), dim3(nb), dim3(256), 0, c->stream, wf, na, bsum);
     hipLaunchKernelGGL((vscan_write<int64_t, AsWidth>), dim3(nb), dim3(256), 0, c->stream, wf, na, bsum, col0, (int64_t *)nullptr);
-    hipLaunchKernelGGL(as_lcb, dim3(blocks), dim3(256), 0, c->stream, fo.alcb, fo.gapcode, fo.score, col0, na, first_a, last_a, lcb_col, score);
+    hipLaunchKernelGGL(as_lcb, dim3(blocks), dim3(256), 0, c->stream, fo.alcb, fo.gapcode, fo.score, col0, na, first_a, last_a, lcb_col, score, fo.d_err);
     hipLaunchKernelGGL(as_extents, dim3(((uint32_t)nl * N + 255) / 256), dim3(256), 0, c->stream, fo.alen, fo.ast, N, (uint32_t)nl, first_a, last_a, left, right,
-                       host_chains ? (const unsigned long long *)nullptr : c->ch_lw.as<unsigned long long>(), lw_row, col0 + na, tot_row);
+                       host_chains ? (const unsigned long long *)nullptr : c->ch_lw.as<unsigned long long>(), lw_row, col0 + na, tot_row, fo.d_err);
     HIPCHK(c, hipGetLastError());
-    const size_t rows_bytes = ((size_t)nl + 1) * 8 + 2 * (size_t)nl * N * 8 + 2 * (size_t)nl * 8 + 8;
+    const uint32_t isl_grid = (uint32_t)std::min<size_t>((size_t)N * ((size_t)nl + 1), 1024);
+    if (isl_dev) {
+        IslandLens G; memset(&G, 0, sizeof G);
+        for (int g = 0; g < N; g++) G.len[g] = c->lens[(size_t)g];
+        hipLaunchKernelGGL(as_island_table, dim3(1), dim3(64u * (uint32_t)std::min(N, ISL_WAVES)), 0, c->stream, left, right, (uint32_t)nl, N, isl_p, G, tot_row, S.sum,
+                           c->as_isl.as<Island>(), isl_row, fo.d_err);
+    }
+    {
+        const uint32_t fb = (uint32_t)std::min<int64_t>(((int64_t)na + 3) / 4, 256 * 8);
+        hipLaunchKernelGGL(as_fill, dim3(fb), dim3(256), 0, c->stream, fo.alen, fo.ast, fo.gapcode, fo.col_off, fo.cols, col0, na, N, S.full, out, fo.d_err,
+                           isl_dev ? (int64_t *)nullptr : stamp);
+    }
+    if (isl_dev)
+        hipLaunchKernelGGL(as_islands, dim3(isl_grid), dim3(256), 0, c->stream, c->as_isl.as<Island>(), 0u, isl_row, out, fo.d_err, stamp);
+    const size_t rows_bytes = ((size_t)nl + 1) * 8 + 2 * (size_t)nl * N * 8 + 2 * (size_t)nl * 8 + 8 + 16 + 24;
     HIPCHK(c, c->pin_asm.ensure(64 + rows_bytes));
     int64_t *h_rows = c->pin_asm.as<int64_t>() + 8;
     HIPCHK(c, hipMemcpyAsync(h_rows, lcb_col, rows_bytes, hipMemcpyDeviceToHost, c->stream));
-    {
-        const uint32_t fb = (uint32_t)std::min<int64_t>(((int64_t)na + 3) / 4, 256 * 8);
-        hipLaunchKernelGGL(as_fill, dim3(fb), dim3(256), 0, c->stream, fo.alen, fo.ast, fo.gapcode, fo.col_off, fo.cols, col0, na, N, S.full, out);
-    }
     R.dev_nm = !host_chains && c->matches_pending ? (size_t)c->n_matches : 0;
     if (S.mums_kept >= 0) {
         std::swap(c->sorted_rec, c->sorted_rec_keep);
@@ -244,6 +376,12 @@
     HIPCHK(c, hipStreamSynchronize(c->stream));
     c->pf.inflight = false;
     const double t1 = now_ms();
+    if (fo.h_err && *fo.h_err) { c->err = dp_cluster_error(); return MAUVE_ERR_HIP; }
+    const int64_t cells = fo.h_cells ? *fo.h_cells : 0;
+    const int64_t *h_stamp = h_rows + (rows_bytes / 8 - 3);
+    static const double ticks_per_ms = [&]() { int khz = 0; return hipDeviceGetAttribute(&khz, hipDeviceAttributeWallClockRate, c->device) == hipSuccess && khz > 0 ? (double)khz : 1e5; }();
+    const double tail_ms = h_stamp[1] > h_stamp[0] ? (double)(h_stamp[1] - h_stamp[0]) / ticks_per_ms : 0.0;
+    c->stage.dp_ms = std::max(0.0, t1 - S.t_dp0 - tail_ms);
     const int64_t *h_col = h_rows, *h_left = h_col + nl + 1, *h_right = h_left + nl * N, *h_score = h_right + nl * N, *h_lw = h_score + nl;
     const int64_t lcb_cols = h_lw[nl];
     R.col_off.assign(h_col, h_col + nl);
@@ -259,27 +397,24 @@
     int64_t ncols = lcb_cols, niv = nl;
     if (S.p.add_unaligned) {
         std::vector<Island> isl;
+        std::vector<IslandExtent> sp;
         for (int g = 0; g < N; g++) {
-            std::vector<std::pair<int64_t, int64_t>> sp;
+            sp.clear();
             for (int64_t l = 0; l < nl; l++) if (R.iv_left[(size_t)l * N + g]) sp.push_back({R.iv_left[(size_t)l * N + g], R.iv_right[(size_t)l * N + g]});
             std::sort(sp.begin(), sp.end());
-            int64_t cur = 1;
-            for (size_t i = 0; i <= sp.size(); i++) {
-                const int64_t lo = cur, hi = i < sp.size() ? sp[i].first - 1 : c->lens[(size_t)g];
-                if (hi >= lo) {
-                    R.col_off.push_back(ncols);
-                    Island is; is.col = ncols; is.len = hi - lo + 1; is.bit = 1u << g; is.pad = 0;
-                    isl.push_back(is);
-                    ncols += hi - lo + 1;
-                    for (int h = 0; h < N; h++) { R.iv_left.push_back(h == g ? lo : 0); R.iv_right.push_back(h == g ? hi : 0); R.iv_reverse.push_back(0); }
-                    R.dp_score.push_back(0);
-                    niv++;
-                }
-                if (i < sp.size() && sp[i].second + 1 > cur) cur = sp[i].second + 1;
-            }
+            niv += island_sweep(sp.data(), (int64_t)sp.size(), c->lens[(size_t)g], &ncols, [&](int64_t col, int64_t lo, int64_t len) {
+                R.col_off.push_back(col);
+                Island is; is.col = col; is.len = len; is.bit = 1u << g; is.pad = 0;
+                isl.push_back(is);
+                for (int h = 0; h < N; h++) { R.iv_left.push_back(h == g ? lo : 0); R.iv_right.push_back(h == g ? lo + len - 1 : 0); R.iv_reverse.push_back(0); }
+                R.dp_score.push_back(0);
+            });
         }
         if (ncols > S.sum) { c->err = "assemble_device: more columns than bases (internal error)"; return MAUVE_ERR_HIP; }
-        if (!isl.empty()) {
+        if (isl_dev) {
+            const int64_t *h_isl = h_lw + nl + 1;
+            if (h_isl[0] != (int64_t)isl.size() || h_isl[1] != ncols) { c->err = "assemble_device: the device's island table differs from the host's (internal error)"; return MAUVE_ERR_HIP; }
+        } else if (!isl.empty()) {
             const size_t ib = isl.size() * sizeof(Island);
             HIPCHK(c, c->pin_asm.ensure(64 + rows_bytes + ib + 64));
             char *pi = c->pin_asm.as<char>() + 64 + rows_bytes;
@@ -287,7 +422,7 @@
             HIPCHK(c, c->as_isl.ensure(ib + 64));
             HIPCHK(c, hipMemcpyAsync(c->as_isl.p, pi, ib, hipMemcpyHostToDevice, c->stream));
             hipLaunchKernelGGL(as_islands, dim3((uint32_t)std::min<size_t>(isl.size(), 1024)), dim3(256), 0, c->stream,
-                               c->as_isl.as<Island>(), (uint32_t)isl.size(), out);
+                               c->as_isl.as<Island>(), (uint32_t)isl.size(), (const int64_t *)nullptr, out, fo.d_err, (int64_t *)nullptr);
             HIPCHK(c, hipGetLastError());
             HIPCHK(c, hipStreamSynchronize(c->stream));
         }
@@ -318,8 +453,9 @@
     R.sz.n_gap_dp = fo.n_dp; R.sz.n_dp_cells = cells;
     *sizes = R.sz;
     const double t2 = now_ms();
-    if (trace) fprintf(stderr, "[trace] assemble (device): layout+fill %.3f ms, islands+tables %.3f\n", t1 - t0, t2 - t1);
-    c->stage.assemble_ms = t2 - t0;
+    if (trace) fprintf(stderr, "[trace] assemble (device): layout+fill %.3f ms, islands+tables %.3f; islands: %s\n", t1 - t0, t2 - t1,
+                       !S.p.add_unaligned ? "none" : isl_dev ? "device" : "host");
+    c->stage.assemble_ms = (t2 - S.t_dp0) - c->stage.dp_ms;
     c->stage.total_ms = t2 - S.t0;
     S.open = false;
     return MAUVE_OK;
diff --git a/mauvealigner_amd/csrc/common.hpp b/mauvealigner_amd/csrc/common.hpp
--- a/mauvealigner_amd/csrc/common.hpp
+++ b/mauvealigner_amd/csrc/common.hpp
@@ -265,7 +265,10 @@
     std::vector<uint8_t> rec_flags;
     bool lazy_matches_ok = false, matches_pending = false;
     int match_nseq = 0;
-    struct DpFrontOut { const int32_t *alen, *ast, *alcb, *gapcode; const int64_t *col_off, *score; const uint32_t *cols; int64_t n_dp, n_cols; } dpf_out{};
+    struct DpFrontOut {
+        const int32_t *alen, *ast, *alcb, *gapcode; const int64_t *col_off, *score; const uint32_t *cols; int64_t n_dp;
+        const int64_t *d_err; const volatile int64_t *h_err, *h_cells, *h_cols;
+    } dpf_out{};
     std::vector<DpSeqDesc> prog_desc;
     const int64_t *dp_last_col_off = nullptr; int64_t dp_last_n = 0;
     int64_t dp_band_from = INT64_MAX;
@@ -438,7 +441,8 @@
 int dp_run_from_anchors(mauve_ctx *ctx, int N, int64_t na, const int32_t *h_len, const int32_t *h_st, const int32_t *h_lcb, int gapped,
                         int64_t max_gapped_len, const mauve_scoring *scoring, int32_t *gapcode, int64_t *n_dp_out, int64_t *code_total_out,
                         PinnedBuf *dcols, std::vector<int64_t> &dcol_off, std::vector<int64_t> &dscore, int64_t *cells, int stay = 0);
-int assemble_device(mauve_ctx *c, int64_t na, int64_t cells, mauve_align_sizes *sizes, bool host_chains = false);
+int assemble_device(mauve_ctx *c, int64_t na, mauve_align_sizes *sizes, bool host_chains = false);
+const char *dp_cluster_error();
 int check_columns(mauve_ctx *c, const char *who, int N, int64_t n_iv, const int64_t *left, const int64_t *right, const int64_t *col_off, const uint32_t *d_cols);
 void coord_index_release(mauve_ctx *c);
 int coord_index_arrays(mauve_ctx *c, const char *who, mauve_ctx::CoordIndex &X, DevBuf &index, int nseq, int64_t n_iv, const int64_t *left, const int64_t *right,
diff --git a/mauvealigner_amd/csrc/dev_scan.hpp b/mauvealigner_amd/csrc/dev_scan.hpp
--- a/mauvealigner_amd/csrc/dev_scan.hpp
+++ b/mauvealigner_amd/csrc/dev_scan.hpp
@@ -96,10 +96,16 @@
 }
 
 
+template <class In> __device__ __forceinline__ auto vscan_live(const In &in, int) -> decltype(in.live()) { return in.live(); }
+template <class In> __device__ __forceinline__ bool vscan_live(const In &, long) { return true; }
+template <class In> __device__ __forceinline__ auto vscan_open(const In &in, uint32_t t, uint32_t nt, int) -> decltype(in.open(t, nt)) { in.open(t, nt); }
+template <class In> __device__ __forceinline__ void vscan_open(const In &, uint32_t, uint32_t, long) {}
 template <class T, class In>
 __global__ void __launch_bounds__(256) vscan_partial(In in, uint32_t n, T *__restrict__ bsum)
 {
     __shared__ T red[4];
+    if (!vscan_live(in, 0)) return;
+    vscan_open(in, blockIdx.x * 256u + threadIdx.x, gridDim.x * 256u, 0);
     const uint32_t r0 = blockIdx.x * (uint32_t)TILE + threadIdx.x * 4u;
     T s = 0;
 #pragma unroll
@@ -115,6 +121,7 @@
 {
     __shared__ T red[4];
     __shared__ T s_before, s_all;
+    if (!vscan_live(in, 0)) return;
     const int lane = threadIdx.x & 63, wave = threadIdx.x >> 6;
     T sb = 0, sa = 0;
     for (uint32_t t = threadIdx.x; t < gridDim.x; t += 256) { const T x = bsum[t]; sa += x; if (t < blockIdx.x) sb += x; }
@@ -145,4 +152,85 @@
     if (blockIdx.x == 0 && threadIdx.x == 0) { if (total) *total = s_all; out[n] = s_all; }
 }
 
-}
+template <class In> __device__ __forceinline__ auto vscan_each(const In &in, uint32_t i, int) -> decltype(in.each(i)) { in.each(i); }
+template <class In> __device__ __forceinline__ void vscan_each(const In &, uint32_t, long) {}
+template <int K, class In>
+__global__ void __launch_bounds__(256) vscank_partial(In in, uint32_t n, int64_t *__restrict__ bsum)
+{
+    __shared__ int64_t red[K][4];
+    const uint32_t r0 = blockIdx.x * (uint32_t)TILE + threadIdx.x * 4u;
+    int64_t s[K];
+#pragma unroll
+    for (int k = 0; k < K; k++) s[k] = 0;
+#pragma unroll
+    for (int i = 0; i < 4; i++)
+        if (r0 + i < n) {
+            int64_t v[K];
+            in.values(r0 + i, v);
+            vscan_each(in, r0 + i, 0);
+#pragma unroll
+            for (int k = 0; k < K; k++) s[k] += v[k];
+        }
+#pragma unroll
+    for (int k = 0; k < K; k++) {
+#pragma unroll
+        for (int o = 32; o > 0; o >>= 1) s[k] += __shfl_down(s[k], o);
+        if ((threadIdx.x & 63) == 0) red[k][threadIdx.x >> 6] = s[k];
+    }
+    __syncthreads();
+    if (threadIdx.x < K) bsum[(size_t)threadIdx.x * gridDim.x + blockIdx.x] = red[threadIdx.x][0] + red[threadIdx.x][1] + red[threadIdx.x][2] + red[threadIdx.x][3];
+}
+template <int K, class In, class Out>
+__global__ void __launch_bounds__(256) vscank_write(In in, Out out, uint32_t n, const int64_t *__restrict__ bsum)
+{
+    __shared__ int64_t red[2 * K][4];
+    __shared__ int64_t wsum[K][4];
+    const int lane = threadIdx.x & 63, wave = threadIdx.x >> 6;
+    int64_t before[K], all[K];
+#pragma unroll
+    for (int k = 0; k < K; k++) {
+        int64_t sb = 0, sa = 0;
+        for (uint32_t t = threadIdx.x; t < gridDim.x; t += 256) { const int64_t x = bsum[(size_t)k * gridDim.x + t]; sa += x; if (t < blockIdx.x) sb += x; }
+#pragma unroll
+        for (int o = 32; o > 0; o >>= 1) { sb += __shfl_down(sb, o); sa += __shfl_down(sa, o); }
+        if (lane == 0) { red[2 * k][wave] = sb; red[2 * k + 1][wave] = sa; }
+    }
+    __syncthreads();
+#pragma unroll
+    for (int k = 0; k < K; k++) {
+        before[k] = red[2 * k][0] + red[2 * k][1] + red[2 * k][2] + red[2 * k][3];
+        all[k] = red[2 * k + 1][0] + red[2 * k + 1][1] + red[2 * k + 1][2] + red[2 * k + 1][3];
+    }
+    const uint32_t r0 = blockIdx.x * (uint32_t)TILE + threadIdx.x * 4u;
+    int64_t v[4][K], run[K];
+#pragma unroll
+    for (int i = 0; i < 4; i++) {
+        if (r0 + i < n) in.values(r0 + i, v[i]);
+        else {
+#pragma unroll
+            for (int k = 0; k < K; k++) v[i][k] = 0;
+        }
+    }
+#pragma unroll
+    for (int k = 0; k < K; k++) {
+        const int64_t s = v[0][k] + v[1][k] + v[2][k] + v[3][k];
+        int64_t inc = s;
+#pragma unroll
+        for (int o = 1; o < 64; o <<= 1) { const int64_t t = __shfl_up(inc, o); if (lane >= o) inc += t; }
+        if (lane == 63) wsum[k][wave] = inc;
+        run[k] = before[k] + inc - s;
+    }
+    __syncthreads();
+#pragma unroll
+    for (int k = 0; k < K; k++)
+        for (int w = 0; w < wave; w++) run[k] += wsum[k][w];
+#pragma unroll
+    for (int i = 0; i < 4; i++) {
+        if (r0 + i < n) out.put(r0 + i, run);
+#pragma unroll
+        for (int k = 0; k < K; k++) run[k] += v[i][k];
+    }
+    if (blockIdx.x == 0 && threadIdx.x == 0) out.total(all);
+}
+
+}
diff --git a/mauvealigner_amd/csrc/dp_batch.hip b/mauvealigner_amd/csrc/dp_batch.hip
--- a/mauvealigner_amd/csrc/dp_batch.hip
+++ b/mauvealigner_amd/csrc/dp_batch.hip
@@ -1613,6 +1613,7 @@
 }
 
 static const char *const DP_ERR_CLUSTER = "dp: a cluster of workgroups could not make progress on an interval (wide sweep)";
+const char *dp_cluster_error() { return DP_ERR_CLUSTER; }
 static DpScoring dp_scoring_of(const mauve_scoring *scoring)
 {
     DpScoring sc; sc.go = scoring->gap_open; sc.ge = scoring->gap_extend; memcpy(sc.s, scoring->matrix, sizeof sc.s);
@@ -1850,13 +1851,23 @@
         need[s] = z.need; rowsn[s] = z.rows(); est[s] = z.est; cand[s] = z.cand(); cls[s] = z.cls();
         sizekey[s] = z.sizekey(); slotval[s] = s;
     }
+    __device__ void put_empty(uint32_t s) const
+    {
+        need[s] = 0; rowsn[s] = 0; est[s] = 0; cand[s] = 0; cls[s] = 0;
+        sizekey[s] = 63u; slotval[s] = s;
+    }
 };
 __global__ void __launch_bounds__(256) dpf_desc(const int32_t *__restrict__ alen, const int32_t *__restrict__ ast, int N,
-                                                const uint32_t *__restrict__ anchor_of, const DpFrontTotals *__restrict__ tot,
+                                                const uint32_t *__restrict__ anchor_of, const DpFrontTotals *__restrict__ tot, uint32_t na,
                                                 DpSeqDesc *__restrict__ desc, DpSizingOut out, int no_mw, int no_groups, int64_t band_from, int class_mode)
 {
     const uint32_t s = blockIdx.x * 256u + threadIdx.x;
-    if (s >= (uint32_t)tot->n_dp) return;
+    if (s >= na) return;
+    if (s >= (uint32_t)tot->n_dp) {
+        for (int g = 0; g < N; g++) { DpSeqDesc d; d.genome = g; d.rev = 0; d.lo0 = 0; d.len = 0; desc[(size_t)s * N + g] = d; }
+        out.put_empty(s);
+        return;
+    }
     const uint32_t k = anchor_of[s];
     int64_t longest = 0;
     for (int g = 0; g < N; g++) {
@@ -1886,20 +1897,41 @@
     for (int g = 0; g < N; g++) z.add(desc[(size_t)s * N + g].len);
     out.put(s, z);
 }
-struct DescLen { const DpSeqDesc *d; __device__ int64_t value(uint32_t i) const { return d[i].len; } };
-struct ArrVal { const int64_t *a; __device__ int64_t value(uint32_t i) const { return a[i]; } };
-struct ListVal { const int64_t *a; const uint32_t *order; __device__ int64_t value(uint32_t j) const { return a[order[j]]; } };
-__global__ void __launch_bounds__(256) dpf_tb_scatter(const int64_t *__restrict__ tb_list, const uint32_t *__restrict__ order, uint32_t n, int64_t *__restrict__ tb_off)
-{
-    const uint32_t j = blockIdx.x * 256u + threadIdx.x;
-    if (j < n) tb_off[order[j]] = tb_list[j];
-}
+struct DpOffsetsIn {
+    const DpSeqDesc *d; const int64_t *rowsn, *est; int N;
+    __device__ void values(uint32_t s, int64_t v[3]) const
+    {
+        int64_t b = 0;
+        for (int g = 0; g < N; g++) b += d[(size_t)s * N + g].len;
+        v[0] = b; v[1] = rowsn[s]; v[2] = est[s];
+    }
+};
+struct DpOffsetsOut {
+    const DpSeqDesc *d; int N; uint32_t n; int64_t *seq_off, *rows_off; DpFrontTotals *tot;
+    __device__ void put(uint32_t s, const int64_t e[3]) const
+    {
+        int64_t b = e[0];
+        for (int g = 0; g < N; g++) { seq_off[(size_t)s * N + g] = b; b += d[(size_t)s * N + g].len; }
+        rows_off[s] = e[1];
+    }
+    __device__ void total(const int64_t a[3]) const { seq_off[(size_t)n * N] = a[0]; rows_off[n] = a[1]; tot->codes = a[0]; tot->rows = a[1]; tot->est = a[2]; }
+};
+struct DpTbIn { const int64_t *need; const uint32_t *order; __device__ void values(uint32_t j, int64_t v[1]) const { v[0] = need[order[j]]; } };
+struct DpTbOut {
+    const uint32_t *order; uint32_t n; int64_t *tb_list, *tb_off; DpFrontTotals *tot;
+    __device__ void put(uint32_t j, const int64_t e[1]) const { tb_list[j] = e[0]; tb_off[order[j]] = e[0]; }
+    __device__ void total(const int64_t a[1]) const { tb_list[n] = a[0]; tot->tb = a[0]; }
+};
 
 struct DpBigPick {
-    const uint32_t *order; const uint8_t *cand, *cls; const int64_t *est; const DpFrontTotals *tot; uint32_t *key2; int64_t wide_min; uint32_t maxn;
-    __device__ uint32_t domain(int) const { return (uint32_t)tot->n_dp; }
-    __device__ bool flag(uint32_t j, int) const { const uint32_t s = order[j]; return cand[s] == 1 && est[s] >= wide_min; }
-    __device__ void each(uint32_t j, uint32_t before, bool fl, int) const { key2[j] = ((fl && before < maxn) || cand[order[j]] == 2) ? 0u : (uint32_t)cls[order[j]]; }
+    const uint32_t *order; const uint8_t *cand, *cls; const int64_t *est; const DpFrontTotals *tot; uint32_t *key2; int64_t wide_min; uint32_t maxn, n;
+    __device__ uint32_t domain(int) const { return n; }
+    __device__ bool flag(uint32_t j, int) const { if (j >= (uint32_t)tot->n_dp) return false; const uint32_t s = order[j]; return cand[s] == 1 && est[s] >= wide_min; }
+    __device__ void each(uint32_t j, uint32_t before, bool fl, int) const
+    {
+        if (j >= (uint32_t)tot->n_dp) { key2[j] = 7u; return; }
+        key2[j] = ((fl && before < maxn) || cand[order[j]] == 2) ? 0u : (uint32_t)cls[order[j]];
+    }
     __device__ void emit(uint32_t, uint32_t, int) const {}
     __device__ void total(uint32_t, int) const {}
 };
@@ -1918,13 +1950,16 @@
         if (j == 0) tot->first_med = lo; else if (j == 1) tot->first_c = lo; else if (j == 2) tot->first_s32 = lo; else tot->first_s16 = lo;
     }
 }
-struct MetaCols { const DpMeta *m; __device__ int64_t value(uint32_t i) const { return m[i].m; } };
-struct MetaCells { const DpMeta *m; __device__ int64_t value(uint32_t i) const { return m[i].cells; } };
-__global__ void __launch_bounds__(256) dpf_scores(const DpMeta *__restrict__ meta, uint32_t n, int64_t *__restrict__ score, DpFrontTotals *__restrict__ tot)
-{
-    const uint32_t i = blockIdx.x * 256u + threadIdx.x;
-    if (i < n) { score[i] = meta[i].score; if (meta[i].pad) tot->err = 1; }
-}
+struct DpResultsIn {
+    const DpMeta *m; int64_t *score; DpFrontTotals *tot;
+    __device__ void values(uint32_t i, int64_t v[2]) const { v[0] = m[i].m; v[1] = m[i].cells; }
+    __device__ void each(uint32_t i) const { score[i] = m[i].score; if (m[i].pad) tot->err = 1; }
+};
+struct DpResultsOut {
+    uint32_t n; int64_t *col_off; DpFrontTotals *tot;
+    __device__ void put(uint32_t i, const int64_t e[2]) const { col_off[i] = e[0]; }
+    __device__ void total(const int64_t a[2]) const { col_off[n] = a[0]; tot->cols = a[0]; tot->cells = a[1]; }
+};
 
 }
 
@@ -1940,7 +1975,7 @@
     const uint32_t nb = (na + TILE - 1) / TILE;
     auto up8 = [](size_t x) { return (x + 7) & ~(size_t)7; };
     const size_t o_cand = (size_t)na * 24, o_k = up8(o_cand + 2 * (size_t)na), o_bcnt = o_k + (size_t)na * 20, o_bsum = up8(o_bcnt + (size_t)nb * 4),
-                 o_bsum2 = o_bsum + ((size_t)nb * N + 8) * 8, w_total = o_bsum2 + ((size_t)nb + 8) * 8;
+                 o_bsum2 = o_bsum + ((size_t)nb * (N > 3 ? N : 3) + 8) * 8, w_total = o_bsum2 + ((size_t)nb + 8) * 8;
     HIPCHK(ctx, ctx->dp_desc.ensure((size_t)na * N * sizeof(DpSeqDesc)));
     HIPCHK(ctx, ctx->dpf_work.ensure(w_total));
     HIPCHK(ctx, ctx->dp_off.ensure(((size_t)na * N + 1 + 3 * ((size_t)na + 1)) * sizeof(int64_t)));
@@ -1959,22 +1994,24 @@
     return MAUVE_OK;
 }
 
-struct DpFrontRun { int64_t n_big; DpClasses cl; int rounds; double t_sized; };
-static int dpf_run(mauve_ctx *ctx, const DpFrontWork &W, int N, uint32_t n_dp, const DpScoring &sc, DpFrontTotals *ht, DpFrontRun &R)
-{
-    const uint32_t nbd = (n_dp + TILE - 1) / TILE, nbs = (n_dp * (uint32_t)N + TILE - 1) / TILE, blk_d = (n_dp + 255) / 256;
+struct DpFrontRun { int64_t n_big; DpClasses cl; int rounds; double t_sized; uint32_t n_dp; };
+static int dpf_run(mauve_ctx *ctx, const DpFrontWork &W, int N, uint32_t n_slots, int64_t n_known, const DpScoring &sc, DpFrontTotals *ht, DpFrontRun &R,
+                   void *also_dst = nullptr, const void *also_src = nullptr, size_t also_bytes = 0)
+{
+    uint32_t n_dp = n_slots;
+    uint32_t nbd = (n_dp + TILE - 1) / TILE, blk_d = (n_dp + 255) / 256;
     DpFrontTotals *tot = W.tot;
-    hipLaunchKernelGGL((vscan_partial<int64_t, DescLen>), dim3(nbs), dim3(256), 0, ctx->stream, DescLen{W.desc}, n_dp * (uint32_t)N, W.bsum);
-    hipLaunchKernelGGL((vscan_write<int64_t, DescLen>), dim3(nbs), dim3(256), 0, ctx->stream, DescLen{W.desc}, n_dp * (uint32_t)N, W.bsum, W.d_seq_off, &tot->codes);
-    hipLaunchKernelGGL((vscan_partial<int64_t, ArrVal>), dim3(nbd), dim3(256), 0, ctx->stream, ArrVal{W.rowsn}, n_dp, W.bsum);
-    hipLaunchKernelGGL((vscan_write<int64_t, ArrVal>), dim3(nbd), dim3(256), 0, ctx->stream, ArrVal{W.rowsn}, n_dp, W.bsum, W.d_rows_off, &tot->rows);
-    hipLaunchKernelGGL((vscan_partial<int64_t, ArrVal>), dim3(nbd), dim3(256), 0, ctx->stream, ArrVal{W.est}, n_dp, W.bsum2);
-    hipLaunchKernelGGL((vscan_write<int64_t, ArrVal>), dim3(nbd), dim3(256), 0, ctx->stream, ArrVal{W.est}, n_dp, W.bsum2, W.d_col_off , &tot->est);
+    {
+        const DpOffsetsIn oi{W.desc, W.rowsn, W.est, N};
+        const DpOffsetsOut oo{W.desc, N, n_dp, W.d_seq_off, W.d_rows_off, tot};
+        hipLaunchKernelGGL((vscank_partial<3, DpOffsetsIn>), dim3(nbd), dim3(256), 0, ctx->stream, oi, n_dp, W.bsum);
+        hipLaunchKernelGGL((vscank_write<3, DpOffsetsIn, DpOffsetsOut>), dim3(nbd), dim3(256), 0, ctx->stream, oi, oo, n_dp, W.bsum);
+    }
     uint32_t *ok = W.k1, *ov = W.v1;
     int rc = sort_pairs_u32(ctx, n_dp, 6, &ok, &ov, W.k2, W.v2, MAUVE_K_MISC);
     if (rc) return rc;
     uint32_t *fk = ok == W.k1 ? W.k2 : W.k1, *fv = ov == W.v1 ? W.v2 : W.v1;
-    const DpBigPick bp{ov, W.cand, W.cls, W.est, tot, fk, dp_wide_min(), (uint32_t)dp_big_max()};
+    const DpBigPick bp{ov, W.cand, W.cls, W.est, tot, fk, dp_wide_min(), (uint32_t)dp_big_max(), n_dp};
     hipLaunchKernelGGL((cmp_count<DpBigPick>), dim3(nbd), dim3(256), 0, ctx->stream, bp, W.bcnt);
     hipLaunchKernelGGL((cmp_write<DpBigPick>), dim3(nbd), dim3(256), 0, ctx->stream, bp, W.bcnt);
     uint32_t *ck = fk, *cv = ov;
@@ -1982,12 +2019,21 @@
     if (rc) return rc;
     hipLaunchKernelGGL(dpf_list, dim3(blk_d), dim3(256), 0, ctx->stream, ck, cv, tot, ctx->dp_list.as<int64_t>(), W.d_seq_off, N);
     int64_t *tb_list_dev = W.d_col_off;
-    hipLaunchKernelGGL((vscan_partial<int64_t, ListVal>), dim3(nbd), dim3(256), 0, ctx->stream, ListVal{W.need, cv}, n_dp, W.bsum2);
-    hipLaunchKernelGGL((vscan_write<int64_t, ListVal>), dim3(nbd), dim3(256), 0, ctx->stream, ListVal{W.need, cv}, n_dp, W.bsum2, tb_list_dev, &tot->tb);
-    hipLaunchKernelGGL(dpf_tb_scatter, dim3(blk_d), dim3(256), 0, ctx->stream, tb_list_dev, cv, n_dp, W.d_tb_off);
+    {
+        const DpTbIn ti{W.need, cv};
+        const DpTbOut to{cv, n_dp, tb_list_dev, W.d_tb_off, tot};
+        hipLaunchKernelGGL((vscank_partial<1, DpTbIn>), dim3(nbd), dim3(256), 0, ctx->stream, ti, n_dp, W.bsum2);
+        hipLaunchKernelGGL((vscank_write<1, DpTbIn, DpTbOut>), dim3(nbd), dim3(256), 0, ctx->stream, ti, to, n_dp, W.bsum2);
+    }
     HIPCHK(ctx, hipGetLastError());
     HIPCHK(ctx, hipMemcpyAsync(ht, tot, sizeof(DpFrontTotals), hipMemcpyDeviceToHost, ctx->stream));
+    if (also_bytes) HIPCHK(ctx, hipMemcpyAsync(also_dst, also_src, also_bytes, hipMemcpyDeviceToHost, ctx->stream));
     HIPCHK(ctx, hipStreamSynchronize(ctx->stream));
+    n_dp = n_known >= 0 ? (uint32_t)n_known : (uint32_t)ht->n_dp;
+    R.n_dp = n_dp; R.n_big = 0; R.rounds = 0; R.t_sized = now_ms(); memset(&R.cl, 0, sizeof R.cl);
+    if (n_dp > n_slots) { ctx->err = "dp: more intervals than slots (internal error)"; return MAUVE_ERR_HIP; }
+    if (n_dp == 0) return MAUVE_OK;
+    nbd = (n_dp + TILE - 1) / TILE; blk_d = (n_dp + 255) / 256;
     const int64_t total = ht->codes, tbt = ht->tb, rwt = ht->rows;
     DpClasses &cl = R.cl; memset(&cl, 0, sizeof cl);
     R.n_big = ht->first_med;
@@ -2008,11 +2054,12 @@
     rc = dp_launch_rounds(ctx, N, n_dp, R.n_big, (int64_t)ht->big_len, cl, W.d_seq_off, W.d_tb_off, W.d_rows_off, sc, tb_list.empty() ? nullptr : tb_list.data(), &R.rounds, ctx->dp_band_from);
     if (rc) return rc;
     const DpMeta *meta = ctx->dp_meta.as<DpMeta>();
-    hipLaunchKernelGGL((vscan_partial<int64_t, MetaCols>), dim3(nbd), dim3(256), 0, ctx->stream, MetaCols{meta}, n_dp, W.bsum);
-    hipLaunchKernelGGL((vscan_write<int64_t, MetaCols>), dim3(nbd), dim3(256), 0, ctx->stream, MetaCols{meta}, n_dp, W.bsum, W.d_col_off, &tot->cols);
-    hipLaunchKernelGGL((vscan_partial<int64_t, MetaCells>), dim3(nbd), dim3(256), 0, ctx->stream, MetaCells{meta}, n_dp, W.bsum2);
-    hipLaunchKernelGGL((vscan_write<int64_t, MetaCells>), dim3(nbd), dim3(256), 0, ctx->stream, MetaCells{meta}, n_dp, W.bsum2, W.rowsn , &tot->cells);
-    hipLaunchKernelGGL(dpf_scores, dim3(blk_d), dim3(256), 0, ctx->stream, meta, n_dp, W.need, tot);
+    {
+        const DpResultsIn ri{meta, W.need, tot};
+        const DpResultsOut ro{n_dp, W.d_col_off, tot};
+        hipLaunchKernelGGL((vscank_partial<2, DpResultsIn>), dim3(nbd), dim3(256), 0, ctx->stream, ri, n_dp, W.bsum);
+        hipLaunchKernelGGL((vscank_write<2, DpResultsIn, DpResultsOut>), dim3(nbd), dim3(256), 0, ctx->stream, ri, ro, n_dp, W.bsum);
+    }
     const uint32_t gblocks = (uint32_t)std::min<int64_t>(((int64_t)n_dp + 3) / 4, 256 * 8);
     hipLaunchKernelGGL(dp_gather, dim3(gblocks), dim3(256), 0, ctx->stream, N, (int64_t)n_dp, W.d_seq_off, meta, ctx->dp_prof_mask.as<uint32_t>(),
                        ctx->dp_prof2_mask.as<uint32_t>(), W.d_col_off, ctx->dp_cols.as<uint32_t>());
@@ -2052,36 +2099,31 @@
     const DpSlots sl{d_gapcode, na, anchor_of, tot};
     hipLaunchKernelGGL((cmp_count<DpSlots>), dim3(nb), dim3(256), 0, ctx->stream, sl, W.bcnt);
     hipLaunchKernelGGL((cmp_write<DpSlots>), dim3(nb), dim3(256), 0, ctx->stream, sl, W.bcnt);
-    hipLaunchKernelGGL(dpf_desc, dim3(blocks), dim3(256), 0, ctx->stream, alen, ast, N, anchor_of, tot, W.desc, W.sizing(),
+    hipLaunchKernelGGL(dpf_desc, dim3(blocks), dim3(256), 0, ctx->stream, alen, ast, N, anchor_of, tot, na, W.desc, W.sizing(),
                        (int)no_mw, (int)no_groups, ctx->dp_band_from, dp_class_mode());
     HIPCHK(ctx, hipGetLastError());
     HIPCHK(ctx, ctx->pin_dp_in.ensure(256 + (size_t)na * 4));
     DpFrontTotals *ht = ctx->pin_dp_in.as<DpFrontTotals>();
     int32_t *h_gapcode = reinterpret_cast<int32_t *>(ctx->pin_dp_in.as<char>() + 256);
-    HIPCHK(ctx, hipMemcpyAsync(ht, tot, sizeof(DpFrontTotals), hipMemcpyDeviceToHost, ctx->stream));
-    if (!stay_on_device) HIPCHK(ctx, hipMemcpyAsync(h_gapcode, d_gapcode, (size_t)na * 4, hipMemcpyDeviceToHost, ctx->stream));
-    HIPCHK(ctx, hipStreamSynchronize(ctx->stream));
-    const uint32_t n_dp = (uint32_t)ht->n_dp;
-    if (!stay_on_device) memcpy(gapcode, h_gapcode, (size_t)na * 4);
-    *n_dp_out = n_dp;
     int64_t *d_col_off = W.d_col_off, *d_score = W.need;
     mauve_ctx::DpFrontOut &fo = ctx->dpf_out;
-    fo.alen = alen; fo.ast = ast; fo.alcb = alcb; fo.gapcode = d_gapcode; fo.col_off = d_col_off; fo.score = d_score; fo.cols = nullptr; fo.n_dp = n_dp; fo.n_cols = 0;
+    fo.alen = alen; fo.ast = ast; fo.alcb = alcb; fo.gapcode = d_gapcode; fo.col_off = d_col_off; fo.score = d_score; fo.cols = nullptr; fo.n_dp = 0;
+    fo.d_err = &tot->err; fo.h_err = fo.h_cells = fo.h_cols = nullptr;
     const double t1 = now_ms();
+    DpFrontRun R;
+    rc = dpf_run(ctx, W, N, na, -1, dp_scoring_of(scoring), ht, R, stay_on_device ? nullptr : h_gapcode, d_gapcode, stay_on_device ? 0 : (size_t)na * 4);
+    if (rc) return rc;
+    const uint32_t n_dp = R.n_dp;
+    if (!stay_on_device) memcpy(gapcode, h_gapcode, (size_t)na * 4);
+    *n_dp_out = n_dp; fo.n_dp = n_dp;
     if (n_dp == 0) return MAUVE_OK;
-    DpFrontRun R;
-    rc = dpf_run(ctx, W, N, n_dp, dp_scoring_of(scoring), ht, R);
-    if (rc) return rc;
     *code_total_out = ht->codes;
     const double t2 = R.t_sized;
     if (ctx->shadow) { std::function<void()> f; f.swap(ctx->shadow); f(); }
     if (stay_on_device) {
         HIPCHK(ctx, hipMemcpyAsync(ht, tot, sizeof(DpFrontTotals), hipMemcpyDeviceToHost, ctx->stream));
-        HIPCHK(ctx, hipStreamSynchronize(ctx->stream));
-        if (ht->err) { ctx->err = DP_ERR_CLUSTER; return MAUVE_ERR_HIP; }
-        if (cells) *cells = ht->cells;
-        fo.cols = ctx->dp_cols.as<uint32_t>(); fo.n_cols = ht->cols;
-        if (trace) fprintf(stderr, "[trace] dp (device front, results stay): %u intervals (%lld workgroup, %lld one-wave, %lld two/wave, %lld four/wave), %d round(s); gaps+slots %.3f ms, sizing+order %.3f, kernels+offsets %.3f\n",
+        fo.cols = ctx->dp_cols.as<uint32_t>(); fo.h_err = &ht->err; fo.h_cells = &ht->cells; fo.h_cols = &ht->cols;
+        if (trace) fprintf(stderr, "[trace] dp (device front, results stay): %u intervals (%lld workgroup, %lld one-wave, %lld two/wave, %lld four/wave), %d round(s); gaps+slots %.3f ms, sizing+order %.3f, kernels+offsets queued %.3f\n",
                            n_dp, (long long)R.n_big, (long long)R.cl.n_med, (long long)R.cl.n_s32, (long long)R.cl.n_s16, R.rounds, t1 - t0, t2 - t1, now_ms() - t2);
         return MAUVE_OK;
     }
@@ -2166,7 +2208,7 @@
                        ctx->dp_band_from, dp_class_mode());
     const DpScoring sc = dp_scoring_of(scoring);
     DpFrontRun R;
-    rc = dpf_run(ctx, W, N, n_dp, sc, ht, R);
+    rc = dpf_run(ctx, W, N, n_dp, (int64_t)n_dp, sc, ht, R);
     if (rc) return rc;
     int64_t *d_col_off = W.d_col_off, *d_score = W.need;
     HIPCHK(ctx, ctx->pin_meta.ensure(((size_t)n_dp * 3 + 2) * 8));
diff --git a/mauvealigner_amd/csrc/island_sweep.hpp b/mauvealigner_amd/csrc/island_sweep.hpp
--- /dev/null
+++ b/mauvealigner_amd/csrc/island_sweep.hpp
@@ -0,0 +1,31 @@
+#pragma once
+#include <cstdint>
+#ifndef __host__
+#define __host__
+#define __device__
+#endif
+
+struct IslandExtent {
+    int64_t left, right;
+    __host__ __device__ bool operator<(const IslandExtent &o) const { return left != o.left ? left < o.left : right < o.right; }
+};
+
+__host__ __device__ inline int64_t island_gap(int64_t max_right, int64_t next_left, int64_t *lo)
+{
+    const int64_t cur = max_right + 1;
+    *lo = cur;
+    return next_left - cur;
+}
+
+template <class Emit>
+__host__ __device__ inline int64_t island_sweep(const IslandExtent *ext, int64_t n, int64_t glen, int64_t *col, Emit emit)
+{
+    int64_t max_right = 0, count = 0;
+    for (int64_t i = 0; i <= n; i++) {
+        int64_t lo;
+        const int64_t len = island_gap(max_right, i < n ? ext[i].left : glen + 1, &lo);
+        if (len > 0) { emit(*col, lo, len); *col += len; count++; }
+        if (i < n && ext[i].right > max_right) max_right = ext[i].right;
+    }
+    return count;
+}
diff --git a/mauvealigner_amd/csrc/pipeline.cpp b/mauvealigner_amd/csrc/pipeline.cpp
--- a/mauvealigner_amd/csrc/pipeline.cpp
+++ b/mauvealigner_amd/csrc/pipeline.cpp
@@ -658,7 +658,7 @@
                                  nullptr, S.dcol_off, S.dscore, &cells, 2);
         if (c->shadow) { std::function<void()> f; f.swap(c->shadow); f(); }
         if (rc) return rc;
-        return assemble_device(c, na, cells, sizes, true);
+        return assemble_device(c, na, sizes, true);
     }
     { const int rck = kept_mums_to_host(c); if (rck) return rck; }
     rc = dp_run_from_anchors(c, N, na, h_len, h_st, h_lcb, S.p.gapped, dp_len_limit(&S.p), &S.p.scoring, gapcode, &S.n_dp, &S.code_total,
@@ -738,7 +738,7 @@
                                  nullptr, S.dcol_off, S.dscore, &cells, 1);
         if (c->shadow) { std::function<void()> f; f.swap(c->shadow); if (!rc) f(); }
         if (rc || rc_pf) return rc ? rc : rc_pf;
-        return assemble_device(c, S.n_anchor, cells, sizes);
+        return assemble_device(c, S.n_anchor, sizes);
     }
     if (host_front) return align_dp_finish(c, sizes, !no_shadow);
     return align_tail_host_chains(c, sizes);
```
